# fhausmann/deepgrp

Measured on AMD Instinct MI355X. Metric: Mbp/sec predicted (whole node) at window=200 stride=50, 5-class, higher is better.
Workload: dtype f16

## Files before the change

### deepgrp_amd/_lib.py

```python
from __future__ import annotations

import ctypes as C
import os

_HERE = os.path.dirname(os.path.abspath(__file__))
LIB_PATH = os.path.join(_HERE, "libdeepgrp_hip.so")

i64, i32, vp, cint = C.c_int64, C.c_int32, C.c_void_p, C.c_int


class DgrpError(RuntimeError):
    """A libdeepgrp_hip call failed (message from dgrp_last_error())."""


class Segment(C.Structure):
    _fields_ = [("start", C.c_int64), ("end", C.c_int64), ("label", C.c_int32), ("contig", C.c_int32)]


class TrainJob(C.Structure):
    _fields_ = [("T", cint), ("u", cint), ("C", cint), ("attention", cint), ("d_params", vp), ("d_idx", vp), ("d_truth", vp),
                ("n", i64), ("d_starts", vp), ("B", i64), ("d_masks", vp), ("d_loss", vp), ("d_grads", vp), ("d_work", vp),
                ("work_bytes", i64)]


class InflateStreamStats(C.Structure):
    _fields_ = [(k, C.c_int64) for k in ("spans", "candidates", "repaired", "rounds", "longest_span", "false_starts", "chunks", "reserved")]

    def as_dict(self):
        return {k: int(getattr(self, k)) for k, _ in self._fields_ if k != "reserved"}


TRAIN_MAX_JOBS = 8

_SIGNATURES = {
    "dgrp_abi_version": (cint, []),
    "dgrp_last_error": (C.c_char_p, []),
    "dgrp_device_info": (cint, [C.c_char_p, C.c_size_t, C.POINTER(cint), C.POINTER(i64)]),
    "dgrp_strip_n": (cint, [vp, i64, C.POINTER(i64), C.POINTER(i64)]),
    "dgrp_encode": (cint, [vp, i64, vp, vp]),
    "dgrp_onehot": (cint, [vp, i64, vp, vp]),
    "dgrp_fasta_workspace_bytes": (i64, [i64]),
    "dgrp_fasta_encode": (cint, [vp, i64, vp, C.POINTER(i64), vp, i64, vp]),
    "dgrp_fasta_batch_workspace_bytes": (i64, [i64, i64]),
    "dgrp_fasta_encode_batch": (cint, [vp, i64, vp, vp, vp, vp, vp, i64, vp]),
    "dgrp_fasta_chunks_workspace_bytes": (i64, [i64]),
    "dgrp_fasta_chunks": (cint, [vp, i64, i64, vp, vp, C.POINTER(i64), vp, i64, vp]),
    "dgrp_fasta_mask_workspace_bytes": (i64, [i64, i64, i64]),
    "dgrp_fasta_mask_batch": (cint, [vp, i64, vp, vp, vp, vp, cint, C.c_uint64, vp, vp, i64, vp]),
    "dgrp_fasta_extract_workspace_bytes": (i64, [i64, i64, i64]),
    "dgrp_fasta_extract_batch": (cint, [vp, i64, vp, vp, vp, vp, vp, vp, i64, cint, C.c_uint64, vp, i64, C.POINTER(i64), vp, C.POINTER(i64),
                                        vp, i64, vp]),
    "dgrp_repeat_summary_workspace_bytes": (i64, [i64, i64, i64]),
    "dgrp_repeat_summary_batch": (cint, [vp, i64, vp, vp, vp, vp, cint, i64, vp, vp, vp, vp, vp, i64, vp]),
    "dgrp_twobit_workspace_bytes": (i64, [i64]),
    "dgrp_twobit_encode_batch": (cint, [vp, i64, i64, vp, vp, vp, vp, i64, vp, vp, i64, vp, i64, vp]),
    "dgrp_twobit_text_batch": (cint, [vp, i64, i64, vp, vp, vp, vp, vp, vp, i64, vp, vp, i64, vp, vp, i64, vp, i64, vp]),
    "dgrp_twobit_pack_workspace_bytes": (i64, [i64, i64]),
    "dgrp_twobit_pack_batch": (cint, [vp, i64, vp, vp, vp, i64, i64, vp, vp, vp, i64, vp]),
    "dgrp_format_rows_bound": (i64, [i64, i64]),
    "dgrp_format_rows": (cint, [vp, vp, i64, cint, vp, i64, vp, i64, C.POINTER(i64)]),
    "dgrp_track_workspace_bytes": (i64, [i64, i64]),
    "dgrp_track_text": (cint, [vp, i64, cint, cint, cint, i64, i64, C.c_char_p, i64, vp, i64, C.POINTER(i64), vp, i64, vp]),
    "dgrp_track_batch_workspace_bytes": (i64, [i64, vp, vp, i64, cint, i64]),
    "dgrp_track_text_batch": (cint, [vp, cint, i64, vp, vp, vp, C.c_char_p, vp, vp, cint, cint, i64, vp, i64, vp, vp, i64, vp]),
    "dgrp_track_index_workspace_bytes": (i64, [i64, vp, vp, i64, cint, i64]),
    "dgrp_track_index_batch": (cint, [vp, cint, i64, vp, vp, vp, C.c_char_p, vp, vp, cint, cint, i64, vp, i64, vp, vp, i64, vp, i64, vp]),
    "dgrp_track_sections_workspace_bytes": (i64, [i64, vp, vp, i64, cint]),
    "dgrp_track_sections_batch": (cint, [vp, cint, i64, vp, vp, vp, vp, cint, cint, i64, i64, vp, i64, vp, vp, i64, vp, vp, i64, vp]),
    "dgrp_track_zoom_workspace_bytes": (i64, [i64, vp, vp, i64, cint]),
    "dgrp_track_zoom_batch": (cint, [vp, cint, i64, vp, vp, vp, vp, cint, cint, i64, i64, vp, i64, vp, vp, i64, vp, vp, vp, i64, vp]),
    "dgrp_zlib_bound": (i64, [i64, i64]),
    "dgrp_zlib_workspace_bytes": (i64, [i64, cint]),
    "dgrp_zlib_compress_batch": (cint, [vp, i64, vp, i64, i64, cint, vp, i64, vp, C.POINTER(i64), vp, i64, vp]),
    "dgrp_zlib_compress_host": (cint, [vp, i64, vp, i64, i64, cint, vp, i64, vp, C.POINTER(i64)]),
    "dgrp_window_count":(i64, [i64, i64, i64]),
    "dgrp_windows_onehot": (cint, [vp, i64, i64, i64, i64, i64, cint, vp, vp]),
    "dgrp_model_create": (cint, [C.POINTER(vp), cint, cint, cint, cint, vp, vp, vp, vp, vp, vp]),
    "dgrp_model_create_lstm": (cint, [C.POINTER(vp), cint, cint, cint, vp, vp, vp, vp, vp]),
    "dgrp_model_destroy": (cint, [vp]),
    "dgrp_model_dims": (cint, [vp, C.POINTER(cint), C.POINTER(cint), C.POINTER(cint), C.POINTER(cint)]),
    "dgrp_model_flags": (cint, [vp]),
    "dgrp_model_set_precision": (cint, [vp, cint]),
    "dgrp_model_view": (cint, [vp, cint, C.POINTER(vp)]),
    "dgrp_model_plan": (cint, [vp, cint, i64, C.POINTER(cint), C.POINTER(i64), C.POINTER(cint), C.POINTER(cint)]),
    "dgrp_forward_workspace_bytes": (i64, [vp, i64]),
    "dgrp_forward_window_chunk": (i64, [vp]),
    "dgrp_forward_windows": (cint, [vp, vp, i64, i64, i64, i64, vp, vp, i64, vp]),
    "dgrp_forward_merge": (cint, [vp, vp, i64, i64, i64, i64, i64, vp, vp, i64, vp]),
    "dgrp_forward_merge_record": (cint, [vp, vp, i64, i64, i64, vp, vp, i64, vp]),
    "dgrp_forward_merge_record_workspace_bytes": (i64, [vp, i64, i64]),
    "dgrp_forward_reference_workspace_bytes": (i64, [vp, i64]),
    "dgrp_forward_windows_reference": (cint, [vp, vp, i64, i64, i64, i64, vp, vp, i64, vp]),
    "dgrp_get_max": (cint, [vp, i64, vp, i64, i64, i64, i64, vp]),
    "dgrp_scores": (cint, [vp, i64, cint, vp, vp, vp]),
    "dgrp_softmax_labels": (cint, [vp, i64, cint, vp, vp, vp, i64, vp]),
    "dgrp_mss_workspace_bytes": (i64, [i64]),
    "dgrp_mss_labels": (cint, [vp, vp, i64, cint, cint, cint, vp, vp, vp, i64, vp]),
    "dgrp_mss_segments_host": (cint, [vp, i64, vp, i64, C.POINTER(i64)]),
    "dgrp_mss_batch_workspace_bytes": (i64, [i64, i64]),
    "dgrp_mss_labels_batch": (cint, [vp, vp, i64, i64, vp, cint, cint, cint, vp, vp, i64, vp]),
    "dgrp_segments_workspace_bytes": (i64, [i64]),
    "dgrp_segments": (cint, [vp, i64, i64, i32, vp, i64, vp, vp, i64, vp]),
    "dgrp_record_workspace_bytes": (i64, [vp, i64, i64, cint]),
    "dgrp_predict_record": (cint, [vp, vp, i64, i64, i64, cint, cint, cint, i64, i32, vp, i64, C.POINTER(i64), vp, i64, vp]),
    "dgrp_batch_workspace_bytes": (i64, [vp, i64, vp, i64]),
    "dgrp_predict_batch": (cint, [vp, vp, i64, vp, vp, vp, vp, i64, i64, cint, cint, vp, i64, C.POINTER(i64), vp, i64, vp]),
    "dgrp_batch_rows": (i64, [i64, vp]),
    "dgrp_predict_batch_probs": (cint, [vp, vp, i64, vp, vp, vp, vp, i64, i64, cint, cint, vp, i64, C.POINTER(i64), vp, i64, vp, vp]),
    "dgrp_confusion_matrix": (cint, [vp, vp, i64, cint, vp, vp, vp]),
    "dgrp_filter_segments": (cint, [vp, vp, i64, i64, vp]),
    "dgrp_eval_workspace_bytes": (i64, [i64, i64]),
    "dgrp_paint_rows_batch": (cint, [vp, i64, vp, vp, vp, vp, vp, vp, i64, vp]),
    "dgrp_row_hits_batch": (cint, [vp, i64, vp, vp, vp, vp, vp, vp, vp, i64, vp]),
    "dgrp_row_scores_workspace_bytes": (i64, [i64, i64]),
    "dgrp_row_scores_batch": (cint, [vp, cint, i64, vp, vp, vp, vp, vp, vp, vp, i64, vp]),
    "dgrp_prob_hist_workspace_bytes": (i64, [i64, cint, cint]),
    "dgrp_prob_hist_batch": (cint, [vp, cint, i64, vp, vp, vp, vp, cint, vp, vp, vp, i64, vp]),
    "dgrp_row_detect_workspace_bytes": (i64, [i64, i64]),
    "dgrp_paint_row_keys_batch": (cint, [vp, i64, vp, vp, vp, vp, vp, vp, vp, i64, vp]),
    "dgrp_row_detect_batch": (cint, [vp, i64, vp, vp, vp, vp, vp, vp, vp, vp, i64, vp]),
    "dgrp_format_bed_bound": (i64, [i64, i64]),
    "dgrp_format_bed_rows": (cint, [vp, vp, i64, cint, vp, vp, i64, cint, vp, i64, C.POINTER(i64)]),
    "dgrp_bed_text_workspace_bytes": (i64, [i64, i64, i64]),
    "dgrp_bed_text_batch": (cint, [vp, vp, i64, cint, vp, vp, i64, cint, vp, i64, C.POINTER(i64), vp, i64, vp]),
    "dgrp_bed_index_workspace_bytes": (i64, [i64, i64, i64, i64]),
    "dgrp_bed_index_batch": (cint, [vp, vp, i64, cint, vp, vp, i64, cint, i64, vp, vp, i64, C.POINTER(i64), vp, i64, vp, vp, i64, vp]),
    "dgrp_gff_text_workspace_bytes": (i64, [i64, i64, i64, i64, i64]),
    "dgrp_gff_text_batch": (cint, [vp, vp, i64, cint, vp, vp, i64, vp, vp, i64, cint, i64, vp, i64, C.POINTER(i64), C.POINTER(i64), vp, i64,
                                   vp]),
    "dgrp_gff_index_workspace_bytes": (i64, [i64, i64, i64, i64, i64, i64]),
    "dgrp_gff_index_batch": (cint, [vp, vp, i64, cint, vp, vp, i64, vp, vp, i64, cint, i64, i64, vp, vp, i64, C.POINTER(i64), vp, i64, vp, vp,
                                    i64, vp]),
    "dgrp_bed_blocks_workspace_bytes": (i64, [i64, i64, vp]),
    "dgrp_bed_blocks_batch": (cint, [cint, vp, vp, i64, cint, i64, vp, i64, vp, i64, C.POINTER(i64), vp, i64, C.POINTER(i64), C.POINTER(i64),
                                     vp, i64, vp]),
    "dgrp_bed_zoom_workspace_bytes": (i64, [i64, i64, vp]),
    "dgrp_bed_zoom_batch": (cint, [cint, vp, vp, i64, cint, i64, vp, i64, vp, i64, vp, vp, i64, vp, vp, vp, i64, vp]),
    "dgrp_inflate_raw_host": (cint, [vp, i64, vp, i64, C.POINTER(i64), C.POINTER(i64), C.POINTER(cint)]),
    "dgrp_inflate_workspace_bytes": (i64, [i64]),
    "dgrp_inflate_batch": (cint, [vp, i64, i64, vp, vp, vp, vp, i64, C.POINTER(i64), C.POINTER(cint), vp, i64, vp]),
    "dgrp_inflate_stream_host": (cint, [vp, i64, i64, i64, cint, vp, i64, C.POINTER(i64), C.POINTER(i64), vp, C.POINTER(cint)]),
    "dgrp_inflate_stream_workspace_bytes": (i64, [i64, i64]),
    "dgrp_inflate_stream_scan": (cint, [vp, i64, i64, i64, i64, cint, C.POINTER(i64), vp, C.POINTER(cint), vp, i64, vp]),
    "dgrp_inflate_stream_write": (cint, [vp, i64, i64, i64, vp, vp, i64, C.POINTER(C.c_uint32), C.POINTER(i64), C.POINTER(cint), vp, i64,
                                         vp]),
    "dgrp_bgzf_bound": (i64, [i64, cint]),
    "dgrp_bgzf_workspace_bytes": (i64, [i64]),
    "dgrp_bgzf_compress": (cint, [vp, i64, vp, i64, C.POINTER(i64), cint, vp, i64, vp]),
    "dgrp_bgzf_compress_host": (cint, [vp, i64, vp, i64, C.POINTER(i64), cint]),
    "dgrp_bgzf_workspace_bytes_level": (i64, [i64, cint]),
    "dgrp_bgzf_compress_level": (cint, [vp, i64, vp, i64, C.POINTER(i64), cint, cint, vp, i64, vp]),
    "dgrp_bgzf_compress_host_level": (cint, [vp, i64, vp, i64, C.POINTER(i64), cint, cint]),
    "dgrp_train_param_count": (i64, [cint, cint, cint]),
    "dgrp_train_workspace_bytes": (i64, [cint, cint, cint, cint, i64]),
    "dgrp_train_step": (cint, [cint, cint, cint, cint, vp, vp, vp, i64, vp, i64, vp, vp, vp, vp, i64, vp]),
    "dgrp_train_step_multi": (cint, [C.POINTER(TrainJob), cint, vp]),
    "dgrp_optimizer_step": (cint, [cint, vp, vp, vp, vp, i64, C.c_double, C.c_double, C.c_double, C.c_double, i64, vp]),
    "dgrp_truth_workspace_bytes": (i64, [i64, i64]),
    "dgrp_truth_multihot_batch": (cint, [vp, cint, i64, i64, vp, vp, vp, vp, vp, vp, i64, vp]),
    "dgrp_class_starts_workspace_bytes": (i64, [i64, i64]),
    "dgrp_class_window_starts": (cint, [vp, i64, i64, vp, vp, cint, vp, i64, C.POINTER(i64), vp, i64, vp]),
    "dgrp_train_resolve_starts": (cint, [vp, i64, vp, vp, cint, vp, vp, i64, vp, vp]),
    "dgrp_kernel_timer_enable": (cint, [cint]),
    "dgrp_kernel_timer_read": (cint, [C.POINTER(C.c_double), C.POINTER(i64), C.POINTER(i64)]),
}

_lib = None


def lib() -> C.CDLL:
    global _lib
    if _lib is None:
        if not os.path.exists(LIB_PATH):
            raise ImportError(
                f"{LIB_PATH} is missing: build it with `make -C deepgrp_amd/csrc` (hipcc, gfx950) "
                "or `python -c 'import __graft_entry__ as g; g.build()'`. There is no CPU fallback.")
        import torch
        L = C.CDLL(LIB_PATH)
        for name, (res, args) in _SIGNATURES.items():
            f = getattr(L, name)
            f.restype = res
            f.argtypes = args
        if L.dgrp_abi_version() != 1:
            raise ImportError("libdeepgrp_hip.so ABI version mismatch")
        _lib = L
    return _lib


def check(rc: int, what: str = "") -> None:
    if rc != 0:
        msg = lib().dgrp_last_error().decode("utf-8", "replace")
        raise DgrpError(f"{what or 'libdeepgrp_hip'} failed (code {rc}): {msg}")


def name_blob(names):
    import numpy as np
    raw = [nm if isinstance(nm, bytes) else nm.encode("utf-8", "surrogateescape") for nm in names]
    off = np.zeros(len(raw) + 1, np.int64)
    np.cumsum([len(x) for x in raw], out=off[1:])
    return raw, b"".join(raw), off


def exported_symbols():
    return sorted(_SIGNATURES)
```

### deepgrp_amd/csrc/api.hip

```cpp
#include "dgrp_model.h"

#include <stdarg.h>
#include <string.h>

#include <algorithm>
#include <vector>
#include <mutex>

static thread_local char g_err[512] = "";

void dgrp_set_error(const char *fmt, ...)
{
    va_list ap;
    va_start(ap, fmt);
    vsnprintf(g_err, sizeof(g_err), fmt, ap);
    va_end(ap);
}

DGRP_EXPORT int dgrp_abi_version(void) { return DGRP_ABI_VERSION; }
DGRP_EXPORT const char *dgrp_last_error(void) { return g_err; }

DGRP_EXPORT int dgrp_device_info(char *name, size_t name_cap, int *cu_count, int64_t *hbm_bytes)
{
    int dev = 0;
// ... 545 lines not shown

DGRP_EXPORT int dgrp_model_plan(const dgrp_model *m, int mode, int64_t step, int *kernel, int64_t *lds_bytes, int *ospan, int *avg_up)
{
    DGRP_REQUIRE(m, "dgrp_model_plan: NULL model");
    DGRP_REQUIRE(kernel && lds_bytes && ospan && avg_up, "dgrp_model_plan: NULL output pointer");
    DGRP_REQUIRE(mode >= 0 && mode <= 2, "dgrp_model_plan: mode %d (0 merged, 1 window probabilities, 2 attention pre-pass)", mode);
    DGRP_REQUIRE(step >= 1, "dgrp_model_plan: step %lld < 1", (long long)step);
    DGRP_REQUIRE(mode != 2 || m->attention, "dgrp_model_plan: mode 2 on a model without attention");
    if (m->ref_only) {
        *kernel = DGRP_KERNEL_FP32; *lds_bytes = 0; *ospan = 0; *avg_up = 0;
        return DGRP_OK;
    }
    const dgrp_gru_plan plan = dgrp_gru_plan_for(m, mode, step);
    *kernel = (int)plan.kernel; *lds_bytes = (int64_t)plan.lds; *ospan = plan.ospan; *avg_up = plan.avg_up;
    return DGRP_OK;
}

DGRP_EXPORT int dgrp_model_set_precision(dgrp_model *m, int level)
{
    DGRP_REQUIRE(m, "dgrp_model_set_precision: NULL model");
    DGRP_REQUIRE(level == 0 || level == 1, "dgrp_model_set_precision: level must be 0 (fp16 operands) or 1 (split operands)");
    if (m->ref_only) return DGRP_OK;
    DGRP_REQUIRE(level == 0 || m->d_pack_lo || m->d_stream, "dgrp_model_set_precision: this model has no split-operand kernel");
    m->precision = level;
    return DGRP_OK;
}

static int64_t ref_sub_windows(const dgrp_model *m)
{
    const int64_t per = 2 * (int64_t)m->T * m->u * 4 + (int64_t)m->T * (m->C + 1) * 4 + 2 * (int64_t)m->u * 4;
    return std::max<int64_t>(16, std::min<int64_t>(4096, (512ll << 20) / per) / 16 * 16);
}

DGRP_EXPORT int64_t dgrp_forward_workspace_bytes(const dgrp_model *m, int64_t nw)
{
    if (!m || nw < 0) return 0;
    if (m->ref_only) {
        const int64_t sub = std::min<int64_t>(ref_sub_windows(m), std::max<int64_t>(nw, 1));
        return dgrp_align_up(dgrp_forward_reference_workspace_bytes(m, sub), 256) + dgrp_align_up(sub * m->T * (int64_t)m->C * 4, 256);
    }
    if (!m->attention) return 256;
    return dgrp_align_up(nw * m->T * (int64_t)m->UP * 4, 256) + dgrp_align_up(nw * m->T * (int64_t)m->C * 4, 256) + 256;
}

static unsigned *forward_queue(const dgrp_model *m, int64_t nw, void *d_work, int64_t work_bytes)
{
    if (!d_work || work_bytes < dgrp_forward_workspace_bytes(m, nw)) return nullptr;
    return (unsigned *)((char *)d_work + (m->attention ? dgrp_forward_workspace_bytes(m, nw) - 256 : 0));
}

static int forward_ref(const dgrp_model *m, const uint8_t *d_idx, int64_t n, int64_t s, dgrp_placement place, int64_t w0, int64_t nw,
                       int merge, float *d_out, void *d_work, int64_t work_bytes, hipStream_t stream)
{
    if (work_bytes < dgrp_forward_workspace_bytes(m, nw) || !d_work) {
        dgrp_set_error("dgrp_forward: this model runs on the fp32 kernels and needs %lld bytes of workspace for %lld windows",
                       (long long)dgrp_forward_workspace_bytes(m, nw), (long long)nw);
        return DGRP_ENOMEM;
    }
    const int64_t sub = std::min<int64_t>(ref_sub_windows(m), nw);
    const int64_t ref_bytes = dgrp_align_up(dgrp_forward_reference_workspace_bytes(m, sub), 256);
    float *probs = (float *)((char *)d_work + ref_bytes);
    for (int64_t a = w0; a < w0 + nw; a += sub) {
        const int64_t k = std::min<int64_t>(sub, w0 + nw - a);
        float *dst = merge ? probs : d_out + (a - w0) * (int64_t)m->T * m->C;
        int rc = dgrp_forward_windows_reference(m, d_idx, n, s, a, k, dst, d_work, ref_bytes, stream);
        if (rc) return rc;
        if (!merge) continue;
        for (int64_t b = a; b < a + k;) {
            const int64_t e = (b < place.nfullB && a + k > place.nfullB) ? place.nfullB : a + k;
            const int64_t row = dgrp_place_row(place, b, s);
            if (row < n) {
                rc = dgrp_get_max(d_out + row * m->C, n - row, probs + (b - a) * (int64_t)m->T * m->C, m->T, m->C, s, e - b, stream);
                if (rc) return rc;
            }
            b = e;
        }
    }
    return DGRP_OK;
}

static int forward_common(const dgrp_model *m, const uint8_t *d_idx, int64_t n, int64_t s, int64_t batch, int64_t w0,
                          int64_t nw, int merge, float *d_out, void *d_work, int64_t work_bytes, hipStream_t stream)
{
    DGRP_REQUIRE(m && s >= 1 && w0 >= 0 && nw >= 0 && n >= 0, "dgrp_forward: bad arguments");
    if (nw == 0) return DGRP_OK;
    DGRP_REQUIRE(d_idx && d_out, "dgrp_forward: NULL pointer");
    DGRP_REQUIRE((w0 + nw - 1) * s + m->T <= n, "dgrp_forward: window %lld (start %lld) runs past n=%lld",
                 (long long)(w0 + nw - 1), (long long)((w0 + nw - 1) * s), (long long)n);
    dgrp_placement place = { 0, 0 };
    if (merge) {
        DGRP_REQUIRE(batch >= 1, "dgrp_forward_merge: batch must be >= 1");
        const int64_t total = dgrp_window_count(n, m->T, s);
        DGRP_REQUIRE(w0 + nw <= total, "dgrp_forward_merge: windows %lld..%lld exceed the record's %lld",
                     (long long)w0, (long long)(w0 + nw), (long long)total);
        place = dgrp_make_placement(total, batch);
    }
    if (m->ref_only) return forward_ref(m, d_idx, n, s, place, w0, nw, merge, d_out, d_work, work_bytes, stream);
    if (!m->attention)
        return dgrp_gru_launch(m, dgrp_gru_plan_for(m, merge ? 0 : 1, s), d_idx, n, place, w0, nw, d_out, nullptr,
                               forward_queue(m, nw, d_work, work_bytes), stream);
    if (work_bytes < dgrp_forward_workspace_bytes(m, nw) || !d_work) {
        dgrp_set_error("dgrp_forward: attention model needs %lld bytes of workspace for %lld windows",
                       (long long)dgrp_forward_workspace_bytes(m, nw), (long long)nw);
        return DGRP_ENOMEM;
    }
    void *avg = d_work;
    float *pl = (float *)((char *)d_work + dgrp_align_up(nw * m->T * (int64_t)m->UP * 4, 256));
    const dgrp_gru_plan pre = dgrp_gru_plan_for(m, 2, s);
    int rc = dgrp_gru_launch(m, pre, d_idx, n, place, w0, nw, pl, avg, forward_queue(m, nw, d_work, work_bytes), stream);
    if (rc) return rc;
    return dgrp_attention_launch_recs(m, pre, place, w0, nw, merge, n, avg, pl, d_out, nullptr, 0, stream);
}

DGRP_EXPORT int dgrp_forward_windows(const dgrp_model *m, const uint8_t *d_idx, int64_t n, int64_t s, int64_t w0,
                                     int64_t nw, float *d_probs, void *d_work, int64_t work_bytes, void *stream)
{
    return forward_common(m, d_idx, n, s, 1, w0, nw, 0, d_probs, d_work, work_bytes, (hipStream_t)stream);
}

DGRP_EXPORT int dgrp_forward_merge(const dgrp_model *m, const uint8_t *d_idx, int64_t n, int64_t s, int64_t batch,
                                   int64_t w0, int64_t nw, float *d_out, void *d_work, int64_t work_bytes, void *stream)
{
    return forward_common(m, d_idx, n, s, batch, w0, nw, 1, d_out, d_work, work_bytes, (hipStream_t)stream);
}

static int64_t spill_cap_bytes()
{
    static const int64_t cap = [] {
        if (const char *e = getenv("DGRP_SPILL_BYTES")) {
            const long long v = atoll(e);
            if (v >= (1ll << 20)) return (int64_t)v;
        }
        size_t free_b = 0, total_b = 0;
        if (hipMemGetInfo(&free_b, &total_b) != hipSuccess || total_b == 0) return (int64_t)(4ll << 30);
        return std::min<int64_t>(8ll << 30, std::max<int64_t>(1ll << 30, (int64_t)(total_b / 32)));
    }();
    return cap;
}

static int64_t record_window_chunk(const dgrp_model *m)
{
    if (m->ref_only) return ref_sub_windows(m);
    if (!m->attention) return 1ll << 23;
    const int64_t per = (int64_t)m->T * ((int64_t)m->UP * 4 + (int64_t)m->C * 4);
    int64_t c = spill_cap_bytes() / per;
    c = c >= 32768 ? c / 32768 * 32768 : c >= 4096 ? c / 4096 * 4096 : c / 16 * 16;
    if (c < 16) c = 16;
    return c < (1ll << 20) ? c : (1ll << 20);
}

DGRP_EXPORT int64_t dgrp_forward_window_chunk(const dgrp_model *m)
{
    return m ? record_window_chunk(m) : 0;
}

#define DGRP_LANES 3
static int64_t lane_window_chunk(const dgrp_model *m)
{
    if (m->ref_only || !m->attention) return 0;
    if (const char *e = getenv("DGRP_LANE_CHUNK")) {
        const long long v = atoll(e);
        return v >= 16 ? (int64_t)(v / 16 * 16) : 0;
    }
    const int64_t c = record_window_chunk(m);
    if (c < 65536) return 0;
    const int64_t lc = c / DGRP_LANES / 32768 * 32768;
    return lc >= 32768 ? lc : 32768;
}
struct lane_pool { hipStream_t s[DGRP_LANES]; int dev; bool ok; };
static lane_pool *lanes_get()
{
    static std::mutex mu;
    static std::vector<lane_pool *> pools;
    int dev = 0;
    if (hipGetDevice(&dev) != hipSuccess) return nullptr;
    std::lock_guard<std::mutex> lock(mu);
    for (lane_pool *q : pools)
        if (q->dev == dev) return q->ok ? q : nullptr;
    lane_pool *q = new lane_pool();
    q->dev = dev; q->ok = true;
    for (int i = 0; i < DGRP_LANES; ++i)
        if (hipStreamCreateWithFlags(&q->s[i], hipStreamNonBlocking) != hipSuccess) q->ok = false;
    pools.push_back(q);
    return q->ok ? q : nullptr;
}

static int64_t record_forward_bytes(const dgrp_model *m, int64_t nwin)
{
    const int64_t lc = lane_window_chunk(m);
    if (lc > 0 && nwin > lc)
        return DGRP_LANES * dgrp_align_up(std::max<int64_t>(dgrp_forward_workspace_bytes(m, std::min(lc, nwin)), 256), 256);
    const int64_t chunk = std::min<int64_t>(record_window_chunk(m), nwin > 0 ? nwin : 1);
    return std::max<int64_t>(dgrp_forward_workspace_bytes(m, chunk), 256);
}

DGRP_EXPORT int64_t dgrp_forward_merge_record_workspace_bytes(const dgrp_model *m, int64_t n, int64_t s)
{
    if (!m || n < 0 || s < 1) return 0;
    return record_forward_bytes(m, dgrp_window_count(n, m->T, s));
}

DGRP_EXPORT int dgrp_forward_merge_record(const dgrp_model *m, const uint8_t *d_idx, int64_t n, int64_t s, int64_t batch, float *d_out,
                                          void *d_work, int64_t work_bytes, void *stream_)
{
    hipStream_t stream = (hipStream_t)stream_;
    DGRP_REQUIRE(m && n >= 0 && s >= 1 && batch >= 1, "dgrp_forward_merge_record: bad arguments");
    const int64_t nwin = dgrp_window_count(n, m->T, s);
    if (nwin == 0) return DGRP_OK;
    DGRP_REQUIRE(d_idx && d_out && d_work, "dgrp_forward_merge_record: NULL pointer");
    const int64_t need = record_forward_bytes(m, nwin);
    if (work_bytes < need) {
        dgrp_set_error("dgrp_forward_merge_record: workspace %lld < %lld bytes", (long long)work_bytes, (long long)need);
        return DGRP_ENOMEM;
    }
    const int64_t lc = lane_window_chunk(m);
    lane_pool *lp = lc > 0 && nwin > lc ? lanes_get() : nullptr;
    if (!lp) {
        const int64_t chunk = lc > 0 && nwin > lc ? lc : record_window_chunk(m);
        for (int64_t w0 = 0; w0 < nwin; w0 += chunk) {
            const int64_t nw = std::min<int64_t>(chunk, nwin - w0);
            const int rc = dgrp_forward_merge(m, d_idx, n, s, batch, w0, nw, d_out, d_work, work_bytes, stream);
            if (rc) return rc;
        }
        return DGRP_OK;
    }
    const int64_t per = need / DGRP_LANES;
    hipEvent_t fork = nullptr, join[DGRP_LANES] = { nullptr, nullptr, nullptr };
    int rc = DGRP_OK;
    auto bail = [&](hipError_t e) { if (e != hipSuccess && rc == DGRP_OK) { dgrp_set_error("dgrp_forward_merge_record: %s", hipGetErrorString(e)); rc = DGRP_EHIP; } };
    bail(hipEventCreateWithFlags(&fork, hipEventDisableTiming));
    for (int i = 0; i < DGRP_LANES; ++i) bail(hipEventCreateWithFlags(&join[i], hipEventDisableTiming));
    if (rc == DGRP_OK) {
        bail(hipEventRecord(fork, stream));
        for (int i = 0; i < DGRP_LANES; ++i) bail(hipStreamWaitEvent(lp->s[i], fork, 0));
        int64_t k = 0;
        for (int64_t w0 = 0; w0 < nwin && rc == DGRP_OK; w0 += lc, ++k) {
            const int64_t nw = std::min<int64_t>(lc, nwin - w0);
            const int lane = (int)(k % DGRP_LANES);
            rc = dgrp_forward_merge(m, d_idx, n, s, batch, w0, nw, d_out, (char *)d_work + lane * per, per, lp->s[lane]);
        }
        for (int i = 0; i < DGRP_LANES; ++i) {
            bail(hipEventRecord(join[i], lp->s[i]));
            bail(hipStreamWaitEvent(stream, join[i], 0));
        }
    }
    if (fork) (void)hipEventDestroy(fork);
    for (int i = 0; i < DGRP_LANES; ++i)
        if (join[i]) (void)hipEventDestroy(join[i]);
    return rc;
}

struct record_layout {
    int64_t out, scores, cls, labels, count, fwd, post, bytes, post_bytes, fwd_bytes;
};

static record_layout record_carve(const dgrp_model *m, int64_t n, int64_t s, int use_mss)
{
    record_layout l;
    int64_t p = 0;
    auto take = [&](int64_t b) { const int64_t q = p; p += dgrp_align_up(b, 256); return q; };
    const int64_t nwin = dgrp_window_count(n, m->T, s);
    l.out = take(n * m->C * 4);
    l.scores = take(use_mss ? n * 8 : 0);
    l.cls = take(use_mss ? n : 0);
    l.labels = take(n);
    l.count = take(8);
    l.fwd_bytes = record_forward_bytes(m, nwin);
    l.fwd = take(l.fwd_bytes);
    l.post_bytes = std::max<int64_t>(std::max<int64_t>(use_mss ? dgrp_mss_workspace_bytes(n) : 4096, dgrp_segments_workspace_bytes(n)), 4096);
    l.post = take(l.post_bytes);
    l.bytes = p;
    return l;
}

DGRP_EXPORT int64_t dgrp_record_workspace_bytes(const dgrp_model *m, int64_t n, int64_t s, int use_mss)
{
    if (!m || n < 0 || s < 1) return 0;
    return record_carve(m, n, s, use_mss).bytes;
}

DGRP_EXPORT int dgrp_predict_record(const dgrp_model *m, const uint8_t *d_idx, int64_t n, int64_t s, int64_t batch,
                                    int min_mss_len, int xdrop_len, int use_mss, int64_t offset, int32_t contig,
                                    dgrp_segment *d_records, int64_t cap, int64_t *h_count, void *d_work,
                                    int64_t work_bytes, void *stream_)
{
    hipStream_t stream = (hipStream_t)stream_;
    DGRP_REQUIRE(m && n >= 0 && s >= 1 && batch >= 1 && cap >= 0 && h_count, "dgrp_predict_record: bad arguments");
    *h_count = 0;
    if (n == 0) return DGRP_OK;
    DGRP_REQUIRE(d_idx && d_work && (cap == 0 || d_records), "dgrp_predict_record: NULL pointer");
    const record_layout l = record_carve(m, n, s, use_mss);
    if (work_bytes < l.bytes) {
        dgrp_set_error("dgrp_predict_record: workspace %lld < %lld bytes", (long long)work_bytes, (long long)l.bytes);
        return DGRP_ENOMEM;
    }
    char *w = (char *)d_work;
    float *out = (float *)(w + l.out);
    int8_t *labels = (int8_t *)(w + l.labels);
    int64_t *d_count = (int64_t *)(w + l.count);
    DGRP_HIP(hipMemsetAsync(out, 0, (size_t)n * m->C * 4, stream));
    int rc = dgrp_forward_merge_record(m, d_idx, n, s, batch, out, w + l.fwd, l.fwd_bytes, stream);
    if (rc) return rc;
    if (use_mss) {
        rc = dgrp_scores(out, n, m->C, (double *)(w + l.scores), (int8_t *)(w + l.cls), stream);
        if (rc) return rc;
        rc = dgrp_mss_labels((const double *)(w + l.scores), (const int8_t *)(w + l.cls), n, m->C, min_mss_len, xdrop_len,
                             labels, nullptr, w + l.post, l.post_bytes, stream);
    } else {
        rc = dgrp_softmax_labels(out, n, m->C, nullptr, labels, w + l.post, l.post_bytes, stream);
    }
    if (rc) return rc;
    rc = dgrp_segments(labels, n, offset, contig, d_records, cap, d_count, w + l.post, l.post_bytes, stream);
    if (rc) return rc;
    DGRP_HIP(hipMemcpyAsync(h_count, d_count, 8, hipMemcpyDeviceToHost, stream));
    DGRP_HIP(hipStreamSynchronize(stream));
    return DGRP_OK;
}

int dgrp_batch_marks(const int64_t *d_start, const int64_t *d_len, int64_t nrec, int64_t total_n, uint8_t *d_marks,
                     double *d_scores, int8_t *d_cls, hipStream_t stream);
int dgrp_batch_segments(const int8_t *d_labels, const uint8_t *d_marks, int64_t total_n, const int64_t *d_start, int64_t nrec,
                        const int64_t *d_startpos, const int32_t *d_contig, dgrp_segment *d_records, int64_t cap,
                        int64_t *d_count, void *d_work, int64_t work_bytes, hipStream_t stream);

struct batch_layout {
    int64_t out, scores, cls, labels, marks, count, recs, wgf, start, len, spos, contig, post, post_bytes, avg, pl, queue, bytes;
};

static batch_layout batch_carve(const dgrp_model *m, int64_t nrec, int64_t total_rows, int64_t total_windows)
{
    batch_layout l;
    int64_t p = 0;
    auto take = [&](int64_t b) { const int64_t q = p; p += dgrp_align_up(b, 256); return q; };
    l.out = take(total_rows * m->C * 4);
    l.scores = take(total_rows * 8);
    l.cls = take(total_rows);
    l.labels = take(total_rows);
    l.marks = take(total_rows);
    l.count = take(8);
    l.recs = take(nrec * 64);
    l.wgf = take((nrec + 1) * 8);
    l.start = take((nrec + 1) * 8);
    l.len = take(nrec * 8);
    l.spos = take(nrec * 8);
    l.contig = take(nrec * 4);
    l.post_bytes = std::max<int64_t>(std::max<int64_t>(dgrp_mss_batch_workspace_bytes(total_rows, nrec), dgrp_segments_workspace_bytes(total_rows)), 4096);
    l.post = take(l.post_bytes);
    l.avg = take(m->attention ? total_windows * m->T * (int64_t)m->UP * 4 : 0);
    l.pl = take(m->attention ? total_windows * m->T * (int64_t)m->C * 4 : 0);
    l.queue = take(4);
    l.bytes = p;
    return l;
}

static int64_t batch_windows(const dgrp_model *m, int64_t nrec, const int64_t *h_n, int64_t s)
{
    int64_t w = 0;
    for (int64_t r = 0; r < nrec; ++r) w += dgrp_window_count(h_n[r], m->T, s);
    return w;
}

static int64_t batch_rows(int64_t nrec, const int64_t *h_n)
{
    int64_t rows = 0;
    for (int64_t r = 0; r < nrec; ++r) rows += dgrp_align_up(h_n[r], 64);
    return rows;
}

DGRP_EXPORT int64_t dgrp_batch_workspace_bytes(const dgrp_model *m, int64_t nrec, const int64_t *h_n, int64_t s)
{
    if (!m || nrec < 0 || s < 1 || (nrec > 0 && !h_n)) return 0;
    for (int64_t r = 0; r < nrec; ++r)
        if (h_n[r] < 1) return 0;
    return batch_carve(m, nrec, batch_rows(nrec, h_n), batch_windows(m, nrec, h_n, s)).bytes;
}

DGRP_EXPORT int64_t dgrp_batch_rows(int64_t nrec, const int64_t *h_n)
{
    return nrec > 0 && h_n ? batch_rows(nrec, h_n) : 0;
}

static int predict_batch_common(const char *who, const dgrp_model *m, const uint8_t *d_idx, int64_t nrec, const int64_t *h_idx_off,
                                const int64_t *h_n, const int64_t *h_startpos, const int32_t *h_contig, int64_t s,
                                int64_t batch, int min_mss_len, int xdrop_len, dgrp_segment *d_records, int64_t cap,
                                int64_t *h_count, void *d_work, int64_t work_bytes, hipStream_t stream, float *d_probs)
{
    DGRP_REQUIRE(m && nrec >= 0 && s >= 1 && batch >= 1 && cap >= 0 && h_count, "%s: bad arguments", who);
    *h_count = 0;
    if (nrec == 0) return DGRP_OK;
    DGRP_REQUIRE(!m->ref_only && (m->cell == 0 || (m->cell == 1 && m->NW <= 8)), "%s: unsupported model (fp32 path: record by record)", who);
    DGRP_REQUIRE(d_idx && h_idx_off && h_n && h_startpos && h_contig && d_work && (cap == 0 || d_records), "%s: NULL pointer", who);
    for (int64_t r = 0; r < nrec; ++r)
        DGRP_REQUIRE(h_n[r] >= 1 && h_idx_off[r] >= 0, "%s: record %lld: empty records do not belong in a batch", who, (long long)r);
    const int64_t rows = batch_rows(nrec, h_n);
    DGRP_REQUIRE(rows < (1ll << 31), "%s: %lld rows in one batch (limit 2^31)", who, (long long)rows);
    const int64_t windows = batch_windows(m, nrec, h_n, s);
    DGRP_REQUIRE(windows < (1ll << 31), "%s: too many windows in one batch", who);
    const batch_layout l = batch_carve(m, nrec, rows, windows);
    if (work_bytes < l.bytes) {
        dgrp_set_error("%s: workspace %lld < %lld bytes", who, (long long)work_bytes, (long long)l.bytes);
        return DGRP_ENOMEM;
    }
    char *w = (char *)d_work;
    std::vector<int64_t> recs((size_t)nrec * 8, 0), wgf((size_t)nrec + 1, 0), start((size_t)nrec + 1, 0);
    int64_t wfirst = 0;
    for (int64_t r = 0; r < nrec; ++r) {
        const int64_t nwin = dgrp_window_count(h_n[r], m->T, s);
        const dgrp_placement pl = dgrp_make_placement(nwin, batch);
        int64_t *e = recs.data() + (size_t)r * 8;
        e[0] = h_idx_off[r]; e[1] = h_n[r]; e[2] = start[(size_t)r]; e[3] = nwin; e[4] = pl.nfullB; e[5] = pl.shift; e[6] = wfirst;
        wfirst += nwin;
        wgf[(size_t)r + 1] = wgf[(size_t)r] + (nwin + 15) / 16;
        start[(size_t)r + 1] = start[(size_t)r] + dgrp_align_up(h_n[r], 64);
    }
    DGRP_HIP(hipMemcpyAsync(w + l.recs, recs.data(), recs.size() * 8, hipMemcpyHostToDevice, stream));
    DGRP_HIP(hipMemcpyAsync(w + l.wgf, wgf.data(), wgf.size() * 8, hipMemcpyHostToDevice, stream));
    DGRP_HIP(hipMemcpyAsync(w + l.start, start.data(), start.size() * 8, hipMemcpyHostToDevice, stream));
    DGRP_HIP(hipMemcpyAsync(w + l.len, h_n, (size_t)nrec * 8, hipMemcpyHostToDevice, stream));
    DGRP_HIP(hipMemcpyAsync(w + l.spos, h_startpos, (size_t)nrec * 8, hipMemcpyHostToDevice, stream));
    DGRP_HIP(hipMemcpyAsync(w + l.contig, h_contig, (size_t)nrec * 4, hipMemcpyHostToDevice, stream));
    float *out = d_probs ? d_probs : (float *)(w + l.out);
    DGRP_HIP(hipMemsetAsync(out, 0, (size_t)rows * m->C * 4, stream));
    int rc;
    if (!m->attention) {
        rc = dgrp_gru_launch_batch(m, dgrp_gru_plan_for(m, 0, s), d_idx, w + l.recs, (const int64_t *)(w + l.wgf), nrec, wgf[(size_t)nrec],
                                   out, nullptr, (unsigned *)(w + l.queue), stream);
        if (rc) return rc;
    } else {
        const dgrp_gru_plan pre = dgrp_gru_plan_for(m, 2, s);
        rc = dgrp_gru_launch_batch(m, pre, d_idx, w + l.recs, (const int64_t *)(w + l.wgf), nrec, wgf[(size_t)nrec], (float *)(w + l.pl),
                                   w + l.avg, (unsigned *)(w + l.queue), stream);
        if (rc) return rc;
        rc = dgrp_attention_launch_recs(m, pre, dgrp_placement{ 0, 0 }, 0, windows, 1, rows, w + l.avg, (const float *)(w + l.pl), out,
                                        w + l.recs, nrec, stream);
        if (rc) return rc;
    }
    double *scores = (double *)(w + l.scores);
    int8_t *cls = (int8_t *)(w + l.cls), *labels = (int8_t *)(w + l.labels);
    uint8_t *marks = (uint8_t *)(w + l.marks);
    rc = dgrp_scores(out, rows, m->C, scores, cls, stream);
    if (rc) return rc;
    rc = dgrp_batch_marks((const int64_t *)(w + l.start), (const int64_t *)(w + l.len), nrec, rows, marks, scores, cls, stream);
    if (rc) return rc;
    rc = dgrp_mss_labels_batch(scores, cls, rows, nrec, start.data(), m->C, min_mss_len, xdrop_len, labels, w + l.post, l.post_bytes, stream);
    if (rc) return rc;
    int64_t *d_count = (int64_t *)(w + l.count);
    rc = dgrp_batch_segments(labels, marks, rows, (const int64_t *)(w + l.start), nrec, (const int64_t *)(w + l.spos),
                             (const int32_t *)(w + l.contig), d_records, cap, d_count, w + l.post, l.post_bytes, stream);
    if (rc) return rc;
    DGRP_HIP(hipMemcpyAsync(h_count, d_count, 8, hipMemcpyDeviceToHost, stream));
    DGRP_HIP(hipStreamSynchronize(stream));
    return DGRP_OK;
}

DGRP_EXPORT int dgrp_predict_batch(const dgrp_model *m, const uint8_t *d_idx, int64_t nrec, const int64_t *h_idx_off,
                                   const int64_t *h_n, const int64_t *h_startpos, const int32_t *h_contig, int64_t s,
                                   int64_t batch, int min_mss_len, int xdrop_len, dgrp_segment *d_records, int64_t cap,
                                   int64_t *h_count, void *d_work, int64_t work_bytes, void *stream)
{
    return predict_batch_common("dgrp_predict_batch", m, d_idx, nrec, h_idx_off, h_n, h_startpos, h_contig, s, batch, min_mss_len, xdrop_len,
                                d_records, cap, h_count, d_work, work_bytes, (hipStream_t)stream, nullptr);
}

DGRP_EXPORT int dgrp_predict_batch_probs(const dgrp_model *m, const uint8_t *d_idx, int64_t nrec, const int64_t *h_idx_off,
                                         const int64_t *h_n, const int64_t *h_startpos, const int32_t *h_contig, int64_t s,
                                         int64_t batch, int min_mss_len, int xdrop_len, dgrp_segment *d_records, int64_t cap,
                                         int64_t *h_count, void *d_work, int64_t work_bytes, void *stream, float *d_probs)
{
    DGRP_REQUIRE(d_probs || nrec <= 0, "dgrp_predict_batch_probs: NULL d_probs");
    return predict_batch_common("dgrp_predict_batch_probs", m, d_idx, nrec, h_idx_off, h_n, h_startpos, h_contig, s, batch, min_mss_len,
                                xdrop_len, d_records, cap, h_count, d_work, work_bytes, (hipStream_t)stream, d_probs);
}
```

### deepgrp_amd/csrc/mss_kernels.hip

```cpp
#include "dgrp_common.h"
#include "scan.h"
#include <vector>
#include <math.h>

struct mss_cand { int32_t st, en; double L, R; int32_t pre, pad; };

#define MSS_SUB_MIN 256
#define MSS_SUBENT_BYTES 80
struct mss_subent {
    int64_t start, run;
    double L, peak, run_L;
    int64_t run_st;
    int32_t open, first;
    int32_t vci, nst;
    int32_t reset, pad;
    double Lf;
};
static_assert(sizeof(mss_subent) == 80, "MSS_SUBENT_BYTES");
#define MSS_LCAP 160
#define MSS_NEG (-1e30)
#define MSS_QNONE (-4096)
#define MSS_QBAD 4096

struct mss_layout {
    int64_t nblk;
    uint64_t *blk;
    double *blk_sum;
    double *blk_abs;
    int32_t *blk_q;
    uint8_t *flags;
    int64_t nsup;
    double *sup_sum, *sup_abs;
    int32_t *sup_q;
    uint8_t *sup_flags;
    uint64_t *tiles;
    uint64_t *grand;
    int64_t *ustart;
    int64_t *urun;
    double *exitL[2];
    uint64_t *segcnt;
    uint64_t *cutcnt;
    uint64_t *lblk;
    int64_t *lstart, *lrun;
    uint8_t *lforced;
    void *lstate[2];
    int64_t *cut_st, *cut_run;
    double *cut_L;
    int2 *cut_kj;
    int64_t *ustart2, *urun2;
    double *entry2;
    void *subs;
    int64_t dump_cap;
    mss_cand *dump;
    mss_cand *stack;
    int32_t *segs;
    int32_t *segs_out;
    int64_t bytes;
};

static mss_layout mss_carve(void *work, int64_t n)
{
    mss_layout l;
    unsigned char *p = (unsigned char *)work;
    auto take = [&](int64_t bytes) { unsigned char *q = p; p += dgrp_align_up(bytes, 256); return q; };
    l.nblk = (n + 63) / 64;
    const int64_t maxunits = l.nblk + 1, maxruns = n / 2 + 2;
    l.blk = (uint64_t *)take((l.nblk + 1) * 8);
    l.blk_sum = (double *)take(l.nblk * 8);
    l.blk_abs = (double *)take(l.nblk * 8);
    l.blk_q = (int32_t *)take(l.nblk * 4);
    l.flags = (uint8_t *)take(l.nblk + 64);
    l.nsup = (l.nblk + 63) / 64;
    l.sup_sum = (double *)take(l.nsup * 8);
    l.sup_abs = (double *)take(l.nsup * 8);
    l.sup_q = (int32_t *)take(l.nsup * 4);
    l.sup_flags = (uint8_t *)take(l.nsup + 64);
    l.tiles = (uint64_t *)take(((maxunits + 1 + SCAN_TILE - 1) / SCAN_TILE + 1) * 8);
    l.grand = (uint64_t *)take(64);
    l.ustart = (int64_t *)take((maxunits + 1) * 8);
    l.urun = (int64_t *)take((maxunits + 1) * 8);
    l.exitL[0] = (double *)take(maxunits * 8);
    l.exitL[1] = (double *)take(maxunits * 8);
    l.segcnt = (uint64_t *)take((maxunits + 1) * 8);
    l.cutcnt = (uint64_t *)take((maxunits + 1) * 8);
    l.lblk = (uint64_t *)take((l.nblk + 1) * 8);
    l.lstart = (int64_t *)take((maxunits + 1) * 8);
    l.lrun = (int64_t *)take((maxunits + 1) * 8);
    l.lforced = (uint8_t *)take(maxunits + 64);
    l.lstate[0] = take(maxunits * 64);
    l.lstate[1] = take(maxunits * 64);
    l.cut_st = (int64_t *)take(l.nblk * 8);
    l.cut_run = (int64_t *)take(l.nblk * 8);
    l.cut_L = (double *)take(l.nblk * 8);
    l.cut_kj = (int2 *)take(l.nblk * 8);
    l.ustart2 = (int64_t *)take((2 * maxunits + 2) * 8);
    l.urun2 = (int64_t *)take((2 * maxunits + 2) * 8);
    l.entry2 = (double *)take((2 * maxunits + 2) * 8);
    l.subs = take((maxunits + 8) * (int64_t)MSS_SUBENT_BYTES);
    l.dump_cap = 2 * (l.nblk / MSS_SUB_MIN + 2);
    l.dump = (mss_cand *)take(l.dump_cap * MSS_LCAP * (int64_t)sizeof(mss_cand));
    l.stack = (mss_cand *)take(maxruns * (int64_t)sizeof(mss_cand));
    l.segs = (int32_t *)take(maxruns * 8);
    l.segs_out = (int32_t *)take(maxruns * 8);
    l.bytes = p - (unsigned char *)work;
    return l;
}

DGRP_EXPORT int64_t dgrp_mss_workspace_bytes(int64_t n)
{
    if (n < 0) return 0;
    return mss_carve(nullptr, n).bytes;
}

__device__ __forceinline__ int quantum_exp(double x)
{
    const uint64_t b = (uint64_t)__double_as_longlong(x) & 0x7fffffffffffffffull;
    if (b == 0) return MSS_QNONE;
    const int e = (int)(b >> 52);
    if (e == 0 || e == 0x7ff) return MSS_QBAD;
    const uint64_t m = b & 0x000fffffffffffffull;
    const int tz = m ? __builtin_ctzll(m) : 52;
    return -((e - 1023) - 52 + tz);
}

__device__ __forceinline__ bool mss_certified(double L, double sumabs, int q_scores)
{
    const int qL = quantum_exp(L);
    const int Q = qL > q_scores ? qL : q_scores;
    if (Q >= MSS_QBAD) return false;
    const int ex = 53 - Q;
    if (ex > 1000) return true;
    if (ex < -1000) return false;
    return (fabs(L) + sumabs) * 1.0000001 < ldexp(1.0, ex);
}

__device__ __forceinline__ double wave_sum(double v)
{
#pragma unroll
    for (int o = 32; o > 0; o >>= 1) v += __shfl_xor(v, o);
    return v;
}
__device__ __forceinline__ int wave_max(int v)
{
#pragma unroll
    for (int o = 32; o > 0; o >>= 1) { int w = __shfl_xor(v, o); v = w > v ? w : v; }
    return v;
}

__device__ __forceinline__ double lane_value(double x, int l)
{
    const long long b = __double_as_longlong(x);
    const int lo = __builtin_amdgcn_readlane((int)b, l), hi = __builtin_amdgcn_readlane((int)(b >> 32), l);
    return __longlong_as_double(((long long)hi << 32) | (unsigned int)lo);
}

__global__ void __launch_bounds__(256) mss_blockstat_kernel(const double *__restrict__ S, int64_t n,
                                                            uint64_t *__restrict__ blk, double *__restrict__ blk_sum,
                                                            double *__restrict__ blk_abs, int32_t *__restrict__ blk_q,
                                                            uint8_t *__restrict__ flags)
{
    const int lane = threadIdx.x & 63;
    const int64_t b = (int64_t)blockIdx.x * 4 + (threadIdx.x >> 6);
    if (b * 64 >= n) return;
    const int64_t i = b * 64 + lane;
    const double s = i < n ? S[i] : 0.0;
    const bool pos = i < n && s > 0;
    const bool prevpos = i > 0 && i < n && S[i - 1] > 0;
    const unsigned long long mpos = __ballot(pos);
    const unsigned long long mstart = __ballot(pos && !prevpos);
    const double sum = wave_sum(s), sabs = wave_sum(fabs(s));
    const int q = wave_max(quantum_exp(s));
    if (lane == 0) {
        flags[b] = (uint8_t)(mpos != 0ull ? 1 : 0);
        blk[b] = (uint64_t)__popcll(mstart);
        blk_sum[b] = sum;
        blk_abs[b] = sabs;
        blk_q[b] = q;
    }
}

__global__ void __launch_bounds__(256) mss_superstat_kernel(const double *__restrict__ blk_sum, const double *__restrict__ blk_abs,
                                                            const int32_t *__restrict__ blk_q, const uint8_t *__restrict__ flags,
                                                            int64_t nblk, double *__restrict__ sup_sum, double *__restrict__ sup_abs,
                                                            int32_t *__restrict__ sup_q, uint8_t *__restrict__ sup_flags)
{
    const int lane = threadIdx.x & 63;
    const int64_t g = (int64_t)blockIdx.x * 4 + (threadIdx.x >> 6);
    if (g * 64 >= nblk) return;
    const int64_t b = g * 64 + lane;
    const bool in = b < nblk;
    const unsigned long long mp = __ballot(in && (flags[b] & 1));
    const double sum = wave_sum(in ? blk_sum[b] : 0.0), sabs = wave_sum(in ? blk_abs[b] : 0.0);
    const int q = wave_max(in ? blk_q[b] : MSS_QNONE);
    if (lane == 0) {
        sup_flags[g] = (uint8_t)(mp != 0ull ? 1 : 0);
        sup_sum[g] = sum;
        sup_abs[g] = sabs;
        sup_q[g] = q;
    }
}

__device__ __forceinline__ bool mss_is_boundary(const uint8_t *flags, const double *blk_sum, int64_t b, int64_t nblk,
                                                int64_t n, double thr)
{
    if (!(thr > 0.0) || b + 1 >= nblk || (flags[b] & 1) || !(flags[b + 1] & 1)) return false;
    if (b * 64 + 64 > n) return false;
    double cum = 0.0;
    for (int64_t j = b; j >= 0 && j > b - 16; --j) {
        if (flags[j] & 1) break;
        cum += blk_sum[j];
        if (cum < -thr) return true;
    }
    return false;
}

__global__ void __launch_bounds__(256) mss_boundary_kernel(const uint8_t *__restrict__ flags, const double *__restrict__ blk_sum,
                                                           int64_t nblk, int64_t n, double thr, uint64_t *__restrict__ blk)
{
    const int64_t b = (int64_t)blockIdx.x * blockDim.x + threadIdx.x;
    if (b >= nblk) return;
    if (mss_is_boundary(flags, blk_sum, b, nblk, n, thr)) blk[b] |= 1ull << 32;
}

__global__ void __launch_bounds__(256) mss_units_kernel(const uint64_t *__restrict__ blk, const uint8_t *__restrict__ flags,
                                                        const double *__restrict__ blk_sum, int64_t nblk, int64_t n, double thr,
                                                        int64_t *__restrict__ ustart, int64_t *__restrict__ urun,
                                                        const uint64_t *__restrict__ grand)
{
    const int64_t b = (int64_t)blockIdx.x * blockDim.x + threadIdx.x;
    if (b == 0) {
        ustart[0] = 0;
        urun[0] = 0;
        const int64_t nunits = (int64_t)(grand[0] >> 32) + 1;
        ustart[nunits] = n;
        urun[nunits] = (int64_t)(grand[0] & 0xffffffffull);
    }
    if (b >= nblk) return;
    if (mss_is_boundary(flags, blk_sum, b, nblk, n, thr)) {
        const int64_t k = (int64_t)(blk[b] >> 32) + 1;
        ustart[k] = (b + 1) * 64;
        urun[k] = (int64_t)(blk[b] & 0xffffffffull);
    }
}

template <int CTRL, int RMASK>
__device__ __forceinline__ int dpp_i(int src, int old) { return __builtin_amdgcn_update_dpp(old, src, CTRL, RMASK, 0xf, false); }
template <int CTRL, int RMASK>
__device__ __forceinline__ double dpp_d(double src, double old)
{
    const long long s = __double_as_longlong(src), o = __double_as_longlong(old);
    const int lo = __builtin_amdgcn_update_dpp((int)o, (int)s, CTRL, RMASK, 0xf, false);
    const int hi = __builtin_amdgcn_update_dpp((int)(o >> 32), (int)(s >> 32), CTRL, RMASK, 0xf, false);
    return __longlong_as_double(((long long)hi << 32) | (unsigned int)lo);
}
#define DPP_SHR(n) (0x110 + (n))
#define DPP_BCAST15 0x142
#define DPP_BCAST31 0x143
#define DPP_WAVE_SHR1 0x138
#define DPP_SCAN_STEPS(STEP) STEP(DPP_SHR(1), 0xf) STEP(DPP_SHR(2), 0xf) STEP(DPP_SHR(4), 0xf) STEP(DPP_SHR(8), 0xf) STEP(DPP_BCAST15, 0xa) STEP(DPP_BCAST31, 0xc)
__device__ __forceinline__ double scan_add_d(double x)
{
#define STEP(c, m) x = x + dpp_d<c, m>(x, 0.0);
    DPP_SCAN_STEPS(STEP)
#undef STEP
    return x;
}
__device__ __forceinline__ double scan_min_d(double x)
{
#define STEP(c, m) { const double y = dpp_d<c, m>(x, INFINITY); x = y < x ? y : x; }
    DPP_SCAN_STEPS(STEP)
#undef STEP
    return x;
}
__device__ __forceinline__ int scan_max_i(int x)
{
#define STEP(c, m) { const int y = dpp_i<c, m>(x, -1); x = y > x ? y : x; }
    DPP_SCAN_STEPS(STEP)
#undef STEP
    return x;
}
__device__ __forceinline__ void scan_segmax_d(int &fl, double &v)
{
#define STEP(c, m) { const double yv = dpp_d<c, m>(v, -INFINITY); const int yf = dpp_i<c, m>(fl, 0); if (!fl) v = yv > v ? yv : v; fl |= yf; }
    DPP_SCAN_STEPS(STEP)
#undef STEP
}
__device__ __forceinline__ double lane_below_d(double x, double first) { return dpp_d<DPP_WAVE_SHR1, 0xf>(x, first); }
__device__ __forceinline__ int lane_below_i(int x, int first) { return dpp_i<DPP_WAVE_SHR1, 0xf>(x, first); }
__device__ __forceinline__ int lane_value_i(int x, int l) { return __builtin_amdgcn_readlane(x, l); }

__device__ __forceinline__ double mss_fold(double s, double a0, int t, int nvalid, int lane)
{
    const double sm = lane >= t && lane < nvalid ? s : 0.0;
    double X = a0;
    for (int j = t; j < nvalid; j += 4) {
        X = lane_below_d(X, a0) + sm;
        X = lane_below_d(X, a0) + sm;
        X = lane_below_d(X, a0) + sm;
        X = lane_below_d(X, a0) + sm;
    }
    return X;
}

__global__ void __launch_bounds__(64) mss_scan_kernel(const double *__restrict__ S, const int64_t *__restrict__ ustart,
                                                      const int64_t *__restrict__ urun, int64_t nunits,
                                                      const double *__restrict__ exit_prev, double *__restrict__ exit_cur,
                                                      mss_cand *stack_all, int32_t *__restrict__ segs_all,
                                                      uint64_t *__restrict__ segcnt, int min_sc, double xdrop,
                                                      uint64_t *__restrict__ grand, int pass,
                                                      const double *__restrict__ blk_sum, const double *__restrict__ blk_abs,
                                                      const int32_t *__restrict__ blk_q, const uint8_t *__restrict__ flags,
                                                      const double *__restrict__ sup_sum, const double *__restrict__ sup_abs,
                                                      const int32_t *__restrict__ sup_q, const uint8_t *__restrict__ sup_flags,
                                                      int have_stats, int independent, int cutmode,
                                                      mss_subent *subs, mss_cand *dump_all)
{
    __shared__ double2 sLR[MSS_LCAP];
    __shared__ int4 sIdx[MSS_LCAP];
    const int lane = threadIdx.x;
    const int64_t k = blockIdx.x;
    const bool sub = subs != nullptr;
    const bool head = !sub || subs[k].first != 0;
    const bool tail = !sub || k + 1 == nunits || subs[k + 1].first != 0;
    const int64_t begin = sub ? subs[k].start : ustart[k], end = sub ? subs[k + 1].start : ustart[k + 1];
    const int64_t slot0 = sub ? subs[k].run : urun[k];
    volatile mss_cand *ovf = stack_all + slot0;
    int32_t *segs = segs_all + 2 * slot0;
    int64_t nst = 0, nseg = 0;
    double cur = sub ? subs[k].L : (k == 0 || independent) ? 0.0 : exit_prev[k - 1];
    double peak = sub && !head ? subs[k].peak : MSS_NEG;
    bool run_open = sub && !head && subs[k].open != 0;
    int64_t run_st = run_open ? subs[k].run_st : 0;
    double run_L = run_open ? subs[k].run_L : 0.0;
    bool was_reset = false;
    double Lf = sub && !head ? subs[k].Lf : INFINITY;

    struct cand_v { double L, R; int32_t st, en, pre, open; };
    auto get = [&](int64_t j) -> cand_v {
        cand_v c;
        if (j < MSS_LCAP) {
            const double2 lr = sLR[j];
            const int4 ix = sIdx[j];
            c.L = lr.x; c.R = lr.y; c.st = ix.x; c.en = ix.y; c.pre = ix.z; c.open = ix.w;
        } else {
            volatile mss_cand *o = ovf + (j - MSS_LCAP);
            c.L = o->L; c.R = o->R; c.st = o->st; c.en = o->en; c.pre = o->pre; c.open = o->pad;
        }
        return c;
    };

    auto flush = [&]() {
        for (int64_t base = 0; base < nst; base += 64) {
            const int64_t j = base + lane;
            bool keep = false;
            int32_t a = 0, b = 0;
            if (j < nst) {
                const cand_v c = get(j);
                keep = c.R - c.L >= min_sc;
                a = c.st;
                b = c.en;
            }
            const unsigned long long m = __ballot(keep);
            if (keep) {
                const int64_t slot = nseg + __popcll(m & ((1ull << lane) - 1ull));
                segs[2 * slot] = a;
                segs[2 * slot + 1] = b;
            }
            nseg += __popcll(m);
        }
        nst = 0;
    };

    auto close_run = [&](double R, int64_t en) {
        if (R > peak) peak = R;
        if (!head && run_L <= Lf) { Lf = run_L; peak = R; }
        int32_t tst = (int32_t)run_st;
        double tL = run_L;
        int64_t j;
        for (;;) {
            j = nst - 1;
            cand_v c;
            while (j >= 0) {
                c = get(j);
                if (c.L < tL) break;
                j = c.pre >= 0 ? c.pre : j - 1;
            }
            if (j >= 0 && c.R < R) {
                tst = c.st;
                tL = c.L;
                nst = j;
                continue;
            }
            break;
        }
        const int lopen = j < 0 && !head ? 1 : 0;
        if (j < 0 && head) { flush(); peak = R; }
        if (was_reset && lane == 0) { atomicOr((unsigned long long *)&grand[2], 1ull); atomicOr((unsigned long long *)&grand[4], 8ull); }
        if (nst < MSS_LCAP) {
            if (lane == 0) {
                sLR[nst] = make_double2(tL, R);
                sIdx[nst] = make_int4(tst, (int32_t)en, (int32_t)j, lopen);
            }
        } else {
            volatile mss_cand *c = ovf + (nst - MSS_LCAP);
            c->st = tst; c->en = (int32_t)en; c->L = tL; c->R = R; c->pre = (int32_t)j; c->pad = lopen;
        }
        __threadfence_block();
        ++nst;
        run_open = false;
    };
    auto reset_flush = [&]() {
        if (head) flush(); else { was_reset = true; Lf = INFINITY; }
    };

    int64_t pos = begin;
    while (pos < end) {
        const int nvalid = (int)min((int64_t)64, end - pos);
        if (have_stats && !run_open && peak == MSS_NEG && (pos & 63) == 0) {
            if ((pos & 4095) == 0) {
                const int64_t gj = (pos >> 12) + lane;
                const bool stop2 = gj * 4096 + 4096 > end || (sup_flags[gj] & 1);
                const unsigned long long ms2 = __ballot(stop2);
                const int m2 = ms2 ? __builtin_ctzll(ms2) : 64;
                if (m2 > 0) {
                    const bool in = lane < m2;
                    const double gs = wave_sum(in ? sup_sum[gj] : 0.0);
                    const double ga = wave_sum(in ? sup_abs[gj] : 0.0);
                    const int gq = wave_max(in ? sup_q[gj] : MSS_QNONE);
                    if (mss_certified(cur, ga, gq)) {
                        cur += gs;
                        pos += (int64_t)m2 * 4096;
                        continue;
                    }
                }
            }
            const int64_t b0 = pos >> 6, bend = (end + 63) >> 6;
            const int64_t bj = b0 + lane;
            const bool stop = bj >= bend || (flags[bj] & 1) || (bj * 64 + 64 > end) || (lane > 0 && (bj & 63) == 0);
            const unsigned long long mstop = __ballot(stop);
            const int m = mstop ? __builtin_ctzll(mstop) : 64;
            if (m > 0) {
                const bool in = lane < m;
                const double gs = wave_sum(in ? blk_sum[bj] : 0.0);
                const double ga = wave_sum(in ? blk_abs[bj] : 0.0);
                const int gq = wave_max(in ? blk_q[bj] : MSS_QNONE);
                if (mss_certified(cur, ga, gq)) {
                    cur += gs;
                    pos += (int64_t)m * 64;
                    continue;
                }
            }
        }
        const double s = lane < nvalid ? S[pos + lane] : 0.0;
        const bool ispos = lane < nvalid && s > 0;
        const unsigned long long vmask = nvalid == 64 ? ~0ull : ((1ull << nvalid) - 1ull);
        const unsigned long long mpos = __ballot(ispos);
        const double sabs = wave_sum(fabs(s));
        const int q = wave_max(quantum_exp(s));
        const bool cert = mss_certified(cur, sabs, q);
        if (cert || (q < MSS_QBAD && quantum_exp(cur) < MSS_QBAD)) {
            double pre = s;
            if (cert) {
#pragma unroll
                for (int o = 1; o < 64; o <<= 1) {
                    const double y = __shfl_up(pre, o);
                    if (lane >= o) pre += y;
                }
            } else {
                pre = mss_fold(s, cur, 0, nvalid, lane);
            }
            double base = cert ? cur : 0.0;
            const double front = cur;
            int p = 0;
            if (nst >= 1 && nst <= MSS_LCAP) {
                const cand_v c0 = get(nst - 1);
                const int64_t nb = c0.pre;
                const bool lone = nst == 1 && !c0.open;
                double lim = INFINITY;
                if (!lone && nb >= 0) lim = get(nb).R;
                if (lone || nb >= 0 || c0.open) {
                const double V = base + pre;
                const bool edge_close = run_open && !(mpos & 1ull);
                const bool isend = ispos && lane + 1 < nvalid && !((mpos >> (lane + 1)) & 1ull);
                const bool isstart = ispos && (lane == 0 ? !run_open : !((mpos >> (lane - 1)) & 1ull));
                double vprev = __shfl_up(V, 1);
                if (lane == 0) vprev = cur;
                double rmax = isend ? V : -INFINITY;
#pragma unroll
                for (int o = 1; o < 64; o <<= 1) {
                    const double y = __shfl_up(rmax, o);
                    if (lane >= o) rmax = y > rmax ? y : rmax;
                }
                double before = __shfl_up(rmax, 1);
                if (lane == 0) before = -INFINITY;
                const double base_r = edge_close ? cur : c0.R;
                const double base_peak = edge_close ? (lone ? cur : (cur > peak ? cur : peak)) : peak;
                const double top_r = before > base_r ? before : base_r;
                const double peak_i = lone ? (before > -INFINITY ? before : base_peak) : (before > base_peak ? before : base_peak);
                bool ok = !run_open || c0.L < run_L;
                if (edge_close) ok = ok && cur > c0.R && !(lim < cur);
                if (isend) ok = ok && V > top_r && !(lim < V);
                if (isstart) ok = ok && (c0.L < vprev);
                if (lane < nvalid && !ispos && xdrop > 0.0 && V + xdrop < peak_i) ok = false;
                if (__all(ok)) {
                    const unsigned long long mend = __ballot(isend);
                    if (mend || edge_close) {
                        const int last = mend ? 63 - __builtin_clzll(mend) : -1;
                        const double newR = mend ? lane_value(V, last) : cur;
                        if (lane == 0) {
                            sLR[nst - 1] = make_double2(c0.L, newR);
                            sIdx[nst - 1] = make_int4(c0.st, (int32_t)(pos + last + 1), (int32_t)nb, c0.open);
                        }
                        __threadfence_block();
                        peak = lone ? newR : (newR > peak ? newR : peak);
                    }
                    if ((mpos >> (nvalid - 1)) & 1ull) {
                        const unsigned long long znon = ~mpos & vmask;
                        if (znon || !run_open) {
                            const int ls = znon ? 64 - __builtin_clzll(znon) : 0;
                            run_st = pos + ls;
                            run_L = ls == 0 ? cur : lane_value(V, ls - 1);
                        }
                        run_open = true;
                    } else {
                        run_open = false;
                    }
                    cur = lane_value(V, nvalid - 1);
                    pos += nvalid;
                    continue;
                }
                }
            }
            while (p < nvalid) {
                const unsigned long long rest = vmask & ~((1ull << p) - 1ull);
                if ((mpos >> p) & 1ull) {
                    const unsigned long long z = ~mpos & rest;
                    const int e = z ? __builtin_ctzll(z) : nvalid;
                    if (!run_open) { run_open = true; run_st = pos + p; run_L = p == 0 ? front : base + lane_value(pre, p - 1); }
                    cur = base + lane_value(pre, e - 1);
                    p = e;
                    if (e < nvalid) close_run(cur, pos + e);
                } else {
                    if (run_open) close_run(cur, pos + p);
                    const unsigned long long z = mpos & rest;
                    const int e = z ? __builtin_ctzll(z) : nvalid;
                    if (xdrop > 0.0 && peak != MSS_NEG) {
                        const bool trig = lane >= p && lane < e && ((base + pre) + xdrop < peak);
                        const unsigned long long mt = __ballot(trig);
                        if (mt) {
                            const int t = __builtin_ctzll(mt);
                            reset_flush();
                            peak = MSS_NEG;
                            if (cert) base = t == 0 ? 0.0 : -lane_value(pre, t - 1);
                            else pre = mss_fold(s, 0.0, t, nvalid, lane);
                        }
                    }
                    cur = base + lane_value(pre, e - 1);
                    p = e;
                }
            }
        } else {
            for (int i = 0; i < nvalid; ++i) {
                const double v = lane_value(s, i);
                if (v > 0) {
                    if (!run_open) { run_open = true; run_st = pos + i; run_L = cur; }
                    cur = cur + v;
                } else {
                    if (run_open) close_run(cur, pos + i);
                    if (xdrop > 0.0 && cur + v + xdrop < peak) { reset_flush(); cur = 0.0; peak = MSS_NEG; }
                    cur += v;
                }
            }
        }
        pos += nvalid;
    }
    if (run_open && tail) close_run(cur, end);
    if (sub && !(head && tail)) {
        const int64_t slot = head ? 2 * (int64_t)subs[k + 1].vci + 1 : 2 * (int64_t)subs[k].vci;
        mss_cand *d = dump_all + slot * MSS_LCAP;
        for (int64_t j = lane; j < nst && j < MSS_LCAP; j += 64) {
            const double2 lr = sLR[j];
            const int4 ix = sIdx[j];
            mss_cand c;
            c.st = ix.x; c.en = ix.y; c.L = lr.x; c.R = lr.y; c.pre = ix.z; c.pad = ix.w;
            d[j] = c;
        }
        if (lane == 0) {
            subs[k].nst = (int32_t)(nst < (1ll << 31) ? nst : -1);
            subs[k].reset = was_reset ? 1 : 0;
        }
    } else if (k == nunits - 1 || independent || cutmode) {
        flush();
    } else if (nst != 0 || peak != MSS_NEG) {
        if (lane == 0) atomicOr((unsigned long long *)&grand[2], 1ull);
    }
    if (lane == 0) {
        segcnt[k] = (uint64_t)nseg;
        const double want = sub ? subs[k + 1].L : exit_prev[k];
        if (!independent && (pass == 0 || __double_as_longlong(want) != __double_as_longlong(cur)))
            atomicOr((unsigned long long *)&grand[1], 1ull);
        exit_cur[k] = cur;
    }
}

__global__ void __launch_bounds__(64) mss_stitch_kernel(mss_subent *subs, int64_t nunits, mss_cand *stack_all, const mss_cand *dump_all,
                                                        int32_t *__restrict__ segs_all, uint64_t *__restrict__ segcnt, int min_sc,
                                                        uint64_t *__restrict__ grand)
{
    const int lane = threadIdx.x;
    const int64_t k = blockIdx.x;
    if (!subs[k].first || k + 1 >= nunits || subs[k + 1].first) return;
    __shared__ mss_cand loc[256];
    volatile mss_cand *T = stack_all + subs[k].run;
    int64_t nT = subs[k].nst;
    bool bad = nT < 0;
    if (!bad) {
        for (int64_t hi = nT; hi > MSS_LCAP; hi -= 64) {
            const int64_t j = hi - 1 - lane;
            mss_cand c;
            const bool on = j >= MSS_LCAP;
            if (on) { volatile mss_cand *o = T + (j - MSS_LCAP); c.st = o->st; c.en = o->en; c.L = o->L; c.R = o->R; c.pre = o->pre; c.pad = 0; }
            __threadfence_block();
            if (on) { volatile mss_cand *o = T + j; o->st = c.st; o->en = c.en; o->L = c.L; o->R = c.R; o->pre = c.pre; o->pad = 0; }
            __threadfence_block();
        }
        const mss_cand *d = dump_all + (2 * (int64_t)subs[k + 1].vci + 1) * MSS_LCAP;
        for (int64_t j = lane; j < nT && j < MSS_LCAP; j += 64) {
            const mss_cand c = d[j];
            volatile mss_cand *o = T + j; o->st = c.st; o->en = c.en; o->L = c.L; o->R = c.R; o->pre = c.pre; o->pad = 0;
        }
        __threadfence();
    }
    int64_t nseg = (int64_t)segcnt[k];
    int32_t *segs = segs_all + 2 * subs[k].run;
    auto flush_T = [&]() {
        for (int64_t base = 0; base < nT; base += 64) {
            const int64_t j = base + lane;
            bool keep = false;
            int32_t a = 0, b = 0;
            if (j < nT) {
                volatile mss_cand *c = T + j;
                keep = c->R - c->L >= min_sc;
                a = c->st;
                b = c->en;
            }
            const unsigned long long m = __ballot(keep);
            if (keep) {
                const int64_t slot = nseg + __popcll(m & ((1ull << lane) - 1ull));
                segs[2 * slot] = a;
                segs[2 * slot + 1] = b;
            }
            nseg += __popcll(m);
        }
        nT = 0;
    };
    for (int64_t u = k + 1; !bad && u < nunits && !subs[u].first; ++u) {
        const int64_t nl = subs[u].nst;
        if (nl < 0) { bad = true; break; }
        const mss_cand *d = dump_all + 2 * (int64_t)subs[u].vci * MSS_LCAP;
        const mss_cand *deep = stack_all + subs[u].run;
        if (nl > MSS_LCAP && subs[k].run + nT > subs[u].run) { bad = true; break; }
        int64_t w = 0;
        auto load_chunk = [&]() {
            const int64_t j = w + lane;
            if (j < nl) loc[j & 255] = j < MSS_LCAP ? d[j] : deep[j - MSS_LCAP];
            w += 64;
        };
        __syncthreads();
        while (w < nl && w < 256) load_chunk();
        __syncthreads();
        int64_t delta = 0;
        for (int64_t i = 0; i < nl && !bad; ++i) {
            if (w < nl && i + 192 >= w) {
                if (subs[k].run + nT > subs[u].run + w - MSS_LCAP) { bad = true; break; }
                __syncthreads();
                load_chunk();
                __syncthreads();
            }
            const mss_cand e = loc[i & 255];
            int32_t tst = e.st, pre;
            double tL = e.L;
            if (e.pad) {
                int64_t j;
                for (;;) {
                    j = nT - 1;
                    double cL = 0.0, cR = 0.0;
                    int32_t cst = 0;
                    while (j >= 0) {
                        volatile mss_cand *c = T + j;
                        cL = c->L;
                        if (cL < tL) { cR = c->R; cst = c->st; break; }
                        const int32_t pr = c->pre;
                        j = pr >= 0 ? pr : j - 1;
                    }
                    if (j >= 0 && cR < e.R) { tst = cst; tL = cL; nT = j; continue; }
                    break;
                }
                if (j < 0 && nT > 0) flush_T();
                pre = (int32_t)j;
                delta = nT - i;
            } else {
                if (i == 0 || e.pre < 0) { bad = true; if (lane == 0) atomicOr((unsigned long long *)&grand[4], 4ull); break; }
                pre = (int32_t)(e.pre + delta);
            }
            volatile mss_cand *o = T + nT;
            o->st = tst; o->en = e.en; o->L = tL; o->R = e.R; o->pre = pre; o->pad = 0;
            __threadfence();
            ++nT;
        }
    }
    if (bad) {
        if (lane == 0) atomicOr((unsigned long long *)&grand[2], 1ull);
        return;
    }
    flush_T();
    if (lane == 0) segcnt[k] = (uint64_t)nseg;
}

#define MSS_LIGHT_SUB 2048
struct mss_light_state {
    double L, peak, Lf, run_L;
    int64_t run_st, run_slot;
    int64_t last_blk, open;
};

__global__ void __launch_bounds__(256) mss_lightflag_kernel(const uint8_t *__restrict__ flags, const double *__restrict__ blk_sum,
                                                            int64_t nblk, int64_t n, double thr, int sub, int use_forced,
                                                            uint64_t *__restrict__ lblk)
{
    const int64_t b = (int64_t)blockIdx.x * blockDim.x + threadIdx.x;
    if (b >= nblk) return;
    const bool forced = use_forced && mss_is_boundary(flags, blk_sum, b, nblk, n, thr);
    const bool spec = ((b + 1) % sub) == 0 && (b + 1) * 64 < n;
    lblk[b] = forced || spec ? 1 : 0;
}

__global__ void __launch_bounds__(256) mss_lightunits_kernel(const uint64_t *__restrict__ lblk, const uint64_t *__restrict__ lcount,
                                                             const uint8_t *__restrict__ flags, const double *__restrict__ blk_sum,
                                                             const uint64_t *__restrict__ runs_before, const uint64_t *__restrict__ runs_total,
                                                             int64_t nblk, int64_t n, double thr, int sub, int use_forced,
                                                             int64_t *__restrict__ lstart, int64_t *__restrict__ lrun,
                                                             uint8_t *__restrict__ lforced)
{
    const int64_t b = (int64_t)blockIdx.x * blockDim.x + threadIdx.x;
    if (b == 0) {
        lstart[0] = 0; lrun[0] = 0; lforced[0] = 1;
        const int64_t nl = (int64_t)*lcount + 1;
        lstart[nl] = n; lrun[nl] = (int64_t)(*runs_total & 0xffffffffull); lforced[nl] = 1;
    }
    if (b >= nblk) return;
    const bool forced = use_forced && mss_is_boundary(flags, blk_sum, b, nblk, n, thr);
    const bool spec = ((b + 1) % sub) == 0 && (b + 1) * 64 < n;
    if (forced || spec) {
        const int64_t j = (int64_t)lblk[b] + 1;
        lstart[j] = (b + 1) * 64;
        lrun[j] = (int64_t)((b + 1 < nblk ? runs_before[b + 1] : *runs_total) & 0xffffffffull);
        lforced[j] = forced ? 1 : 0;
    }
}

__global__ void __launch_bounds__(64) mss_light_kernel(const double *__restrict__ S, const int64_t *__restrict__ ustart,
                                                       const int64_t *__restrict__ urun, const uint8_t *__restrict__ uforced,
                                                       int64_t nunits, const mss_light_state *__restrict__ st_prev,
                                                       mss_light_state *__restrict__ st_cur,
                                                       double xdrop, uint64_t *__restrict__ grand, int pass,
                                                       const double *__restrict__ blk_sum, const double *__restrict__ blk_abs,
                                                       const int32_t *__restrict__ blk_q, const uint8_t *__restrict__ flags,
                                                       const double *__restrict__ sup_sum, const double *__restrict__ sup_abs,
                                                       const int32_t *__restrict__ sup_q, const uint8_t *__restrict__ sup_flags,
                                                       uint64_t *__restrict__ cut_cnt, int64_t *__restrict__ cut_st,
                                                       int64_t *__restrict__ cut_run, double *__restrict__ cut_L,
                                                       int2 *__restrict__ cut_kj)
{
    const int lane = threadIdx.x;
    const int64_t k = blockIdx.x;
    const int64_t begin = ustart[k], end = ustart[k + 1];
    const int64_t slot0 = urun[k];
    const bool forced = uforced[k] != 0;
    double cur = 0.0, peak = MSS_NEG, Lf = INFINITY, run_L = 0.0;
    bool run_open = false;
    int64_t run_st = 0, run_slot = 0;
    int64_t last_blk = begin >> 6;
    if (k > 0 && pass > 0) {
        const mss_light_state e = st_prev[k - 1];
        cur = e.L; peak = e.peak; Lf = e.Lf; run_L = e.run_L;
        run_st = e.run_st; run_slot = e.run_slot; run_open = e.open != 0;
        if (!forced) last_blk = e.last_blk;
    }
    int64_t nruns = 0;
    int64_t ncut = forced ? 1 : 0;
    auto file_cut = [&](int64_t st, int64_t slot, double Ls) {
        if (lane == 0) {
            const int64_t b = st >> 6;
            cut_st[b] = st; cut_run[b] = slot; cut_L[b] = Ls; cut_kj[b] = make_int2((int)k, (int)ncut);
        }
    };

    auto close_scalar = [&](double Ls, double R, int64_t st, int64_t slot) {
        if (R > peak) peak = R;
        if (Ls <= Lf) {
            Lf = Ls;
            peak = R;
            if ((st >> 6) != last_blk) {
                file_cut(st, slot, Ls);
                ++ncut;
                last_blk = st >> 6;
            }
        }
    };

    int64_t pos = begin;
    int64_t pf_pos = -1;
    double pf_s = 0.0, pf_abs = 0.0;
    int pf_q = 0;
    while (pos < end) {
        const int nvalid = (int)min((int64_t)(64 - (pos & 63)), end - pos);
        if (!run_open && peak == MSS_NEG && (pos & 63) == 0) {
            if ((pos & 4095) == 0) {
                const int64_t gj = (pos >> 12) + lane;
                const bool stop2 = gj * 4096 + 4096 > end || (sup_flags[gj] & 1);
                const unsigned long long ms2 = __ballot(stop2);
                const int m2 = ms2 ? __builtin_ctzll(ms2) : 64;
                if (m2 > 0) {
                    const bool in = lane < m2;
                    const double gs = wave_sum(in ? sup_sum[gj] : 0.0);
                    const double ga = wave_sum(in ? sup_abs[gj] : 0.0);
                    const int gq = wave_max(in ? sup_q[gj] : MSS_QNONE);
                    if (mss_certified(cur, ga, gq)) { cur += gs; pos += (int64_t)m2 * 4096; continue; }
                }
            }
            const int64_t b0 = pos >> 6, bend = (end + 63) >> 6;
            const int64_t bj = b0 + lane;
            const bool stop = bj >= bend || (flags[bj] & 1) || (bj * 64 + 64 > end) || (lane > 0 && (bj & 63) == 0);
            const unsigned long long mstop = __ballot(stop);
            const int m = mstop ? __builtin_ctzll(mstop) : 64;
            if (m > 0) {
                const bool in = lane < m;
                const double gs = wave_sum(in ? blk_sum[bj] : 0.0);
                const double ga = wave_sum(in ? blk_abs[bj] : 0.0);
                const int gq = wave_max(in ? blk_q[bj] : MSS_QNONE);
                if (mss_certified(cur, ga, gq)) { cur += gs; pos += (int64_t)m * 64; continue; }
            }
        }
        const bool whole = nvalid == 64;
        double s, sabs;
        int q;
        if (pf_pos == pos) { s = pf_s; sabs = pf_abs; q = pf_q; }
        else {
            s = lane < nvalid ? S[pos + lane] : 0.0;
            if (whole) { sabs = blk_abs[pos >> 6]; q = blk_q[pos >> 6]; }
        }
        {
            const int64_t np = pos + nvalid;
            pf_pos = np;
            pf_s = np + lane < end ? S[np + lane] : 0.0;
            if (np + 64 <= end) { pf_abs = blk_abs[np >> 6]; pf_q = blk_q[np >> 6]; }
        }
        const bool ispos = lane < nvalid && s > 0;
        const unsigned long long mpos = __ballot(ispos);
        if (!whole) {
            sabs = lane_value(scan_add_d(fabs(s)), 63);
            q = lane_value_i(scan_max_i(quantum_exp(s) + 8192), 63) - 8192;
        }
        const bool cert = mss_certified(cur, sabs, q);
        if (cert || (q < MSS_QBAD && quantum_exp(cur) < MSS_QBAD)) {
            const double pre = cert ? scan_add_d(s) : 0.0;
            double base = cur;
            double V = cert ? base + pre : mss_fold(s, cur, 0, nvalid, lane);
            int p0 = 0;
            for (;;) {
                const bool act = lane >= p0 && lane < nvalid;
                const double Vb = lane_below_d(V, base);
                const bool prevpos = lane > p0 && ((mpos >> (lane - 1)) & 1ull);
                const bool isstart = act && ispos && !prevpos && !(lane == p0 && run_open);
                const bool closes = act && !ispos && (lane == p0 ? run_open : prevpos);
                const unsigned long long mstart = __ballot(isstart), mclose = __ballot(closes);
                const int ms = scan_max_i(isstart ? lane : -1);
                const int msp = lane_below_i(ms, -1);
                const bool carried = closes && msp < p0;
                const double Ls_g = __shfl(Vb, carried || !closes ? 0 : msp);
                const double Ls = carried ? run_L : Ls_g;
                const double R = Vb;
                const double mn = scan_min_d(closes ? Ls : INFINITY);
                const double mnb = lane_below_d(mn, INFINITY);
                const double Lf_before = mnb < Lf ? mnb : Lf;
                const bool cut = closes && Ls <= Lf_before;
                int fl = cut ? 1 : 0;
                double pk = closes ? R : -INFINITY;
                scan_segmax_d(fl, pk);
                const double peak_here = fl ? pk : (pk > peak ? pk : peak);
                const bool trig = act && !ispos && xdrop > 0.0 && peak_here != MSS_NEG && (V + xdrop < peak_here);
                const unsigned long long mt = __ballot(trig);
                const int t = mt ? __builtin_ctzll(mt) : nvalid;
                const unsigned long long upto = t >= 63 ? ~0ull : ((2ull << t) - 1ull);
                const unsigned long long mcl = mclose & upto;
                if (mcl) {
                    const int lastc = 63 - __builtin_clzll(mcl);
                    const int64_t st_pos = carried ? run_st : pos + msp;
                    const unsigned long long mrep = __ballot(cut && lane <= t && (st_pos >> 6) != last_blk);
                    if (mrep) {
                        const int f = __builtin_ctzll(mrep);
                        const int msp_f = lane_value_i(msp, f);
                        const bool car_f = (bool)lane_value_i((int)carried, f);
                        const int64_t st_f = car_f ? run_st : pos + msp_f;
                        const int64_t sl = car_f ? run_slot : slot0 + nruns + __popcll(mstart & ((1ull << msp_f) - 1ull));
                        const double Ls_f = lane_value(Ls, f);
                        file_cut(st_f, sl, Ls_f);
                        ++ncut;
                        last_blk = st_f >> 6;
                    }
                    const double mn_l = lane_value(mn, lastc);
                    Lf = mn_l < Lf ? mn_l : Lf;
                    peak = lane_value(peak_here, lastc);
                    run_open = false;
                }
                if (t < nvalid) {
                    nruns += __popcll(mstart & upto);
                    Lf = INFINITY;
                    peak = MSS_NEG;
                    run_open = false;
                    if (cert) {
                        base = t == 0 ? 0.0 : -lane_value(pre, t - 1);
                        V = base + pre;
                    } else {
                        base = 0.0;
                        V = mss_fold(s, 0.0, t, nvalid, lane);
                    }
                    p0 = t + 1;
                    if (p0 >= nvalid) { cur = lane_value(V, nvalid - 1); break; }
                    continue;
                }
                cur = lane_value(V, nvalid - 1);
                const bool lastpos = (mpos >> (nvalid - 1)) & 1ull;
                if (lastpos) {
                    const int msl = lane_value_i(ms, nvalid - 1);
                    if (msl >= p0) {
                        run_st = pos + msl;
                        run_L = lane_value(Vb, msl);
                        run_slot = slot0 + nruns + __popcll(mstart & ((1ull << msl) - 1ull));
                    }
                    run_open = true;
                }
                nruns += __popcll(mstart);
                break;
            }
        } else {
            for (int i = 0; i < nvalid; ++i) {
                const double v = lane_value(s, i);
                if (v > 0) {
                    if (!run_open) { run_open = true; run_st = pos + i; run_L = cur; run_slot = slot0 + nruns; ++nruns; }
                    cur = cur + v;
                } else {
                    if (run_open) { close_scalar(run_L, cur, run_st, run_slot); run_open = false; }
                    if (xdrop > 0.0 && cur + v + xdrop < peak) { cur = 0.0; peak = MSS_NEG; Lf = INFINITY; }
                    cur += v;
                }
            }
        }
        pos += nvalid;
    }
    if (run_open && k == nunits - 1) { close_scalar(run_L, cur, run_st, run_slot); run_open = false; }
    if (lane == 0) {
        if (k != nunits - 1 && uforced[k + 1] && (Lf != INFINITY || peak != MSS_NEG || run_open))
            atomicOr((unsigned long long *)&grand[2], 1ull);
        mss_light_state x;
        x.L = cur; x.peak = peak; x.Lf = Lf; x.run_L = run_open ? run_L : 0.0;
        x.run_st = run_open ? run_st : 0; x.run_slot = run_open ? run_slot : 0; x.last_blk = last_blk; x.open = run_open ? 1 : 0;
        bool same = pass > 0;
        if (pass > 0) {
            const long long *o = (const long long *)&st_prev[k], *w = (const long long *)&x;
            for (int i = 0; i < 8; ++i) same = same && o[i] == w[i];
        }
        if (!same) atomicOr((unsigned long long *)&grand[1], 1ull);
        st_cur[k] = x;
        cut_cnt[k] = (uint64_t)ncut;
    }
}

__global__ void __launch_bounds__(256) mss_pieces_kernel(const int64_t *__restrict__ ustart, const int64_t *__restrict__ urun,
                                                         const uint8_t *__restrict__ uforced, int64_t nunits,
                                                         const mss_light_state *__restrict__ st, const uint64_t *__restrict__ cut_off,
                                                         const int64_t *__restrict__ cut_st, const int64_t *__restrict__ cut_run,
                                                         const double *__restrict__ cut_L, const int2 *__restrict__ cut_kj, int64_t nblk,
                                                         int64_t cap, int64_t *__restrict__ ustart2, int64_t *__restrict__ urun2,
                                                         double *__restrict__ entry2)
{
    const int64_t i = (int64_t)blockIdx.x * blockDim.x + threadIdx.x;
    if (i < nunits && uforced[i]) {
        const uint64_t at = cut_off[i];
        if ((int64_t)at < cap) { ustart2[at] = ustart[i]; urun2[at] = urun[i]; entry2[at] = i == 0 ? 0.0 : st[i - 1].L; }
    }
    if (i < nblk && cut_st[i] >= 0) {
        const int2 kj = cut_kj[i];
        const uint64_t at = cut_off[kj.x] + (uint64_t)kj.y;
        if ((int64_t)at < cap) { ustart2[at] = cut_st[i]; urun2[at] = cut_run[i]; entry2[at] = cut_L[i]; }
    }
}

__device__ __forceinline__ int64_t mss_lower_bound(const int64_t *a, int64_t n, int64_t x)
{
    int64_t lo = 0, hi = n;
    while (lo < hi) { const int64_t mid = (lo + hi) >> 1; if (a[mid] < x) lo = mid + 1; else hi = mid; }
    return lo;
}
__global__ void __launch_bounds__(256) mss_specvalid_kernel(const int64_t *__restrict__ lstart, const uint8_t *__restrict__ lforced, int64_t nl,
                                                            const int64_t *__restrict__ pstart, int64_t np, uint64_t *__restrict__ valid)
{
    const int64_t j = (int64_t)blockIdx.x * blockDim.x + threadIdx.x;
    if (j > nl) return;
    bool v = j >= 1 && j < nl && !lforced[j];
    if (v) {
        const int64_t at = mss_lower_bound(pstart, np, lstart[j]);
        v = !(at < np && pstart[at] == lstart[j]);
    }
    valid[j] = v ? 1 : 0;
}
__global__ void __launch_bounds__(256) mss_subtable_kernel(const int64_t *__restrict__ lstart, const int64_t *__restrict__ lrun,
                                                           const uint8_t *__restrict__ lforced, int64_t nl, const mss_light_state *__restrict__ lst,
                                                           const uint64_t *__restrict__ vc, const uint64_t *__restrict__ nv_p,
                                                           const int64_t *__restrict__ pstart, const int64_t *__restrict__ prun,
                                                           const double *__restrict__ pentry, int64_t np, int64_t n, mss_subent *__restrict__ subs)
{
    const int64_t i = (int64_t)blockIdx.x * blockDim.x + threadIdx.x;
    const int64_t nv = (int64_t)*nv_p;
    if (i < np) {
        const int64_t jx = mss_lower_bound(lstart, nl + 1, pstart[i]);
        mss_subent e = {};
        e.start = pstart[i]; e.run = prun[i]; e.L = pentry[i]; e.peak = MSS_NEG; e.first = 1; e.vci = -1; e.nst = 0;
        subs[i + (int64_t)vc[jx]] = e;
    }
    if (i >= 1 && i < nl && !lforced[i]) {
        const bool valid = vc[i + 1] != vc[i];
        if (valid) {
            const int64_t pb = mss_lower_bound(pstart, np, lstart[i] + 1);
            const mss_light_state st = lst[i - 1];
            mss_subent e = {};
            e.start = lstart[i]; e.run = lrun[i]; e.L = st.L; e.peak = st.peak; e.run_L = st.run_L; e.run_st = st.run_st;
            e.open = st.open != 0; e.first = 0; e.vci = (int32_t)vc[i]; e.nst = 0; e.Lf = st.Lf;
            subs[pb + (int64_t)vc[i]] = e;
        }
    }
    if (i == 0) {
        mss_subent e = {};
        e.start = n; e.first = 1; e.L = pentry[np]; e.vci = -1;
        subs[np + nv] = e;
    }
}

__global__ void __launch_bounds__(256) mss_compact_kernel(const int32_t *__restrict__ segs, const int64_t *__restrict__ urun,
                                                          const uint64_t *__restrict__ segoff, const uint64_t *__restrict__ segcnt_total,
                                                          int64_t nunits, int32_t *__restrict__ out, const mss_subent *__restrict__ subs)
{
    const int64_t k = (int64_t)blockIdx.x * blockDim.x + threadIdx.x;
    if (k >= nunits) return;
    const int64_t from = subs ? subs[k].run : urun[k];
    const uint64_t to = segoff[k];
    const uint64_t cnt = (k + 1 < nunits ? segoff[k + 1] : *segcnt_total) - to;
    for (uint64_t j = 0; j < cnt; ++j) {
        out[2 * (to + j)] = segs[2 * (from + j)];
        out[2 * (to + j) + 1] = segs[2 * (from + j) + 1];
    }
}

#define MSS_VOTE_LONG 65536
#define MSS_VOTE_CHUNK 16384
__global__ void __launch_bounds__(256) mss_vote_kernel(const int32_t *__restrict__ segs, const uint64_t *__restrict__ nseg_p,
                                                       const int8_t *__restrict__ cls, int nof_labels,
                                                       int8_t *__restrict__ out, unsigned long long *__restrict__ nlong,
                                                       int32_t *__restrict__ longlist, int64_t longcap)
{
    const int lane = threadIdx.x & 63;
    const int64_t nseg = (int64_t)*nseg_p;
    for (int64_t sidx = (int64_t)blockIdx.x * 4 + (threadIdx.x >> 6); sidx < nseg; sidx += (int64_t)gridDim.x * 4) {
        const int64_t st = segs[2 * sidx], en = segs[2 * sidx + 1];
        if (nlong && en - st > MSS_VOTE_LONG) {
            unsigned long long q = 0;
            if (lane == 0) q = atomicAdd(nlong, 1ull);
            q = __shfl(q, 0);
            if ((int64_t)q < longcap) {
                if (lane == 0) longlist[q] = (int32_t)sidx;
                if (lane < DGRP_MAXC) longlist[longcap + DGRP_MAXC * q + lane] = 0;
                continue;
            }
        }
        int best = 1, bv = 0;
        for (int c0 = 0; c0 < nof_labels; c0 += 16) {
            int cnt[16];
#pragma unroll
            for (int c = 0; c < 16; ++c) cnt[c] = 0;
            for (int64_t j = st + lane; j < en; j += 64) {
                const int l = cls[j] - c0;
#pragma unroll
                for (int c = 0; c < 16; ++c) cnt[c] += (l == c);
            }
#pragma unroll
            for (int c = 0; c < 16; ++c) {
                int v = cnt[c];
                for (int o = 32; o > 0; o >>= 1) v += __shfl_xor(v, o);
                if (c0 + c == 1) bv = v;
                else if (c0 + c > 1 && c0 + c < nof_labels && bv < v) { best = c0 + c; bv = v; }
            }
        }
        for (int64_t j = st + lane; j < en; j += 64)
            if (cls[j] == 0) out[j] = (int8_t)best;
    }
}

template <int PHASE>
__global__ void __launch_bounds__(256) mss_vote_long_kernel(const int32_t *__restrict__ segs, const int8_t *__restrict__ cls, int nof_labels,
                                                            int8_t *__restrict__ out, const unsigned long long *__restrict__ nlong,
                                                            int32_t *__restrict__ longlist, int64_t longcap)
{
    const int64_t nq = (int64_t)min((unsigned long long)longcap, *nlong);
    for (int64_t q = 0; q < nq; ++q) {
        const int64_t sidx = longlist[q];
        const int64_t st = segs[2 * sidx], en = segs[2 * sidx + 1];
        int32_t *hist = longlist + longcap + DGRP_MAXC * q;
        int best = 1;
        if (PHASE == 1) {
            int bv = hist[1];
            for (int c = 2; c < nof_labels; ++c)
                if (bv < hist[c]) { best = c; bv = hist[c]; }
        }
        for (int64_t c0 = st + (int64_t)blockIdx.x * MSS_VOTE_CHUNK; c0 < en; c0 += (int64_t)gridDim.x * MSS_VOTE_CHUNK) {
            const int64_t c1 = min(c0 + (int64_t)MSS_VOTE_CHUNK, en);
            if (PHASE == 0) {
                __shared__ int sh[DGRP_MAXC];
                if (threadIdx.x < DGRP_MAXC) sh[threadIdx.x] = 0;
                __syncthreads();
                for (int b0 = 0; b0 < nof_labels; b0 += 16) {
                    int cnt[16];
#pragma unroll
                    for (int c = 0; c < 16; ++c) cnt[c] = 0;
                    for (int64_t j = c0 + threadIdx.x; j < c1; j += 256) {
                        const int l = cls[j] - b0;
#pragma unroll
                        for (int c = 0; c < 16; ++c) cnt[c] += (l == c);
                    }
#pragma unroll
                    for (int c = 0; c < 16; ++c) {
                        int v = cnt[c];
                        for (int o = 32; o > 0; o >>= 1) v += __shfl_xor(v, o);
                        if ((threadIdx.x & 63) == 0 && v && b0 + c >= 1 && b0 + c < DGRP_MAXC) atomicAdd(&sh[b0 + c], v);
                    }
                }
                __syncthreads();
                if (threadIdx.x >= 1 && threadIdx.x < DGRP_MAXC && sh[threadIdx.x]) atomicAdd(&hist[threadIdx.x], sh[threadIdx.x]);
                __syncthreads();
            } else {
                for (int64_t j = c0 + threadIdx.x; j < c1; j += 256)
                    if (cls[j] == 0) out[j] = (int8_t)best;
            }
        }
    }
}

static int mss_vote_all(const mss_layout &l, const int8_t *d_cls, int nof_labels, int8_t *d_labels_out, int64_t n, hipStream_t stream)
{
    const int64_t longcap = n / MSS_VOTE_LONG + 1;
    unsigned long long *nlong = (unsigned long long *)l.grand;
    DGRP_HIP(hipMemsetAsync(nlong, 0, 8, stream));
    hipLaunchKernelGGL(mss_vote_kernel, dim3(1024), dim3(256), 0, stream, l.segs_out, l.grand + 3, d_cls, nof_labels, d_labels_out, nlong,
                       l.segs, longcap);
    DGRP_LAUNCH_CHECK();
    hipLaunchKernelGGL(mss_vote_long_kernel<0>, dim3(1024), dim3(256), 0, stream, l.segs_out, d_cls, nof_labels, d_labels_out, nlong, l.segs,
                       longcap);
    DGRP_LAUNCH_CHECK();
    hipLaunchKernelGGL(mss_vote_long_kernel<1>, dim3(1024), dim3(256), 0, stream, l.segs_out, d_cls, nof_labels, d_labels_out, nlong, l.segs,
                       longcap);
    DGRP_LAUNCH_CHECK();
    return DGRP_OK;
}

DGRP_EXPORT int dgrp_mss_labels(const double *d_scores, const int8_t *d_cls, int64_t n, int nof_labels,
                                int min_mss_len, int xdrop_len, int8_t *d_labels_out, int64_t *d_nseg,
                                void *d_work, int64_t work_bytes, void *stream_)
{
    hipStream_t stream = (hipStream_t)stream_;
    DGRP_REQUIRE(n >= 0 && n < (1ll << 31), "dgrp_mss_labels: n=%lld out of range (the reference indexes with int)", (long long)n);
    DGRP_REQUIRE(nof_labels >= 2 && nof_labels <= DGRP_MAXC, "dgrp_mss_labels: nof_labels must be in 2..64");
    if (n == 0) {
        if (d_nseg) DGRP_HIP(hipMemsetAsync(d_nseg, 0, sizeof(int64_t), stream));
        return DGRP_OK;
    }
    DGRP_REQUIRE(d_scores && d_cls && d_labels_out && d_work, "dgrp_mss_labels: NULL pointer");
    mss_layout l = mss_carve(d_work, n);
    if (work_bytes < l.bytes) {
        dgrp_set_error("dgrp_mss_labels: workspace %lld < %lld bytes", (long long)work_bytes, (long long)l.bytes);
        return DGRP_ENOMEM;
    }
    const double s0 = log(0.99 / (1.0 - 0.99));
    const double xdrop = xdrop_len > 0 ? s0 * xdrop_len * 10.0 : -1;
    const int min_sc = (int)(s0 * min_mss_len);
    const double thr = xdrop > 0.0 ? xdrop + 1.0 : -1.0;

    DGRP_HIP(hipMemsetAsync(l.blk, 0, (l.nblk + 1) * 8, stream));
    hipLaunchKernelGGL(mss_blockstat_kernel, dim3((unsigned)((l.nblk + 3) / 4)), dim3(256), 0, stream, d_scores, n, l.blk,
                       l.blk_sum, l.blk_abs, l.blk_q, l.flags);
    DGRP_LAUNCH_CHECK();
    hipLaunchKernelGGL(mss_superstat_kernel, dim3((unsigned)((l.nsup + 3) / 4)), dim3(256), 0, stream, l.blk_sum, l.blk_abs,
                       l.blk_q, l.flags, l.nblk, l.sup_sum, l.sup_abs, l.sup_q, l.sup_flags);
    DGRP_LAUNCH_CHECK();

    bool single = false;
    for (int attempt = 0; attempt < 2; ++attempt) {
        int64_t nunits = 1;
        DGRP_HIP(hipMemsetAsync(l.grand, 0, 64, stream));
        if (!single && xdrop > 0.0) {
            if (attempt == 0) {
                hipLaunchKernelGGL(mss_boundary_kernel, dim3((unsigned)((l.nblk + 255) / 256)), dim3(256), 0, stream,
                                   l.flags, l.blk_sum, l.nblk, n, thr, l.blk);
                DGRP_LAUNCH_CHECK();
                int rc = device_exclusive_scan(l.blk, l.blk, l.nblk, l.tiles, l.grand, stream);
                if (rc) return rc;
            }
            hipLaunchKernelGGL(mss_units_kernel, dim3((unsigned)((l.nblk + 255) / 256)), dim3(256), 0, stream, l.blk, l.flags,
                               l.blk_sum, l.nblk, n, thr, l.ustart, l.urun, l.grand);
            DGRP_LAUNCH_CHECK();
            uint64_t g = 0;
            DGRP_HIP(hipMemcpyAsync(&g, l.grand, 8, hipMemcpyDeviceToHost, stream));
            DGRP_HIP(hipStreamSynchronize(stream));
            nunits = (int64_t)(g >> 32) + 1;
        } else {
            int64_t h[2] = { 0, n };
            DGRP_HIP(hipMemcpyAsync(l.ustart, h, 16, hipMemcpyHostToDevice, stream));
            int64_t r[2] = { 0, 0 };
            DGRP_HIP(hipMemcpyAsync(l.urun, r, 16, hipMemcpyHostToDevice, stream));
            DGRP_HIP(hipStreamSynchronize(stream));
        }
        DGRP_REQUIRE(nunits < (1ll << 31), "dgrp_mss_labels: too many stretches");
        DGRP_HIP(hipMemsetAsync(l.exitL[0], 0, nunits * 8, stream));
        DGRP_HIP(hipMemsetAsync(l.exitL[1], 0, nunits * 8, stream));
        bool failed = false;
        bool done = false;
        if (!single && !getenv("DGRP_MSS_NO_CUTS")) {
            int64_t nl = 1;
            if (xdrop > 0.0) {
                const char *e = getenv("DGRP_MSS_SUB");
                const int sub = e && atoi(e) > 0 ? atoi(e) : MSS_LIGHT_SUB;
                hipLaunchKernelGGL(mss_lightflag_kernel, dim3((unsigned)((l.nblk + 255) / 256)), dim3(256), 0, stream, l.flags, l.blk_sum,
                                   l.nblk, n, thr, sub, 1, l.lblk);
                DGRP_LAUNCH_CHECK();
                int rc1 = device_exclusive_scan(l.lblk, l.lblk, l.nblk, l.tiles, l.grand + 6, stream);
                if (rc1) return rc1;
                hipLaunchKernelGGL(mss_lightunits_kernel, dim3((unsigned)((l.nblk + 255) / 256)), dim3(256), 0, stream, l.lblk, l.grand + 6,
                                   l.flags, l.blk_sum, l.blk, l.grand, l.nblk, n, thr, sub, 1, l.lstart, l.lrun, l.lforced);
                DGRP_LAUNCH_CHECK();
                uint64_t g6 = 0;
                DGRP_HIP(hipMemcpyAsync(&g6, l.grand + 6, 8, hipMemcpyDeviceToHost, stream));
                DGRP_HIP(hipStreamSynchronize(stream));
                nl = (int64_t)g6 + 1;
            } else {
                const int64_t h[2] = { 0, n }, r[2] = { 0, 0 };
                const uint8_t f[2] = { 1, 1 };
                DGRP_HIP(hipMemcpyAsync(l.lstart, h, 16, hipMemcpyHostToDevice, stream));
                DGRP_HIP(hipMemcpyAsync(l.lrun, r, 16, hipMemcpyHostToDevice, stream));
                DGRP_HIP(hipMemcpyAsync(l.lforced, f, 2, hipMemcpyHostToDevice, stream));
                DGRP_HIP(hipStreamSynchronize(stream));
            }
            int pass = 0;
            for (;; ++pass) {
                DGRP_HIP(hipMemsetAsync(l.grand + 1, 0, 8, stream));
                DGRP_HIP(hipMemsetAsync(l.cut_st, 0xff, l.nblk * 8, stream));
                hipLaunchKernelGGL(mss_light_kernel, dim3((unsigned)nl), dim3(64), 0, stream, d_scores, l.lstart, l.lrun, l.lforced, nl,
                                   (const mss_light_state *)l.lstate[(pass + 1) & 1], (mss_light_state *)l.lstate[pass & 1], xdrop, l.grand,
                                   pass, l.blk_sum, l.blk_abs, l.blk_q, l.flags, l.sup_sum, l.sup_abs, l.sup_q, l.sup_flags, l.cutcnt,
                                   l.cut_st, l.cut_run, l.cut_L, l.cut_kj);
                DGRP_LAUNCH_CHECK();
                uint64_t g[3] = { 0, 0, 0 };
                DGRP_HIP(hipMemcpyAsync(g, l.grand, 24, hipMemcpyDeviceToHost, stream));
                DGRP_HIP(hipStreamSynchronize(stream));
                if (g[2]) { failed = true; break; }
                if (nl == 1 || (pass > 0 && g[1] == 0)) break;
                if (pass > nl + 2) { failed = true; break; }
            }
            if (getenv("DGRP_MSS_TRACE")) fprintf(stderr, "dgrp_mss_labels: n=%lld stretches=%lld light units=%lld passes=%d%s\n", (long long)n,
                                                  (long long)nunits, (long long)nl, pass + 1, failed ? " FAILED" : "");
            if (failed) {
                if (single) { dgrp_set_error("dgrp_mss_labels: sequential scan reported an inconsistent state"); return DGRP_EHIP; }
                single = true;
                continue;
            }
            int rc2 = device_exclusive_scan(l.cutcnt, l.cutcnt, nl, l.tiles, l.grand + 5, stream);
            if (rc2) return rc2;
            const int64_t piece_cap = 2 * l.nblk + 2;
            {
                const int64_t threads = nl > l.nblk ? nl : l.nblk;
                hipLaunchKernelGGL(mss_pieces_kernel, dim3((unsigned)((threads + 255) / 256)), dim3(256), 0, stream, l.lstart, l.lrun, l.lforced,
                                   nl, (const mss_light_state *)l.lstate[pass & 1], l.cutcnt, l.cut_st, l.cut_run, l.cut_L, l.cut_kj, l.nblk,
                                   piece_cap, l.ustart2, l.urun2, l.entry2);
                DGRP_LAUNCH_CHECK();
            }
            uint64_t np = 0;
            DGRP_HIP(hipMemcpyAsync(&np, l.grand + 5, 8, hipMemcpyDeviceToHost, stream));
            DGRP_HIP(hipStreamSynchronize(stream));
            const int64_t npieces = (int64_t)np;
            if (npieces >= 1 && npieces <= piece_cap) {
                DGRP_HIP(hipMemcpyAsync(l.ustart2 + npieces, &n, 8, hipMemcpyHostToDevice, stream));
                DGRP_HIP(hipMemcpyAsync(l.entry2 + npieces, (const mss_light_state *)l.lstate[pass & 1] + (nl - 1), 8, hipMemcpyDeviceToDevice,
                                        stream));
                bool sub_done = false;
                mss_subent *subs = (mss_subent *)l.subs;
                if (nl > 1 && xdrop > 0.0 && !getenv("DGRP_MSS_NO_SUB")) {
                    const char *e = getenv("DGRP_MSS_SUB");
                    const int sub = e && atoi(e) > 0 ? atoi(e) : MSS_LIGHT_SUB;
                    if (sub >= MSS_SUB_MIN) {
                        hipLaunchKernelGGL(mss_specvalid_kernel, dim3((unsigned)((nl + 1 + 255) / 256)), dim3(256), 0, stream, l.lstart, l.lforced,
                                           nl, l.ustart2, npieces, l.lblk);
                        DGRP_LAUNCH_CHECK();
                        int rcv = device_exclusive_scan(l.lblk, l.lblk, nl + 1, l.tiles, l.grand + 7, stream);
                        if (rcv) return rcv;
                        uint64_t nv = 0;
                        DGRP_HIP(hipMemcpyAsync(&nv, l.grand + 7, 8, hipMemcpyDeviceToHost, stream));
                        DGRP_HIP(hipStreamSynchronize(stream));
                        if (nv > 0 && 2 * (int64_t)nv + 2 <= l.dump_cap && npieces + (int64_t)nv <= l.nblk) {
                            const int64_t nsub = npieces + (int64_t)nv;
                            const int64_t threads = (npieces > nl ? npieces : nl) + 1;
                            hipLaunchKernelGGL(mss_subtable_kernel, dim3((unsigned)((threads + 255) / 256)), dim3(256), 0, stream, l.lstart, l.lrun,
                                               l.lforced, nl, (const mss_light_state *)l.lstate[pass & 1], l.lblk, l.grand + 7, l.ustart2,
                                               l.urun2, l.entry2, npieces, n, subs);
                            DGRP_LAUNCH_CHECK();
                            DGRP_HIP(hipMemsetAsync(l.grand + 1, 0, 16, stream));
                            DGRP_HIP(hipMemsetAsync(l.grand + 4, 0, 8, stream));
                            hipLaunchKernelGGL(mss_scan_kernel, dim3((unsigned)nsub), dim3(64), 0, stream, d_scores, l.ustart2, l.urun2, nsub,
                                               l.entry2 + 1, l.exitL[(pass + 1) & 1], l.stack, l.segs, l.segcnt, min_sc, xdrop, l.grand, 1,
                                               l.blk_sum, l.blk_abs, l.blk_q, l.flags, l.sup_sum, l.sup_abs, l.sup_q, l.sup_flags, 1, 0, 1, subs,
                                               l.dump);
                            DGRP_LAUNCH_CHECK();
                            hipLaunchKernelGGL(mss_stitch_kernel, dim3((unsigned)nsub), dim3(64), 0, stream, subs, nsub, l.stack, l.dump, l.segs,
                                               l.segcnt, min_sc, l.grand);
                            DGRP_LAUNCH_CHECK();
                            uint64_t g[5] = { 0, 0, 0, 0, 0 };
                            DGRP_HIP(hipMemcpyAsync(g, l.grand, 40, hipMemcpyDeviceToHost, stream));
                            DGRP_HIP(hipStreamSynchronize(stream));
                            if (getenv("DGRP_MSS_TRACE"))
                                fprintf(stderr, "dgrp_mss_labels: %lld pieces in %lld parts (%llu speculative edges inside pieces)%s (exit %llu, error %llu, why %llu)\n",
                                        (long long)npieces, (long long)nsub, (unsigned long long)nv, g[1] || g[2] ? ": not stitched" : "",
                                        (unsigned long long)g[1], (unsigned long long)g[2], (unsigned long long)g[4]);
                            if (!g[1] && !g[2]) {
                                int rc3 = device_exclusive_scan(l.segcnt, l.segcnt, nsub, l.tiles, l.grand + 3, stream);
                                if (rc3) return rc3;
                                hipLaunchKernelGGL(mss_compact_kernel, dim3((unsigned)((nsub + 255) / 256)), dim3(256), 0, stream, l.segs,
                                                   l.urun2, l.segcnt, l.grand + 3, nsub, l.segs_out, (const mss_subent *)subs);
                                DGRP_LAUNCH_CHECK();
                                done = sub_done = true;
                            }
                        }
                    }
                }
                if (!sub_done) {
                DGRP_HIP(hipMemsetAsync(l.grand + 1, 0, 16, stream));
                hipLaunchKernelGGL(mss_scan_kernel, dim3((unsigned)npieces), dim3(64), 0, stream, d_scores, l.ustart2, l.urun2, npieces,
                                   l.entry2 + 1, l.exitL[(pass + 1) & 1], l.stack, l.segs, l.segcnt, min_sc, xdrop, l.grand, 1, l.blk_sum,
                                   l.blk_abs, l.blk_q, l.flags, l.sup_sum, l.sup_abs, l.sup_q, l.sup_flags, 1, 0, 1, (mss_subent *)nullptr,
                                   (mss_cand *)nullptr);
                DGRP_LAUNCH_CHECK();
                uint64_t g[3] = { 0, 0, 0 };
                DGRP_HIP(hipMemcpyAsync(g, l.grand, 24, hipMemcpyDeviceToHost, stream));
                DGRP_HIP(hipStreamSynchronize(stream));
                if (!g[1] && !g[2]) {
                    int rc3 = device_exclusive_scan(l.segcnt, l.segcnt, npieces, l.tiles, l.grand + 3, stream);
                    if (rc3) return rc3;
                    hipLaunchKernelGGL(mss_compact_kernel, dim3((unsigned)((npieces + 255) / 256)), dim3(256), 0, stream, l.segs, l.urun2,
                                       l.segcnt, l.grand + 3, npieces, l.segs_out, (const mss_subent *)nullptr);
                    DGRP_LAUNCH_CHECK();
                    done = true;
                }
                }
            }
            if (done) break;
            DGRP_HIP(hipMemsetAsync(l.exitL[0], 0, nunits * 8, stream));
            DGRP_HIP(hipMemsetAsync(l.exitL[1], 0, nunits * 8, stream));
            DGRP_HIP(hipMemsetAsync(l.grand + 1, 0, 16, stream));
        }
        for (int pass = 0;; ++pass) {
            DGRP_HIP(hipMemsetAsync(l.grand + 1, 0, 8, stream));
            hipLaunchKernelGGL(mss_scan_kernel, dim3((unsigned)nunits), dim3(64), 0, stream, d_scores, l.ustart, l.urun,
                               nunits, l.exitL[(pass + 1) & 1], l.exitL[pass & 1], l.stack, l.segs, l.segcnt, min_sc, xdrop,
                               l.grand, pass, l.blk_sum, l.blk_abs, l.blk_q, l.flags, l.sup_sum, l.sup_abs, l.sup_q,
                               l.sup_flags, 1, 0, 0, (mss_subent *)nullptr, (mss_cand *)nullptr);
            DGRP_LAUNCH_CHECK();
            uint64_t g[3] = { 0, 0, 0 };
            DGRP_HIP(hipMemcpyAsync(g, l.grand, 24, hipMemcpyDeviceToHost, stream));
            DGRP_HIP(hipStreamSynchronize(stream));
            if (g[2]) { failed = true; break; }
            if (nunits == 1 || (pass > 0 && g[1] == 0)) break;
            if (pass > nunits + 2) { failed = true; break; }
        }
        if (failed) {
            if (single) { dgrp_set_error("dgrp_mss_labels: sequential scan reported an inconsistent state"); return DGRP_EHIP; }
            single = true;
            continue;
        }
        int rc = device_exclusive_scan(l.segcnt, l.segcnt, nunits, l.tiles, l.grand + 3, stream);
        if (rc) return rc;
        hipLaunchKernelGGL(mss_compact_kernel, dim3((unsigned)((nunits + 255) / 256)), dim3(256), 0, stream, l.segs, l.urun,
                           l.segcnt, l.grand + 3, nunits, l.segs_out, (const mss_subent *)nullptr);
        DGRP_LAUNCH_CHECK();
        break;
    }
    DGRP_HIP(hipMemcpyAsync(d_labels_out, d_cls, n, hipMemcpyDeviceToDevice, stream));
    {
        const int rcv = mss_vote_all(l, d_cls, nof_labels, d_labels_out, n, stream);
        if (rcv) return rcv;
    }
    if (d_nseg) DGRP_HIP(hipMemcpyAsync(d_nseg, l.grand + 3, 8, hipMemcpyDeviceToDevice, stream));
    return DGRP_OK;
}

DGRP_EXPORT int dgrp_mss_segments_host(const void *d_work, int64_t work_bytes, int32_t *h_st_en, int64_t cap, int64_t *n_seg)
{
    DGRP_REQUIRE(d_work && n_seg, "dgrp_mss_segments_host: NULL pointer");
    int64_t lo = 0, hi = (1ll << 31) - 1;
    while (lo < hi) {
        int64_t mid = lo + (hi - lo + 1) / 2;
        if (mss_carve(nullptr, mid).bytes <= work_bytes) lo = mid; else hi = mid - 1;
    }
    mss_layout l = mss_carve((void *)d_work, lo);
    uint64_t cnt = 0;
    DGRP_HIP(hipDeviceSynchronize());
    DGRP_HIP(hipMemcpy(&cnt, l.grand + 3, 8, hipMemcpyDeviceToHost));
    *n_seg = (int64_t)cnt;
    const int64_t take = (int64_t)cnt < cap ? (int64_t)cnt : cap;
    if (take > 0 && h_st_en) DGRP_HIP(hipMemcpy(h_st_en, l.segs_out, take * 8, hipMemcpyDeviceToHost));
    return DGRP_OK;
}

DGRP_EXPORT int64_t dgrp_mss_batch_workspace_bytes(int64_t total_n, int64_t nrec)
{
    if (total_n < 0 || nrec < 0) return 0;
    return mss_carve(nullptr, total_n + 4 * nrec + 64).bytes;
}

DGRP_EXPORT int dgrp_mss_labels_batch(const double *d_scores, const int8_t *d_cls, int64_t total_n, int64_t nrec,
                                      const int64_t *h_start, int nof_labels, int min_mss_len, int xdrop_len,
                                      int8_t *d_labels_out, void *d_work, int64_t work_bytes, void *stream_)
{
    hipStream_t stream = (hipStream_t)stream_;
    DGRP_REQUIRE(total_n >= 0 && total_n < (1ll << 31) && nrec >= 0 && (nrec == 0 || h_start), "dgrp_mss_labels_batch: bad arguments");
    DGRP_REQUIRE(nof_labels >= 2 && nof_labels <= DGRP_MAXC, "dgrp_mss_labels_batch: nof_labels must be in 2..64");
    if (nrec == 0 || total_n == 0) return DGRP_OK;
    DGRP_REQUIRE(d_scores && d_cls && d_labels_out && d_work, "dgrp_mss_labels_batch: NULL pointer");
    DGRP_REQUIRE(h_start[0] == 0 && h_start[nrec] == total_n, "dgrp_mss_labels_batch: starts must run from 0 to total_n");
    for (int64_t r = 0; r < nrec; ++r)
        DGRP_REQUIRE((h_start[r] & 63) == 0 && h_start[r + 1] > h_start[r], "dgrp_mss_labels_batch: record %lld: starts must be increasing multiples of 64", (long long)r);
    mss_layout l = mss_carve(d_work, total_n + 4 * nrec + 64);
    if (work_bytes < l.bytes) {
        dgrp_set_error("dgrp_mss_labels_batch: workspace %lld < %lld bytes", (long long)work_bytes, (long long)l.bytes);
        return DGRP_ENOMEM;
    }
    l.nblk = (total_n + 63) / 64;
    l.nsup = (l.nblk + 63) / 64;
    const double s0 = log(0.99 / (1.0 - 0.99));
    const double xdrop = xdrop_len > 0 ? s0 * xdrop_len * 10.0 : -1;
    const int min_sc = (int)(s0 * min_mss_len);
    hipLaunchKernelGGL(mss_blockstat_kernel, dim3((unsigned)((l.nblk + 3) / 4)), dim3(256), 0, stream, d_scores, total_n, l.blk,
                       l.blk_sum, l.blk_abs, l.blk_q, l.flags);
    hipLaunchKernelGGL(mss_superstat_kernel, dim3((unsigned)((l.nsup + 3) / 4)), dim3(256), 0, stream, l.blk_sum, l.blk_abs,
                       l.blk_q, l.flags, l.nblk, l.sup_sum, l.sup_abs, l.sup_q, l.sup_flags);
    DGRP_LAUNCH_CHECK();
    std::vector<int64_t> urun((size_t)nrec + 1);
    for (int64_t r = 0; r <= nrec; ++r) urun[(size_t)r] = h_start[r] / 2 + 2 * r;
    DGRP_HIP(hipMemcpyAsync(l.ustart, h_start, (size_t)(nrec + 1) * 8, hipMemcpyHostToDevice, stream));
    DGRP_HIP(hipMemcpyAsync(l.urun, urun.data(), (size_t)(nrec + 1) * 8, hipMemcpyHostToDevice, stream));
    DGRP_HIP(hipMemsetAsync(l.grand, 0, 64, stream));
    hipLaunchKernelGGL(mss_scan_kernel, dim3((unsigned)nrec), dim3(64), 0, stream, d_scores, l.ustart, l.urun, nrec, l.exitL[1],
                       l.exitL[0], l.stack, l.segs, l.segcnt, min_sc, xdrop, l.grand, 0, l.blk_sum, l.blk_abs, l.blk_q, l.flags,
                       l.sup_sum, l.sup_abs, l.sup_q, l.sup_flags, 1, 1, 0, (mss_subent *)nullptr, (mss_cand *)nullptr);
    DGRP_LAUNCH_CHECK();
    int rc = device_exclusive_scan(l.segcnt, l.segcnt, nrec, l.tiles, l.grand + 3, stream);
    if (rc) return rc;
    hipLaunchKernelGGL(mss_compact_kernel, dim3((unsigned)((nrec + 255) / 256)), dim3(256), 0, stream, l.segs, l.urun, l.segcnt,
                       l.grand + 3, nrec, l.segs_out, (const mss_subent *)nullptr);
    DGRP_LAUNCH_CHECK();
    DGRP_HIP(hipMemcpyAsync(d_labels_out, d_cls, total_n, hipMemcpyDeviceToDevice, stream));
    hipLaunchKernelGGL(mss_vote_kernel, dim3(1024), dim3(256), 0, stream, l.segs_out, l.grand + 3, d_cls, nof_labels, d_labels_out,
                       (unsigned long long *)nullptr, (int32_t *)nullptr, (int64_t)0);
    DGRP_LAUNCH_CHECK();
    DGRP_HIP(hipStreamSynchronize(stream));
    return DGRP_OK;
}
```

### deepgrp_amd/csrc/post_kernels.hip

```cpp
#include "dgrp_common.h"
#include "scan.h"
#include <vector>

#include <math.h>

__device__ __forceinline__ float np_logf(float xin)
{
    const uint32_t bits = __float_as_uint(xin);
    float k = (float)((int)(bits >> 23) - 126);
    float m = __uint_as_float((bits & 0x007fffffu) | 0x3f000000u);
    if (m <= 0.70710678118654752440f) { m = m + m; k = k - 1.0f; }
    const float x = m - 1.0f;
    float den = fmaf(5.875095403124574342950e-03f, x, 1.546476374983906719538e-01f);
    den = fmaf(den, x, 9.864942958519418960339e-01f);
    den = fmaf(den, x, 2.453006071784736363091e+00f);
    den = fmaf(den, x, 2.612677543073109236779e+00f);
    den = fmaf(den, x, 1.0f);
    float num = fmaf(2.589979117907922693523e-02f, x, 3.808837741388407920751e-01f);
    num = fmaf(num, x, 1.480000633576506585156e+00f);
    num = fmaf(num, x, 2.112677543073053063722e+00f);
    num = fmaf(num, x, 9.999999999999998702752e-01f);
    num = fmaf(num, x, 0.0f);
    return fmaf(k, 0.693147180559945309417232121458176568f, __fdiv_rn(num, den));
}

__device__ __forceinline__ float np_expf(float x)
{
    if (x != x) return x;
    if (x >= 88.72283905206835f) return INFINITY;
    if (x <= -103.97208404541015625f) return 0.0f;
    const float q = rintf(x * 1.44269504088896340736f);
    float r = fmaf(q, -6.93145752e-1f, x);
    r = fmaf(q, -1.42860677e-6f, r);
    float num = fmaf(5.082762527590693718096e-04f, r, 6.757896990527504603057e-03f);
    num = fmaf(num, r, 5.114512081637298353406e-02f);
    num = fmaf(num, r, 2.473615434895520810817e-01f);
    num = fmaf(num, r, 7.257664613233124478488e-01f);
    num = fmaf(num, r, 9.999999999980870924916e-01f);
    float den = fmaf(2.159509375685829852307e-02f, r, -2.742335390411667452936e-01f);
    den = fmaf(den, r, 1.0f);
    return ldexpf(__fdiv_rn(num, den), (int)q);
}

__global__ void __launch_bounds__(256) scores_kernel(const float *__restrict__ probs, int64_t n, int C,
                                                     double *__restrict__ scores, int8_t *__restrict__ cls)
{
    const int64_t nthreads = (int64_t)gridDim.x * blockDim.x;
    for (int64_t i = (int64_t)blockIdx.x * blockDim.x + threadIdx.x; i < n; i += nthreads) {
        const float *p = probs + i * C;
        int a = 0;
        float mx = p[0];
        for (int c = 1; c < C; ++c) {
            const float v = p[c];
            if (v > mx) { mx = v; a = c; }
        }
        float m = mx + 1e-6f;
        if (m > 0.99f) m = 0.99f;
        const float t = np_logf(__fdiv_rn(m, 1.0f - m));
        const float sc = a > 0 ? t : -10.0f * t;
        scores[i] = (double)sc;
        cls[i] = (int8_t)a;
    }
}

DGRP_EXPORT int dgrp_scores(const float *d_probs, int64_t n, int C, double *d_scores, int8_t *d_cls, void *stream)
{
    DGRP_REQUIRE(n >= 0 && C >= 1 && C <= DGRP_MAXC, "dgrp_scores: bad n/C");
    if (n == 0) return DGRP_OK;
    DGRP_REQUIRE(d_probs && d_scores && d_cls, "dgrp_scores: NULL pointer");
    hipLaunchKernelGGL(scores_kernel, dim3(grid_for(n, 256, 256 * 16)), dim3(256), 0, (hipStream_t)stream, d_probs, n,
                       C, d_scores, d_cls);
    DGRP_LAUNCH_CHECK();
    return DGRP_OK;
}

__global__ void __launch_bounds__(256) blockmax_kernel(const float *__restrict__ a, int64_t total, float *__restrict__ part)
{
    __shared__ float red[4];
    const int64_t nthreads = (int64_t)gridDim.x * blockDim.x;
    float m = -INFINITY;
    for (int64_t i = (int64_t)blockIdx.x * blockDim.x + threadIdx.x; i < total; i += nthreads) m = fmaxf(m, a[i]);
    for (int o = 32; o > 0; o >>= 1) m = fmaxf(m, __shfl_xor(m, o));
    if ((threadIdx.x & 63) == 0) red[threadIdx.x >> 6] = m;
    __syncthreads();
    if (threadIdx.x == 0) part[blockIdx.x] = fmaxf(fmaxf(red[0], red[1]), fmaxf(red[2], red[3]));
}

__global__ void __launch_bounds__(256) softmax_labels_kernel(const float *__restrict__ a, int64_t n, int C,
                                                             const float *__restrict__ part, int nparts,
                                                             float *__restrict__ sm, int8_t *__restrict__ labels)
{
    float gmax = -INFINITY;
    for (int i = 0; i < nparts; ++i) gmax = fmaxf(gmax, part[i]);
    const int64_t nthreads = (int64_t)gridDim.x * blockDim.x;
    for (int64_t i = (int64_t)blockIdx.x * blockDim.x + threadIdx.x; i < n; i += nthreads) {
        const float *row = a + i * C;
        float sum;
        if (C < 8) {
            sum = np_expf(row[0] - gmax);
            for (int c = 1; c < C; ++c) sum = sum + np_expf(row[c] - gmax);
        } else {
            float r[8];
#pragma unroll
            for (int k = 0; k < 8; ++k) r[k] = np_expf(row[k] - gmax);
            const int whole = C - C % 8;
            int c = 8;
            for (; c < whole; c += 8) {
#pragma unroll
                for (int k = 0; k < 8; ++k) r[k] = r[k] + np_expf(row[c + k] - gmax);
            }
            sum = ((r[0] + r[1]) + (r[2] + r[3])) + ((r[4] + r[5]) + (r[6] + r[7]));
            for (; c < C; ++c) sum = sum + np_expf(row[c] - gmax);
        }
        int best = 0;
        float bv = __fdiv_rn(np_expf(a[i * C] - gmax), sum);
        if (sm) sm[i * C] = bv;
        for (int c = 1; c < C; ++c) {
            const float v = __fdiv_rn(np_expf(a[i * C + c] - gmax), sum);
            if (sm) sm[i * C + c] = v;
            if (v > bv) { bv = v; best = c; }
        }
        labels[i] = (int8_t)best;
    }
}

DGRP_EXPORT int dgrp_softmax_labels(const float *d_probs, int64_t n, int C, float *d_softmax, int8_t *d_labels,
                                    void *d_work, int64_t work_bytes, void *stream)
{
    DGRP_REQUIRE(n >= 0 && C >= 1 && C <= DGRP_MAXC, "dgrp_softmax_labels: bad n/C");
    if (n == 0) return DGRP_OK;
    const int nparts = 1024;
    DGRP_REQUIRE(d_probs && d_labels && d_work && work_bytes >= (int64_t)(nparts * sizeof(float)),
                 "dgrp_softmax_labels: need %d bytes of workspace", (int)(nparts * sizeof(float)));
    float *part = (float *)d_work;
    hipLaunchKernelGGL(blockmax_kernel, dim3(nparts), dim3(256), 0, (hipStream_t)stream, d_probs, n * C, part);
    DGRP_LAUNCH_CHECK();
    hipLaunchKernelGGL(softmax_labels_kernel, dim3(grid_for(n, 256, 256 * 16)), dim3(256), 0, (hipStream_t)stream,
                       d_probs, n, C, part, nparts, d_softmax, d_labels);
    DGRP_LAUNCH_CHECK();
    return DGRP_OK;
}

__device__ __forceinline__ bool seg_is_start(const int8_t *lab, int64_t i, int64_t n)
{
    const int8_t v = lab[i];
    return v != 0 && (i == 0 || i == n - 1 || lab[i - 1] != v);
}
__device__ __forceinline__ bool seg_is_end(const int8_t *lab, int64_t i, int64_t n)
{
    const int8_t v = lab[i];
    return v != 0 && (i >= n - 2 || lab[i + 1] != v);
}

__device__ __forceinline__ uint64_t seg_flags_batch(const int8_t *lab, const uint8_t *marks, int64_t i)
{
    const uint8_t m = marks[i];
    const int8_t v = lab[i];
    if ((m & 8) || v == 0) return 0;
    const bool st = (m & 1) || (m & 2) || lab[i - 1] != v;
    const bool en = (m & 2) || (m & 4) || lab[i + 1] != v;
    return ((uint64_t)st << 32) + (uint64_t)en;
}

template <bool BATCH>
__device__ __forceinline__ uint64_t seg_flags(const int8_t *lab, const uint8_t *marks, int64_t i, int64_t n)
{
    if (BATCH) return seg_flags_batch(lab, marks, i);
    return ((uint64_t)seg_is_start(lab, i, n) << 32) + (uint64_t)seg_is_end(lab, i, n);
}

struct seg_records {
    const int64_t *start;
    const int64_t *startpos;
    const int32_t *contig;
    int64_t nrec;
};

template <bool BATCH>
__global__ void __launch_bounds__(256) seg_count_kernel(const int8_t *__restrict__ lab, const uint8_t *__restrict__ marks, int64_t n,
                                                        uint64_t *__restrict__ tilecnt)
{
    __shared__ uint64_t lds[4];
    const int64_t base = (int64_t)blockIdx.x * SCAN_TILE;
    uint64_t c = 0;
    for (int j = 0; j < 8; ++j) {
        const int64_t i = base + j * 256 + threadIdx.x;
        if (i < n) c += seg_flags<BATCH>(lab, marks, i, n);
    }
    for (int o = 32; o > 0; o >>= 1) c += __shfl_xor(c, o);
    if ((threadIdx.x & 63) == 0) lds[threadIdx.x >> 6] = c;
    __syncthreads();
    if (threadIdx.x == 0) tilecnt[blockIdx.x] = lds[0] + lds[1] + lds[2] + lds[3];
}

template <bool BATCH>
__global__ void __launch_bounds__(256) seg_emit_kernel(const int8_t *__restrict__ lab, const uint8_t *__restrict__ marks, int64_t n,
                                                       int64_t offset, int32_t contig, seg_records recs,
                                                       const uint64_t *__restrict__ tileoff, dgrp_segment *__restrict__ rec, int64_t cap)
{
    __shared__ uint64_t lds[4];
    const int64_t base = (int64_t)blockIdx.x * SCAN_TILE + (int64_t)threadIdx.x * 8;
    uint64_t f[8], s = 0;
    for (int j = 0; j < 8; ++j) {
        const int64_t i = base + j;
        f[j] = i < n ? seg_flags<BATCH>(lab, marks, i, n) : 0;
        s += f[j];
    }
    uint64_t ex = block_exclusive_scan(s, nullptr, lds) + tileoff[blockIdx.x];
    for (int j = 0; j < 8; ++j) {
        const int64_t i = base + j;
        if (f[j]) {
            int64_t off = offset;
            int32_t tag = contig;
            if (BATCH) {
                int64_t lo = 0, hi = recs.nrec;
                while (hi - lo > 1) {
                    const int64_t mid = (lo + hi) >> 1;
                    if (recs.start[mid] <= i) lo = mid; else hi = mid;
                }
                off = recs.startpos[lo] - recs.start[lo];
                tag = recs.contig[lo];
            }
            if (f[j] >> 32) {
                const int64_t k = (int64_t)(ex >> 32);
                if (k < cap) { rec[k].start = i + off; rec[k].label = lab[i]; rec[k].contig = tag; }
            }
            if (f[j] & 1) {
                const int64_t k = (int64_t)(ex & 0xffffffffull);
                if (k < cap) rec[k].end = i + 1 + off;
            }
        }
        ex += f[j];
    }
}

__global__ void seg_total_kernel(const uint64_t *__restrict__ grand, int64_t *__restrict__ count)
{
    *count = (int64_t)(*grand >> 32);
}

__global__ void __launch_bounds__(64) rec_marks_kernel(const int64_t *__restrict__ start, const int64_t *__restrict__ len,
                                                       int64_t nrec, uint8_t *__restrict__ marks, double *__restrict__ scores,
                                                       int8_t *__restrict__ cls)
{
    const int64_t r = blockIdx.x;
    if (r >= nrec) return;
    const int64_t a = start[r], n = len[r], b = start[r + 1];
    if (threadIdx.x == 0) {
        uint8_t m0 = 1;
        if (n == 1) m0 |= 2;
        if (n == 2) m0 |= 4;
        marks[a] = m0;
        if (n >= 2) marks[a + n - 1] = (uint8_t)(2 | (n == 1 ? 1 : 0));
        if (n >= 3) marks[a + n - 2] = 4;
    }
    for (int64_t i = a + n + threadIdx.x; i < b; i += 64) {
        marks[i] = 8;
        if (scores) scores[i] = 0.0;
        if (cls) cls[i] = 0;
    }
}

int dgrp_batch_marks(const int64_t *d_start, const int64_t *d_len, int64_t nrec, int64_t total_n, uint8_t *d_marks,
                     double *d_scores, int8_t *d_cls, hipStream_t stream)
{
    DGRP_HIP(hipMemsetAsync(d_marks, 0, (size_t)total_n, stream));
    hipLaunchKernelGGL(rec_marks_kernel, dim3((unsigned)nrec), dim3(64), 0, stream, d_start, d_len, nrec, d_marks, d_scores, d_cls);
    DGRP_LAUNCH_CHECK();
    return DGRP_OK;
}

int dgrp_batch_segments(const int8_t *d_labels, const uint8_t *d_marks, int64_t total_n, const int64_t *d_start, int64_t nrec,
                        const int64_t *d_startpos, const int32_t *d_contig, dgrp_segment *d_records, int64_t cap,
                        int64_t *d_count, void *d_work, int64_t work_bytes, hipStream_t stream)
{
    if (work_bytes < dgrp_segments_workspace_bytes(total_n)) {
        dgrp_set_error("dgrp_batch_segments: workspace too small");
        return DGRP_ENOMEM;
    }
    const int64_t ntiles = (total_n + SCAN_TILE - 1) / SCAN_TILE;
    uint64_t *tiles = (uint64_t *)d_work;
    uint64_t *grand = tiles + ntiles + 1;
    hipLaunchKernelGGL(seg_count_kernel<true>, dim3((unsigned)ntiles), dim3(256), 0, stream, d_labels, d_marks, total_n, tiles);
    hipLaunchKernelGGL(scan_sums_kernel, dim3(1), dim3(256), 0, stream, tiles, ntiles, grand);
    hipLaunchKernelGGL(seg_emit_kernel<true>, dim3((unsigned)ntiles), dim3(256), 0, stream, d_labels, d_marks, total_n, (int64_t)0,
                       (int32_t)0, seg_records{ d_start, d_startpos, d_contig, nrec }, tiles, d_records, cap);
    hipLaunchKernelGGL(seg_total_kernel, dim3(1), dim3(1), 0, stream, grand, d_count);
    DGRP_LAUNCH_CHECK();
    return DGRP_OK;
}

DGRP_EXPORT int64_t dgrp_segments_workspace_bytes(int64_t n)
{
    if (n < 0) return 0;
    return dgrp_align_up(((n + SCAN_TILE - 1) / SCAN_TILE + 2) * 8, 256) + 256;
}

DGRP_EXPORT int dgrp_segments(const int8_t *d_labels, int64_t n, int64_t offset, int32_t contig, dgrp_segment *d_records,
                              int64_t cap, int64_t *d_count, void *d_work, int64_t work_bytes, void *stream_)
{
    hipStream_t stream = (hipStream_t)stream_;
    DGRP_REQUIRE(n >= 0 && n < (1ll << 31) && cap >= 0 && d_count, "dgrp_segments: bad arguments");
    if (n == 0) {
        DGRP_HIP(hipMemsetAsync(d_count, 0, sizeof(int64_t), stream));
        return DGRP_OK;
    }
    DGRP_REQUIRE(d_labels && d_work && (cap == 0 || d_records), "dgrp_segments: NULL pointer");
    if (work_bytes < dgrp_segments_workspace_bytes(n)) {
        dgrp_set_error("dgrp_segments: workspace too small");
        return DGRP_ENOMEM;
    }
    const int64_t ntiles = (n + SCAN_TILE - 1) / SCAN_TILE;
    uint64_t *tiles = (uint64_t *)d_work;
    uint64_t *grand = tiles + ntiles + 1;
    hipLaunchKernelGGL(seg_count_kernel<false>, dim3((unsigned)ntiles), dim3(256), 0, stream, d_labels, (const uint8_t *)nullptr, n, tiles);
    DGRP_LAUNCH_CHECK();
    hipLaunchKernelGGL(scan_sums_kernel, dim3(1), dim3(256), 0, stream, tiles, ntiles, grand);
    DGRP_LAUNCH_CHECK();
    hipLaunchKernelGGL(seg_emit_kernel<false>, dim3((unsigned)ntiles), dim3(256), 0, stream, d_labels, (const uint8_t *)nullptr, n, offset,
                       contig, seg_records{ nullptr, nullptr, nullptr, 0 }, tiles, d_records, cap);
    DGRP_LAUNCH_CHECK();
    hipLaunchKernelGGL(seg_total_kernel, dim3(1), dim3(1), 0, stream, grand, d_count);
    DGRP_LAUNCH_CHECK();
    return DGRP_OK;
}
```

### include/deepgrp_hip.h

```cpp
#ifndef DEEPGRP_HIP_H_
#define DEEPGRP_HIP_H_

#include <stddef.h>
#include <stdint.h>

#ifdef __cplusplus
extern "C" {
#endif

#define DGRP_OK 0
#define DGRP_EINVAL (-1)
#define DGRP_EHIP (-2)
#define DGRP_ENOMEM (-3)
#define DGRP_ENODEV (-4)

#define DGRP_ABI_VERSION 1

typedef struct dgrp_segment {
    int64_t start;
    int64_t end;
    int32_t label;
    int32_t contig;
} dgrp_segment;

typedef struct dgrp_model dgrp_model;

int dgrp_abi_version(void);
const char *dgrp_last_error(void);
int dgrp_device_info(char *name, size_t name_cap, int *cu_count, int64_t *hbm_bytes);

int dgrp_strip_n(const uint8_t *h_seq, int64_t len, int64_t *startpos, int64_t *kept);
int dgrp_encode(const uint8_t *d_seq, int64_t n, uint8_t *d_idx, void *stream);
int dgrp_onehot(const uint8_t *d_seq, int64_t n, int8_t *d_onehot, void *stream);

int64_t dgrp_fasta_workspace_bytes(int64_t nbytes);
int dgrp_fasta_encode(const uint8_t *d_raw, int64_t nbytes, uint8_t *d_idx, int64_t *h_info, void *d_work,
                      int64_t work_bytes, void *stream);

int64_t dgrp_fasta_batch_workspace_bytes(int64_t nrec, int64_t total_bytes);
int dgrp_fasta_encode_batch(const uint8_t *d_raw, int64_t nrec, const int64_t *h_off, const int64_t *h_len,
                            uint8_t *d_idx, int64_t *h_info, void *d_work, int64_t work_bytes, void *stream);

int64_t dgrp_fasta_chunks_workspace_bytes(int64_t cap);
int dgrp_fasta_chunks(const uint8_t *d_raw, int64_t nbytes, int64_t cap, int64_t *h_start, int64_t *h_first_lf,
                      int64_t *n_chunks, void *d_work, int64_t work_bytes, void *stream);

int64_t dgrp_fasta_mask_workspace_bytes(int64_t nrec, int64_t total_bytes, int64_t nrows);
int dgrp_fasta_mask_batch(const uint8_t *d_raw, int64_t nrec, const int64_t *h_off, const int64_t *h_len,
                          const dgrp_segment *d_rows, const int64_t *h_row_off, int mode, uint64_t class_mask,
                          uint8_t *d_out, void *d_work, int64_t work_bytes, void *stream);

int64_t dgrp_twobit_workspace_bytes(int64_t nrec);
int dgrp_twobit_encode_batch(const uint8_t *d_file, int64_t file_bytes, int64_t nrec, const int64_t *h_packed_off,
                             const int64_t *h_dna_size, const int64_t *d_n_iv, const int64_t *h_n_iv_off, int64_t n_iv,
                             const int64_t *h_out_off, uint8_t *d_idx, int64_t idx_cap, void *d_work, int64_t work_bytes,
                             void *stream);
int dgrp_twobit_text_batch(const uint8_t *d_file, int64_t file_bytes, int64_t nrec, const int64_t *h_name_off,
                           const int64_t *h_name_len, const int64_t *h_packed_off, const int64_t *h_dna_size,
                           const int64_t *d_n_iv, const int64_t *h_n_iv_off, int64_t n_iv, const int64_t *d_m_iv,
                           const int64_t *h_m_iv_off, int64_t m_iv, const int64_t *h_text_off, uint8_t *d_text,
                           int64_t text_cap, void *d_work, int64_t work_bytes, void *stream);

int64_t dgrp_twobit_pack_workspace_bytes(int64_t nrec, int64_t total_bytes);
int dgrp_twobit_pack_batch(const uint8_t *d_raw, int64_t nrec, const int64_t *h_off, const int64_t *h_len, uint8_t *d_out,
                           int64_t out_off, int64_t out_cap, int64_t *h_counts, int64_t *h_blob_off, void *d_work,
                           int64_t work_bytes, void *stream);

typedef struct dgrp_extract_entry {
    int64_t text_off;
    int64_t base_off;
    int64_t bases;
} dgrp_extract_entry;
int64_t dgrp_fasta_extract_workspace_bytes(int64_t nrec, int64_t total_bytes, int64_t nrows);
int dgrp_fasta_extract_batch(const uint8_t *d_raw, int64_t nrec, const int64_t *h_off, const int64_t *h_len,
                             const dgrp_segment *d_rows, const int64_t *h_row_off, const uint8_t *d_names,
                             const int64_t *h_name_off, int64_t flank, int width, uint64_t class_mask, uint8_t *d_text,
                             int64_t text_cap, int64_t *h_text_bytes, dgrp_extract_entry *d_entries, int64_t *h_kept,
                             void *d_work, int64_t work_bytes, void *stream);

int64_t dgrp_repeat_summary_workspace_bytes(int64_t nrec, int64_t total_bytes, int64_t nrows);
int dgrp_repeat_summary_batch(const uint8_t *d_raw, int64_t nrec, const int64_t *h_off, const int64_t *h_len,
                              const dgrp_segment *d_rows, const int64_t *h_row_off, int C, int64_t bin, const int64_t *h_bin_off,
                              int64_t *d_counts, int64_t *d_bins, int64_t *d_bad, void *d_work, int64_t work_bytes, void *stream);

int64_t dgrp_window_count(int64_t n, int64_t T, int64_t s);
int dgrp_windows_onehot(const uint8_t *d_idx, int64_t n, int64_t T, int64_t s, int64_t w0,
                        int64_t nw, int elem, void *d_out, void *stream);

int dgrp_model_create(dgrp_model **out, int T, int u, int C, int attention, const float *h_kernel,
                      const float *h_recurrent, const float *h_bias, const float *h_scale,
                      const float *h_ff_kernel, const float *h_ff_bias);
int dgrp_model_create_lstm(dgrp_model **out, int T, int u, int C, const float *h_kernel,
                           const float *h_recurrent, const float *h_bias, const float *h_ff_kernel,
                           const float *h_ff_bias);
int dgrp_model_destroy(dgrp_model *m);
int dgrp_model_dims(const dgrp_model *m, int *T, int *u, int *C, int *attention);
int dgrp_model_flags(const dgrp_model *m);
int dgrp_model_set_precision(dgrp_model *m, int level);
int dgrp_model_view(const dgrp_model *m, int level, dgrp_model **out);

#define DGRP_KERNEL_NONE 0
#define DGRP_KERNEL_WAVE 1
#define DGRP_KERNEL_SPLIT2 2
#define DGRP_KERNEL_STREAM64 3
#define DGRP_KERNEL_STREAM 4
#define DGRP_KERNEL_SPLIT 5
#define DGRP_KERNEL_LSTM 6
#define DGRP_KERNEL_FUSED 7
#define DGRP_KERNEL_FP32 8
int dgrp_model_plan(const dgrp_model *m, int mode, int64_t step, int *kernel, int64_t *lds_bytes, int *ospan, int *avg_up);

int64_t dgrp_forward_workspace_bytes(const dgrp_model *m, int64_t nw);
int64_t dgrp_forward_window_chunk(const dgrp_model *m);
int dgrp_forward_windows(const dgrp_model *m, const uint8_t *d_idx, int64_t n, int64_t s,
                         int64_t w0, int64_t nw, float *d_probs, void *d_work, int64_t work_bytes,
                         void *stream);

int dgrp_forward_merge(const dgrp_model *m, const uint8_t *d_idx, int64_t n, int64_t s,
                       int64_t batch, int64_t w0, int64_t nw, float *d_out, void *d_work,
                       int64_t work_bytes, void *stream);

int64_t dgrp_forward_merge_record_workspace_bytes(const dgrp_model *m, int64_t n, int64_t s);
int dgrp_forward_merge_record(const dgrp_model *m, const uint8_t *d_idx, int64_t n, int64_t s, int64_t batch, float *d_out,
                              void *d_work, int64_t work_bytes, void *stream);

int64_t dgrp_forward_reference_workspace_bytes(const dgrp_model *m, int64_t nw);
int dgrp_forward_windows_reference(const dgrp_model *m, const uint8_t *d_idx, int64_t n, int64_t s, int64_t w0,
                                   int64_t nw, float *d_probs, void *d_work, int64_t work_bytes, void *stream);

int dgrp_get_max(float *d_output, int64_t out_rows, const float *d_inputs, int64_t dim0,
                 int64_t dim1, int64_t stride, int64_t batchsize, void *stream);

int dgrp_scores(const float *d_probs, int64_t n, int C, double *d_scores, int8_t *d_cls,
                void *stream);
int dgrp_softmax_labels(const float *d_probs, int64_t n, int C, float *d_softmax, int8_t *d_labels,
                        void *d_work, int64_t work_bytes, void *stream);

int64_t dgrp_mss_workspace_bytes(int64_t n);
int dgrp_mss_labels(const double *d_scores, const int8_t *d_cls, int64_t n, int nof_labels,
                    int min_mss_len, int xdrop_len, int8_t *d_labels_out, int64_t *d_nseg,
                    void *d_work, int64_t work_bytes, void *stream);
int dgrp_mss_segments_host(const void *d_work, int64_t work_bytes, int32_t *h_st_en, int64_t cap,
                           int64_t *n_seg);

int64_t dgrp_mss_batch_workspace_bytes(int64_t total_n, int64_t nrec);
int dgrp_mss_labels_batch(const double *d_scores, const int8_t *d_cls, int64_t total_n, int64_t nrec,
                          const int64_t *h_start, int nof_labels, int min_mss_len, int xdrop_len,
                          int8_t *d_labels_out, void *d_work, int64_t work_bytes, void *stream);

int64_t dgrp_segments_workspace_bytes(int64_t n);
int dgrp_segments(const int8_t *d_labels, int64_t n, int64_t offset, int32_t contig,
                  dgrp_segment *d_records, int64_t cap, int64_t *d_count, void *d_work,
                  int64_t work_bytes, void *stream);

int64_t dgrp_format_rows_bound(int64_t nrows, int64_t longest_prefix);
int dgrp_format_rows(const char *prefixes, const int64_t *prefix_off, int64_t nprefix, int by_contig,
                     const dgrp_segment *rows, int64_t nrows, char *out, int64_t cap, int64_t *written);

#define DGRP_TRACK_NAME_ROOM 65536
int64_t dgrp_track_workspace_bytes(int64_t n, int64_t bin);
int dgrp_track_text(const float *d_probs, int64_t n, int C, int cls, int digits, int64_t bin, int64_t offset,
                    const char *name, int64_t name_len, char *d_text, int64_t cap, int64_t *h_bytes,
                    void *d_work, int64_t work_bytes, void *stream);

int64_t dgrp_track_batch_workspace_bytes(int64_t nrec, const int64_t *h_n, const int64_t *h_startpos, int64_t bin, int ncls,
                                         int64_t names_bytes);
int dgrp_track_text_batch(const float *d_probs, int C, int64_t nrec, const int64_t *h_row0, const int64_t *h_n,
                          const int64_t *h_startpos, const char *names, const int64_t *h_name_off, const int *h_cls, int ncls,
                          int digits, int64_t bin, char *d_text, int64_t cap, int64_t *h_class_off, void *d_work,
                          int64_t work_bytes, void *stream);

typedef struct { int64_t beg, end; int32_t rec; uint32_t bin; } dgrp_track_chunk;
int64_t dgrp_track_index_workspace_bytes(int64_t nrec, const int64_t *h_n, const int64_t *h_startpos, int64_t bin, int ncls,
                                         int64_t names_bytes);
int dgrp_track_index_batch(const float *d_probs, int C, int64_t nrec, const int64_t *h_row0, const int64_t *h_n,
                           const int64_t *h_startpos, const char *names, const int64_t *h_name_off, const int *h_cls, int ncls,
                           int digits, int64_t bin, dgrp_track_chunk *d_chunks, int64_t chunk_cap, int64_t *h_chunk_off,
                           int64_t *d_linear, int64_t linear_cap, void *d_work, int64_t work_bytes, void *stream);

typedef struct { int64_t off, bytes; int32_t rec; uint32_t start, end, pad; } dgrp_track_section;
int64_t dgrp_track_sections_workspace_bytes(int64_t nrec, const int64_t *h_n, const int64_t *h_startpos, int64_t bin, int ncls);
int dgrp_track_sections_batch(const float *d_probs, int C, int64_t nrec, const int64_t *h_row0, const int64_t *h_n,
                              const int64_t *h_startpos, const int *h_cls, int ncls, int digits, int64_t bin, int64_t chrom0, char *d_out,
                              int64_t cap, int64_t *h_class_off, dgrp_track_section *d_table, int64_t table_cap, int64_t *h_section_off,
                              void *d_work, int64_t work_bytes, void *stream);

#define DGRP_TRACK_ZOOM_LEVELS 10
typedef struct { int64_t off, bytes; int32_t cls, level, rec0, rec1; uint32_t start, end; } dgrp_track_zoom_block;
typedef struct { uint64_t covered, qmin, qmax, sum, sumsq; } dgrp_track_totals;
int64_t dgrp_track_zoom_workspace_bytes(int64_t nrec, const int64_t *h_n, const int64_t *h_startpos, int64_t bin, int ncls);
int dgrp_track_zoom_batch(const float *d_probs, int C, int64_t nrec, const int64_t *h_row0, const int64_t *h_n,
                          const int64_t *h_startpos, const int *h_cls, int ncls, int digits, int64_t bin, int64_t chrom0, char *d_out,
                          int64_t cap, int64_t *h_record_off, dgrp_track_zoom_block *d_table, int64_t table_cap, int64_t *h_block_off,
                          dgrp_track_totals *h_totals, void *d_work, int64_t work_bytes, void *stream);

int64_t dgrp_zlib_bound(int64_t nblk, int64_t in_bytes);
int64_t dgrp_zlib_workspace_bytes(int64_t nblk, int level);
int dgrp_zlib_compress_batch(const uint8_t *d_in, int64_t in_bytes, const void *d_rows, int64_t stride, int64_t nblk, int level,
                             uint8_t *d_out, int64_t out_cap, int64_t *d_sizes, int64_t *h_out_bytes, void *d_work, int64_t work_bytes,
                             void *stream);
int dgrp_zlib_compress_host(const uint8_t *h_in, int64_t in_bytes, const void *h_rows, int64_t stride, int64_t nblk, int level,
                            uint8_t *h_out, int64_t out_cap, int64_t *h_sizes, int64_t *h_out_bytes);

int64_t dgrp_record_workspace_bytes(const dgrp_model *m, int64_t n, int64_t s, int use_mss);
int dgrp_predict_record(const dgrp_model *m, const uint8_t *d_idx, int64_t n, int64_t s, int64_t batch,
                        int min_mss_len, int xdrop_len, int use_mss, int64_t offset, int32_t contig,
                        dgrp_segment *d_records, int64_t cap, int64_t *h_count, void *d_work, int64_t work_bytes,
                        void *stream);

int64_t dgrp_batch_workspace_bytes(const dgrp_model *m, int64_t nrec, const int64_t *h_n, int64_t s);
int dgrp_predict_batch(const dgrp_model *m, const uint8_t *d_idx, int64_t nrec, const int64_t *h_idx_off,
                       const int64_t *h_n, const int64_t *h_startpos, const int32_t *h_contig, int64_t s, int64_t batch,
                       int min_mss_len, int xdrop_len, dgrp_segment *d_records, int64_t cap, int64_t *h_count,
                       void *d_work, int64_t work_bytes, void *stream);

int64_t dgrp_batch_rows(int64_t nrec, const int64_t *h_n);
int dgrp_predict_batch_probs(const dgrp_model *m, const uint8_t *d_idx, int64_t nrec, const int64_t *h_idx_off,
                             const int64_t *h_n, const int64_t *h_startpos, const int32_t *h_contig, int64_t s, int64_t batch,
                             int min_mss_len, int xdrop_len, dgrp_segment *d_records, int64_t cap, int64_t *h_count,
                             void *d_work, int64_t work_bytes, void *stream, float *d_probs);

int dgrp_confusion_matrix(const int8_t *d_true, const int8_t *d_pred, int64_t n, int ncls, int64_t *d_cnf,
                          int *d_bad, void *stream);
int dgrp_filter_segments(const int8_t *d_labels, int8_t *d_out, int64_t n, int64_t min_len, void *stream);

int64_t dgrp_eval_workspace_bytes(int64_t nrec, int64_t nrows);
int dgrp_paint_rows_batch(int8_t *d_labels, int64_t nrec, const int64_t *h_off, const int64_t *h_len, const int64_t *h_origin,
                          const dgrp_segment *d_rows, const int64_t *h_row_off, void *d_work, int64_t work_bytes, void *stream);
int dgrp_row_hits_batch(const int8_t *d_labels, int64_t nrec, const int64_t *h_off, const int64_t *h_len, const int64_t *h_origin,
                        const dgrp_segment *d_rows, const int64_t *h_row_off, int64_t *d_hits, void *d_work, int64_t work_bytes,
                        void *stream);

typedef struct { uint64_t sum; int64_t bases; int64_t agree; uint32_t qmin; uint32_t pad; } dgrp_row_score;
int64_t dgrp_row_scores_workspace_bytes(int64_t nrec, int64_t nrows);
int dgrp_row_scores_batch(const float *d_probs, int C, int64_t nrec, const int64_t *h_row0, const int64_t *h_n,
                          const int64_t *h_startpos, const dgrp_segment *d_rows, const int64_t *h_row_off,
                          dgrp_row_score *d_scores, void *d_work, int64_t work_bytes, void *stream);

int64_t dgrp_prob_hist_workspace_bytes(int64_t nrec, int C, int bins);
int dgrp_prob_hist_batch(const float *d_probs, int C, int64_t nrec, const int64_t *h_row0, const int64_t *h_n,
                         const int8_t *d_truth, const int64_t *h_off, int bins, int64_t *d_hist, int *d_bad,
                         void *d_work, int64_t work_bytes, void *stream);

int64_t dgrp_row_detect_workspace_bytes(int64_t nrec, int64_t nrows);
int dgrp_paint_row_keys_batch(uint16_t *d_keys, int64_t nrec, const int64_t *h_off, const int64_t *h_len, const int64_t *h_origin,
                              const dgrp_segment *d_pred, const int64_t *h_pred_off, const dgrp_row_score *d_scores, void *d_work,
                              int64_t work_bytes, void *stream);
int dgrp_row_detect_batch(const uint16_t *d_keys, int64_t nrec, const int64_t *h_off, const int64_t *h_len, const int64_t *h_origin,
                          const dgrp_segment *d_true, const int64_t *h_true_off, const int64_t *d_need, int32_t *d_detect,
                          void *d_work, int64_t work_bytes, void *stream);

int64_t dgrp_format_bed_bound(int64_t nrows, int64_t longest_name);
int dgrp_format_bed_rows(const char *names, const int64_t *name_off, int64_t nnames, int by_contig,
                         const dgrp_segment *rows, const dgrp_row_score *scores, int64_t nrows, int min_score,
                         char *out, int64_t cap, int64_t *written);

int64_t dgrp_bed_text_workspace_bytes(int64_t nrows, int64_t nnames, int64_t names_bytes);
int dgrp_bed_text_batch(const char *names, const int64_t *name_off, int64_t nnames, int by_contig, const dgrp_segment *d_rows,
                        const dgrp_row_score *d_scores, int64_t nrows, int min_score, char *d_text, int64_t cap, int64_t *h_bytes,
                        void *d_work, int64_t work_bytes, void *stream);

int64_t dgrp_bed_index_workspace_bytes(int64_t nrows, int64_t nnames, int64_t names_bytes, int64_t nrec);
int dgrp_bed_index_batch(const char *names, const int64_t *name_off, int64_t nnames, int by_contig, const dgrp_segment *d_rows,
                         const dgrp_row_score *d_scores, int64_t nrows, int min_score, int64_t nrec, const int64_t *h_rec_end,
                         dgrp_track_chunk *d_chunks, int64_t chunk_cap, int64_t *h_nchunks, int64_t *d_linear, int64_t linear_cap,
                         int64_t *d_rec_last, void *d_work, int64_t work_bytes, void *stream);

int64_t dgrp_gff_text_workspace_bytes(int64_t nrows, int64_t nnames, int64_t names_bytes, int64_t ncnames, int64_t cnames_bytes);
int dgrp_gff_text_batch(const char *names, const int64_t *name_off, int64_t nnames, int by_contig, const char *cnames,
                        const int64_t *cname_off, int64_t ncnames, const dgrp_segment *d_rows, const dgrp_row_score *d_scores,
                        int64_t nrows, int min_score, int64_t id0, char *d_text, int64_t cap, int64_t *h_bytes, int64_t *h_lines,
                        void *d_work, int64_t work_bytes, void *stream);
int64_t dgrp_gff_index_workspace_bytes(int64_t nrows, int64_t nnames, int64_t names_bytes, int64_t ncnames, int64_t cnames_bytes,
                                       int64_t nrec);
int dgrp_gff_index_batch(const char *names, const int64_t *name_off, int64_t nnames, int by_contig, const char *cnames,
                         const int64_t *cname_off, int64_t ncnames, const dgrp_segment *d_rows, const dgrp_row_score *d_scores,
                         int64_t nrows, int min_score, int64_t id0, int64_t nrec, const int64_t *h_rec_end,
                         dgrp_track_chunk *d_chunks, int64_t chunk_cap, int64_t *h_nchunks, int64_t *d_linear, int64_t linear_cap,
                         int64_t *d_rec_last, void *d_work, int64_t work_bytes, void *stream);

typedef struct { int64_t off, bytes; int32_t rec; uint32_t start, end, items; } dgrp_bed_block;
int64_t dgrp_bed_blocks_workspace_bytes(int64_t nrows, int64_t nrec, const int64_t *h_rec_end);
int dgrp_bed_blocks_batch(int by_contig, const dgrp_segment *d_rows, const dgrp_row_score *d_scores, int64_t nrows, int min_score,
                          int64_t nrec, const int64_t *h_rec_end, int64_t chrom0, char *d_out, int64_t cap, int64_t *h_bytes,
                          dgrp_bed_block *d_table, int64_t table_cap, int64_t *h_nblocks, int64_t *h_items, void *d_work,
                          int64_t work_bytes, void *stream);
int64_t dgrp_bed_zoom_workspace_bytes(int64_t nrows, int64_t nrec, const int64_t *h_rec_end);
int dgrp_bed_zoom_batch(int by_contig, const dgrp_segment *d_rows, const dgrp_row_score *d_scores, int64_t nrows, int min_score,
                        int64_t nrec, const int64_t *h_rec_end, int64_t chrom0, char *d_out, int64_t cap, int64_t *h_record_off,
                        dgrp_track_zoom_block *d_table, int64_t table_cap, int64_t *h_block_off, dgrp_track_totals *h_totals,
                        void *d_work, int64_t work_bytes, void *stream);

#define DGRP_EDATA (-5)
#define DGRP_INFLATE_OK 0
#define DGRP_INFLATE_EINPUT 1
#define DGRP_INFLATE_EBLOCK 2
#define DGRP_INFLATE_ESTORED 3
#define DGRP_INFLATE_ECODES 4
#define DGRP_INFLATE_ESYMBOL 5
#define DGRP_INFLATE_EDIST 6
#define DGRP_INFLATE_EOUTPUT 7
#define DGRP_INFLATE_ECRC 8
#define DGRP_INFLATE_EISIZE 9
#define DGRP_INFLATE_ETRAIL 10

int dgrp_inflate_raw_host(const uint8_t *h_in, int64_t in_len, uint8_t *h_out, int64_t out_cap, int64_t *h_out_len,
                          int64_t *h_in_used, int *h_reason);

int64_t dgrp_inflate_workspace_bytes(int64_t nmem);
int dgrp_inflate_batch(const uint8_t *d_in, int64_t in_bytes, int64_t nmem, const int64_t *h_in_off, const int64_t *h_in_len,
                       const int64_t *h_out_off, uint8_t *d_out, int64_t out_bytes, int64_t *h_bad, int *h_reason, void *d_work,
                       int64_t work_bytes, void *stream);

#define DGRP_INFLATE_ESPAN 11
#define DGRP_INFLATE_EROUNDS 12
typedef struct dgrp_inflate_stream_stats {
    int64_t spans;
    int64_t candidates;
    int64_t repaired;
    int64_t rounds;
    int64_t longest_span;
    int64_t false_starts;
    int64_t chunks;
    int64_t reserved;
} dgrp_inflate_stream_stats;

int dgrp_inflate_stream_host(const uint8_t *h_in, int64_t in_len, int64_t chunk_bytes, int64_t max_span_bytes, int max_rounds,
                             uint8_t *h_out, int64_t out_cap, int64_t *h_out_len, int64_t *h_in_used,
                             dgrp_inflate_stream_stats *h_stats, int *h_reason);

int64_t dgrp_inflate_stream_workspace_bytes(int64_t in_bytes, int64_t chunk_bytes);
int dgrp_inflate_stream_scan(const uint8_t *d_in, int64_t in_bytes, int64_t data_off, int64_t chunk_bytes, int64_t max_span_bytes,
                             int max_rounds, int64_t *h_total, dgrp_inflate_stream_stats *h_stats, int *h_reason, void *d_work,
                             int64_t work_bytes, void *stream);
int dgrp_inflate_stream_write(const uint8_t *d_in, int64_t in_bytes, int64_t data_off, int64_t chunk_bytes, uint16_t *d_sym,
                              uint8_t *d_out, int64_t out_bytes, uint32_t *h_crc, int64_t *h_in_used, int *h_reason, void *d_work,
                              int64_t work_bytes, void *stream);

int64_t dgrp_bgzf_bound(int64_t n, int eof);
int64_t dgrp_bgzf_workspace_bytes(int64_t n);
int dgrp_bgzf_compress(const uint8_t *d_in, int64_t n, uint8_t *d_out, int64_t out_cap, int64_t *h_out_bytes, int eof, void *d_work,
                       int64_t work_bytes, void *stream);
int dgrp_bgzf_compress_host(const uint8_t *h_in, int64_t n, uint8_t *h_out, int64_t out_cap, int64_t *h_out_bytes, int eof);

int64_t dgrp_bgzf_workspace_bytes_level(int64_t n, int level);
int dgrp_bgzf_compress_level(const uint8_t *d_in, int64_t n, uint8_t *d_out, int64_t out_cap, int64_t *h_out_bytes, int eof, int level,
                             void *d_work, int64_t work_bytes, void *stream);
int dgrp_bgzf_compress_host_level(const uint8_t *h_in, int64_t n, uint8_t *h_out, int64_t out_cap, int64_t *h_out_bytes, int eof,
                                  int level);

int64_t dgrp_train_param_count(int u, int C, int attention);
int64_t dgrp_train_workspace_bytes(int T, int u, int C, int attention, int64_t B);
int dgrp_train_step(int T, int u, int C, int attention, const float *d_params, const uint8_t *d_idx, const int8_t *d_truth,
                    int64_t n, const int64_t *d_starts, int64_t B, const float *d_masks, float *d_loss, float *d_grads,
                    void *d_work, int64_t work_bytes, void *stream);

#define DGRP_TRAIN_MAX_JOBS 8
typedef struct dgrp_train_job {
    int T, u, C, attention;
    const float *d_params;
    const uint8_t *d_idx;
    const int8_t *d_truth;
    int64_t n;
    const int64_t *d_starts;
    int64_t B;
    const float *d_masks;
    float *d_loss, *d_grads;
    void *d_work;
    int64_t work_bytes;
} dgrp_train_job;
int dgrp_train_step_multi(const dgrp_train_job *h_jobs, int K, void *stream);

#define DGRP_OPT_RMSPROP 0
#define DGRP_OPT_ADAM 1
int dgrp_optimizer_step(int kind, float *d_params, const float *d_grads, float *d_state1, float *d_state2, int64_t count,
                        double learning_rate, double rho, double momentum, double epsilon, int64_t step, void *stream);

int64_t dgrp_truth_workspace_bytes(int64_t nrec, int64_t nrows);
int dgrp_truth_multihot_batch(int8_t *d_truth, int C, int64_t n_total, int64_t nrec, const int64_t *h_off, const int64_t *h_len,
                              const int64_t *h_origin, const dgrp_segment *d_rows, const int64_t *h_row_off, void *d_work,
                              int64_t work_bytes, void *stream);

int64_t dgrp_class_starts_workspace_bytes(int64_t nrec, int64_t n_total);
int dgrp_class_window_starts(const int8_t *d_row, int64_t n_total, int64_t nrec, const int64_t *h_off, const int64_t *h_len, int T,
                             int64_t *d_starts, int64_t cap, int64_t *h_count, void *d_work, int64_t work_bytes, void *stream);

int dgrp_train_resolve_starts(const int64_t *d_picks, int64_t B, const int64_t *const *d_set_ptr, const int64_t *d_set_size,
                              int nsets, const int64_t *d_base, const int64_t *d_wprefix, int64_t nrec, int64_t *d_starts,
                              void *stream);

int dgrp_kernel_timer_enable(int on);
int dgrp_kernel_timer_read(double *h_ms, int64_t *h_launches, int64_t *h_windows);

#ifdef __cplusplus
}
#endif
#endif
```

Before: 573.2.

## Fuse score computation with MSS block stats and skip unchanged light-unit rewalks

Adds a scores_blockstat kernel that computes per-position scores and the per-64-block MSS statistics in one pass, so the separate blockstat kernel and its memset disappear from the record path. The light-pass MSS kernel now remembers its entry state and returns early when that state is unchanged between passes. It also carries cuts that begin before the unit, removes the per-pass cut_st memset, and defers the units count readback into a later combined sync. This adds complexity in the cross-pass bookkeeping, with a risk to correctness if the early-exit state comparison misses a dependency.

```diff
diff --git a/deepgrp_amd/_lib.py b/deepgrp_amd/_lib.py
--- a/deepgrp_amd/_lib.py
+++ b/deepgrp_amd/_lib.py
@@ -97,6 +97,10 @@
     "dgrp_mss_workspace_bytes": (i64, [i64]),
     "dgrp_mss_labels": (cint, [vp, vp, i64, cint, cint, cint, vp, vp, vp, i64, vp]),
     "dgrp_mss_segments_host": (cint, [vp, i64, vp, i64, C.POINTER(i64)]),
+    "dgrp_scores_mss_labels": (cint, [vp, i64, cint, vp, vp, cint, cint, vp, vp, vp, i64, vp]),
+    "dgrp_scores_blockstats": (cint, [vp, i64, cint, vp, vp, vp, i64, vp]),
+    "dgrp_mss_blockstats": (cint, [vp, i64, vp, i64, vp]),
+    "dgrp_mss_blockstats_fetch": (cint, [vp, i64, i64, vp, vp, vp, vp, vp, vp]),
     "dgrp_mss_batch_workspace_bytes": (i64, [i64, i64]),
     "dgrp_mss_labels_batch": (cint, [vp, vp, i64, i64, vp, cint, cint, cint, vp, vp, i64, vp]),
     "dgrp_segments_workspace_bytes": (i64, [i64]),
diff --git a/deepgrp_amd/csrc/api.hip b/deepgrp_amd/csrc/api.hip
--- a/deepgrp_amd/csrc/api.hip
+++ b/deepgrp_amd/csrc/api.hip
@@ -871,10 +871,8 @@
     int rc = dgrp_forward_merge_record(m, d_idx, n, s, batch, out, w + l.fwd, l.fwd_bytes, stream);
     if (rc) return rc;
     if (use_mss) {
-        rc = dgrp_scores(out, n, m->C, (double *)(w + l.scores), (int8_t *)(w + l.cls), stream);
-        if (rc) return rc;
-        rc = dgrp_mss_labels((const double *)(w + l.scores), (const int8_t *)(w + l.cls), n, m->C, min_mss_len, xdrop_len,
-                             labels, nullptr, w + l.post, l.post_bytes, stream);
+        rc = dgrp_scores_mss_labels(out, n, m->C, (double *)(w + l.scores), (int8_t *)(w + l.cls), min_mss_len, xdrop_len, labels, nullptr,
+                                    w + l.post, l.post_bytes, stream);
     } else {
         rc = dgrp_softmax_labels(out, n, m->C, nullptr, labels, w + l.post, l.post_bytes, stream);
     }
diff --git a/deepgrp_amd/csrc/mss_kernels.hip b/deepgrp_amd/csrc/mss_kernels.hip
--- a/deepgrp_amd/csrc/mss_kernels.hip
+++ b/deepgrp_amd/csrc/mss_kernels.hip
@@ -1,5 +1,6 @@
 #include "dgrp_common.h"
 #include "scan.h"
+#include "mss_stats.h"
 #include <vector>
 #include <math.h>
 
@@ -19,8 +20,6 @@
 static_assert(sizeof(mss_subent) == 80, "MSS_SUBENT_BYTES");
 #define MSS_LCAP 160
 #define MSS_NEG (-1e30)
-#define MSS_QNONE (-4096)
-#define MSS_QBAD 4096
 
 struct mss_layout {
     int64_t nblk;
@@ -44,6 +43,8 @@
     int64_t *lstart, *lrun;
     uint8_t *lforced;
     void *lstate[2];
+    void *lentry;
+    void *ccut;
     int64_t *cut_st, *cut_run;
     double *cut_L;
     int2 *cut_kj;
@@ -89,6 +90,8 @@
     l.lforced = (uint8_t *)take(maxunits + 64);
     l.lstate[0] = take(maxunits * 64);
     l.lstate[1] = take(maxunits * 64);
+    l.lentry = take(maxunits * 64);
+    l.ccut = take(maxunits * 32);
     l.cut_st = (int64_t *)take(l.nblk * 8);
     l.cut_run = (int64_t *)take(l.nblk * 8);
     l.cut_L = (double *)take(l.nblk * 8);
@@ -112,17 +115,6 @@
     return mss_carve(nullptr, n).bytes;
 }
 
-__device__ __forceinline__ int quantum_exp(double x)
-{
-    const uint64_t b = (uint64_t)__double_as_longlong(x) & 0x7fffffffffffffffull;
-    if (b == 0) return MSS_QNONE;
-    const int e = (int)(b >> 52);
-    if (e == 0 || e == 0x7ff) return MSS_QBAD;
-    const uint64_t m = b & 0x000fffffffffffffull;
-    const int tz = m ? __builtin_ctzll(m) : 52;
-    return -((e - 1023) - 52 + tz);
-}
-
 __device__ __forceinline__ bool mss_certified(double L, double sumabs, int q_scores)
 {
     const int qL = quantum_exp(L);
@@ -134,19 +126,6 @@
     return (fabs(L) + sumabs) * 1.0000001 < ldexp(1.0, ex);
 }
 
-__device__ __forceinline__ double wave_sum(double v)
-{
-#pragma unroll
-    for (int o = 32; o > 0; o >>= 1) v += __shfl_xor(v, o);
-    return v;
-}
-__device__ __forceinline__ int wave_max(int v)
-{
-#pragma unroll
-    for (int o = 32; o > 0; o >>= 1) { int w = __shfl_xor(v, o); v = w > v ? w : v; }
-    return v;
-}
-
 __device__ __forceinline__ double lane_value(double x, int l)
 {
     const long long b = __double_as_longlong(x);
@@ -166,17 +145,7 @@
     const double s = i < n ? S[i] : 0.0;
     const bool pos = i < n && s > 0;
     const bool prevpos = i > 0 && i < n && S[i - 1] > 0;
-    const unsigned long long mpos = __ballot(pos);
-    const unsigned long long mstart = __ballot(pos && !prevpos);
-    const double sum = wave_sum(s), sabs = wave_sum(fabs(s));
-    const int q = wave_max(quantum_exp(s));
-    if (lane == 0) {
-        flags[b] = (uint8_t)(mpos != 0ull ? 1 : 0);
-        blk[b] = (uint64_t)__popcll(mstart);
-        blk_sum[b] = sum;
-        blk_abs[b] = sabs;
-        blk_q[b] = q;
-    }
+    mss_block_stats(s, pos, prevpos, lane, b, blk, blk_sum, blk_abs, blk_q, flags);
 }
 
 __global__ void __launch_bounds__(256) mss_superstat_kernel(const double *__restrict__ blk_sum, const double *__restrict__ blk_abs,
@@ -723,6 +692,9 @@
     int64_t run_st, run_slot;
     int64_t last_blk, open;
 };
+static_assert(sizeof(mss_light_state) == 64, "mss_carve: lstate, lentry");
+struct mss_carried_cut { int64_t st, run; double L; int64_t j; };
+static_assert(sizeof(mss_carried_cut) == 32, "mss_carve: ccut");
 
 __global__ void __launch_bounds__(256) mss_lightflag_kernel(const uint8_t *__restrict__ flags, const double *__restrict__ blk_sum,
                                                             int64_t nblk, int64_t n, double thr, int sub, int use_forced,
@@ -770,27 +742,44 @@
                                                        const int32_t *__restrict__ sup_q, const uint8_t *__restrict__ sup_flags,
                                                        uint64_t *__restrict__ cut_cnt, int64_t *__restrict__ cut_st,
                                                        int64_t *__restrict__ cut_run, double *__restrict__ cut_L,
-                                                       int2 *__restrict__ cut_kj)
+                                                       int2 *__restrict__ cut_kj, mss_light_state *__restrict__ entry_used,
+                                                       mss_carried_cut *__restrict__ ccut, int rewalk_all)
 {
     const int lane = threadIdx.x;
     const int64_t k = blockIdx.x;
     const int64_t begin = ustart[k], end = ustart[k + 1];
     const int64_t slot0 = urun[k];
     const bool forced = uforced[k] != 0;
-    double cur = 0.0, peak = MSS_NEG, Lf = INFINITY, run_L = 0.0;
-    bool run_open = false;
-    int64_t run_st = 0, run_slot = 0;
-    int64_t last_blk = begin >> 6;
+    mss_light_state e;
+    e.L = 0.0; e.peak = MSS_NEG; e.Lf = INFINITY; e.run_L = 0.0; e.run_st = 0; e.run_slot = 0; e.last_blk = begin >> 6; e.open = 0;
     if (k > 0 && pass > 0) {
-        const mss_light_state e = st_prev[k - 1];
-        cur = e.L; peak = e.peak; Lf = e.Lf; run_L = e.run_L;
-        run_st = e.run_st; run_slot = e.run_slot; run_open = e.open != 0;
-        if (!forced) last_blk = e.last_blk;
-    }
+        e = st_prev[k - 1];
+        if (forced) e.last_blk = begin >> 6;
+    }
+    if (pass > 0 && !rewalk_all) {
+        const long long *o = (const long long *)&entry_used[k], *w = (const long long *)&e;
+        bool same = true;
+        for (int i = 0; i < 8; ++i) same = same && o[i] == w[i];
+        if (same) {
+            if (lane == 0) st_cur[k] = st_prev[k];
+            return;
+        }
+    }
+    if (lane == 0) entry_used[k] = e;
+    for (int64_t b = (begin >> 6) + lane; b < ((end + 63) >> 6); b += 64) cut_st[b] = -1;
+    __threadfence_block();
+    double cur = e.L, peak = e.peak, Lf = e.Lf, run_L = e.run_L;
+    bool run_open = e.open != 0;
+    int64_t run_st = e.run_st, run_slot = e.run_slot;
+    int64_t last_blk = e.last_blk;
     int64_t nruns = 0;
     int64_t ncut = forced ? 1 : 0;
+    mss_carried_cut cc;
+    cc.st = -1; cc.run = 0; cc.L = 0.0; cc.j = 0;
     auto file_cut = [&](int64_t st, int64_t slot, double Ls) {
-        if (lane == 0) {
+        if (st < begin) {
+            cc.st = st; cc.run = slot; cc.L = Ls; cc.j = ncut;
+        } else if (lane == 0) {
             const int64_t b = st >> 6;
             cut_st[b] = st; cut_run[b] = slot; cut_L[b] = Ls; cut_kj[b] = make_int2((int)k, (int)ncut);
         }
@@ -974,6 +963,7 @@
         if (!same) atomicOr((unsigned long long *)&grand[1], 1ull);
         st_cur[k] = x;
         cut_cnt[k] = (uint64_t)ncut;
+        ccut[k] = cc;
     }
 }
 
@@ -981,14 +971,20 @@
                                                          const uint8_t *__restrict__ uforced, int64_t nunits,
                                                          const mss_light_state *__restrict__ st, const uint64_t *__restrict__ cut_off,
                                                          const int64_t *__restrict__ cut_st, const int64_t *__restrict__ cut_run,
-                                                         const double *__restrict__ cut_L, const int2 *__restrict__ cut_kj, int64_t nblk,
-                                                         int64_t cap, int64_t *__restrict__ ustart2, int64_t *__restrict__ urun2,
+                                                         const double *__restrict__ cut_L, const int2 *__restrict__ cut_kj,
+                                                         const mss_carried_cut *__restrict__ ccut, int64_t nblk, int64_t cap,
+                                                         int64_t *__restrict__ ustart2, int64_t *__restrict__ urun2,
                                                          double *__restrict__ entry2)
 {
     const int64_t i = (int64_t)blockIdx.x * blockDim.x + threadIdx.x;
     if (i < nunits && uforced[i]) {
         const uint64_t at = cut_off[i];
         if ((int64_t)at < cap) { ustart2[at] = ustart[i]; urun2[at] = urun[i]; entry2[at] = i == 0 ? 0.0 : st[i - 1].L; }
+    }
+    if (i < nunits && ccut[i].st >= 0) {
+        const mss_carried_cut c = ccut[i];
+        const uint64_t at = cut_off[i] + (uint64_t)c.j;
+        if ((int64_t)at < cap) { ustart2[at] = c.st; urun2[at] = c.run; entry2[at] = c.L; }
     }
     if (i < nblk && cut_st[i] >= 0) {
         const int2 kj = cut_kj[i];
@@ -1172,11 +1168,9 @@
     return DGRP_OK;
 }
 
-DGRP_EXPORT int dgrp_mss_labels(const double *d_scores, const int8_t *d_cls, int64_t n, int nof_labels,
-                                int min_mss_len, int xdrop_len, int8_t *d_labels_out, int64_t *d_nseg,
-                                void *d_work, int64_t work_bytes, void *stream_)
-{
-    hipStream_t stream = (hipStream_t)stream_;
+static int mss_labels_impl(const double *d_scores, const int8_t *d_cls, int64_t n, int nof_labels, int min_mss_len, int xdrop_len,
+                           int8_t *d_labels_out, int64_t *d_nseg, void *d_work, int64_t work_bytes, hipStream_t stream, bool have_stats)
+{
     DGRP_REQUIRE(n >= 0 && n < (1ll << 31), "dgrp_mss_labels: n=%lld out of range (the reference indexes with int)", (long long)n);
     DGRP_REQUIRE(nof_labels >= 2 && nof_labels <= DGRP_MAXC, "dgrp_mss_labels: nof_labels must be in 2..64");
     if (n == 0) {
@@ -1194,10 +1188,12 @@
     const int min_sc = (int)(s0 * min_mss_len);
     const double thr = xdrop > 0.0 ? xdrop + 1.0 : -1.0;
 
-    DGRP_HIP(hipMemsetAsync(l.blk, 0, (l.nblk + 1) * 8, stream));
-    hipLaunchKernelGGL(mss_blockstat_kernel, dim3((unsigned)((l.nblk + 3) / 4)), dim3(256), 0, stream, d_scores, n, l.blk,
-                       l.blk_sum, l.blk_abs, l.blk_q, l.flags);
-    DGRP_LAUNCH_CHECK();
+    if (!have_stats) {
+        DGRP_HIP(hipMemsetAsync(l.blk, 0, (l.nblk + 1) * 8, stream));
+        hipLaunchKernelGGL(mss_blockstat_kernel, dim3((unsigned)((l.nblk + 3) / 4)), dim3(256), 0, stream, d_scores, n, l.blk,
+                           l.blk_sum, l.blk_abs, l.blk_q, l.flags);
+        DGRP_LAUNCH_CHECK();
+    }
     hipLaunchKernelGGL(mss_superstat_kernel, dim3((unsigned)((l.nsup + 3) / 4)), dim3(256), 0, stream, l.blk_sum, l.blk_abs,
                        l.blk_q, l.flags, l.nblk, l.sup_sum, l.sup_abs, l.sup_q, l.sup_flags);
     DGRP_LAUNCH_CHECK();
@@ -1205,6 +1201,8 @@
     bool single = false;
     for (int attempt = 0; attempt < 2; ++attempt) {
         int64_t nunits = 1;
+        const bool cuts = !single && !getenv("DGRP_MSS_NO_CUTS");
+        bool units_pending = false;
         DGRP_HIP(hipMemsetAsync(l.grand, 0, 64, stream));
         if (!single && xdrop > 0.0) {
             if (attempt == 0) {
@@ -1217,10 +1215,14 @@
             hipLaunchKernelGGL(mss_units_kernel, dim3((unsigned)((l.nblk + 255) / 256)), dim3(256), 0, stream, l.blk, l.flags,
                                l.blk_sum, l.nblk, n, thr, l.ustart, l.urun, l.grand);
             DGRP_LAUNCH_CHECK();
-            uint64_t g = 0;
-            DGRP_HIP(hipMemcpyAsync(&g, l.grand, 8, hipMemcpyDeviceToHost, stream));
-            DGRP_HIP(hipStreamSynchronize(stream));
-            nunits = (int64_t)(g >> 32) + 1;
+            if (cuts) {
+                units_pending = true;
+            } else {
+                uint64_t g = 0;
+                DGRP_HIP(hipMemcpyAsync(&g, l.grand, 8, hipMemcpyDeviceToHost, stream));
+                DGRP_HIP(hipStreamSynchronize(stream));
+                nunits = (int64_t)(g >> 32) + 1;
+            }
         } else {
             int64_t h[2] = { 0, n };
             DGRP_HIP(hipMemcpyAsync(l.ustart, h, 16, hipMemcpyHostToDevice, stream));
@@ -1228,12 +1230,14 @@
             DGRP_HIP(hipMemcpyAsync(l.urun, r, 16, hipMemcpyHostToDevice, stream));
             DGRP_HIP(hipStreamSynchronize(stream));
         }
-        DGRP_REQUIRE(nunits < (1ll << 31), "dgrp_mss_labels: too many stretches");
-        DGRP_HIP(hipMemsetAsync(l.exitL[0], 0, nunits * 8, stream));
-        DGRP_HIP(hipMemsetAsync(l.exitL[1], 0, nunits * 8, stream));
+        if (!units_pending) {
+            DGRP_REQUIRE(nunits < (1ll << 31), "dgrp_mss_labels: too many stretches");
+            DGRP_HIP(hipMemsetAsync(l.exitL[0], 0, nunits * 8, stream));
+            DGRP_HIP(hipMemsetAsync(l.exitL[1], 0, nunits * 8, stream));
+        }
         bool failed = false;
         bool done = false;
-        if (!single && !getenv("DGRP_MSS_NO_CUTS")) {
+        if (cuts) {
             int64_t nl = 1;
             if (xdrop > 0.0) {
                 const char *e = getenv("DGRP_MSS_SUB");
@@ -1246,10 +1250,16 @@
                 hipLaunchKernelGGL(mss_lightunits_kernel, dim3((unsigned)((l.nblk + 255) / 256)), dim3(256), 0, stream, l.lblk, l.grand + 6,
                                    l.flags, l.blk_sum, l.blk, l.grand, l.nblk, n, thr, sub, 1, l.lstart, l.lrun, l.lforced);
                 DGRP_LAUNCH_CHECK();
-                uint64_t g6 = 0;
-                DGRP_HIP(hipMemcpyAsync(&g6, l.grand + 6, 8, hipMemcpyDeviceToHost, stream));
+                uint64_t g7[7] = { 0, 0, 0, 0, 0, 0, 0 };
+                DGRP_HIP(hipMemcpyAsync(g7, l.grand, 56, hipMemcpyDeviceToHost, stream));
                 DGRP_HIP(hipStreamSynchronize(stream));
-                nl = (int64_t)g6 + 1;
+                nl = (int64_t)g7[6] + 1;
+                if (units_pending) {
+                    nunits = (int64_t)(g7[0] >> 32) + 1;
+                    DGRP_REQUIRE(nunits < (1ll << 31), "dgrp_mss_labels: too many stretches");
+                    DGRP_HIP(hipMemsetAsync(l.exitL[0], 0, nunits * 8, stream));
+                    DGRP_HIP(hipMemsetAsync(l.exitL[1], 0, nunits * 8, stream));
+                }
             } else {
                 const int64_t h[2] = { 0, n }, r[2] = { 0, 0 };
                 const uint8_t f[2] = { 1, 1 };
@@ -1258,14 +1268,15 @@
                 DGRP_HIP(hipMemcpyAsync(l.lforced, f, 2, hipMemcpyHostToDevice, stream));
                 DGRP_HIP(hipStreamSynchronize(stream));
             }
+            const int rewalk_all = getenv("DGRP_MSS_NO_SKIP") ? 1 : 0;
             int pass = 0;
             for (;; ++pass) {
                 DGRP_HIP(hipMemsetAsync(l.grand + 1, 0, 8, stream));
-                DGRP_HIP(hipMemsetAsync(l.cut_st, 0xff, l.nblk * 8, stream));
                 hipLaunchKernelGGL(mss_light_kernel, dim3((unsigned)nl), dim3(64), 0, stream, d_scores, l.lstart, l.lrun, l.lforced, nl,
                                    (const mss_light_state *)l.lstate[(pass + 1) & 1], (mss_light_state *)l.lstate[pass & 1], xdrop, l.grand,
                                    pass, l.blk_sum, l.blk_abs, l.blk_q, l.flags, l.sup_sum, l.sup_abs, l.sup_q, l.sup_flags, l.cutcnt,
-                                   l.cut_st, l.cut_run, l.cut_L, l.cut_kj);
+                                   l.cut_st, l.cut_run, l.cut_L, l.cut_kj, (mss_light_state *)l.lentry, (mss_carried_cut *)l.ccut,
+                                   rewalk_all);
                 DGRP_LAUNCH_CHECK();
                 uint64_t g[3] = { 0, 0, 0 };
                 DGRP_HIP(hipMemcpyAsync(g, l.grand, 24, hipMemcpyDeviceToHost, stream));
@@ -1287,8 +1298,8 @@
             {
                 const int64_t threads = nl > l.nblk ? nl : l.nblk;
                 hipLaunchKernelGGL(mss_pieces_kernel, dim3((unsigned)((threads + 255) / 256)), dim3(256), 0, stream, l.lstart, l.lrun, l.lforced,
-                                   nl, (const mss_light_state *)l.lstate[pass & 1], l.cutcnt, l.cut_st, l.cut_run, l.cut_L, l.cut_kj, l.nblk,
-                                   piece_cap, l.ustart2, l.urun2, l.entry2);
+                                   nl, (const mss_light_state *)l.lstate[pass & 1], l.cutcnt, l.cut_st, l.cut_run, l.cut_L, l.cut_kj,
+                                   (const mss_carried_cut *)l.ccut, l.nblk, piece_cap, l.ustart2, l.urun2, l.entry2);
                 DGRP_LAUNCH_CHECK();
             }
             uint64_t np = 0;
@@ -1408,6 +1419,84 @@
     return DGRP_OK;
 }
 
+DGRP_EXPORT int dgrp_mss_labels(const double *d_scores, const int8_t *d_cls, int64_t n, int nof_labels,
+                                int min_mss_len, int xdrop_len, int8_t *d_labels_out, int64_t *d_nseg,
+                                void *d_work, int64_t work_bytes, void *stream)
+{
+    return mss_labels_impl(d_scores, d_cls, n, nof_labels, min_mss_len, xdrop_len, d_labels_out, d_nseg, d_work, work_bytes,
+                           (hipStream_t)stream, false);
+}
+
+int dgrp_scores_blockstat_launch(const float *d_probs, int64_t n, int C, double *d_scores, int8_t *d_cls, uint64_t *blk,
+                                 double *blk_sum, double *blk_abs, int32_t *blk_q, uint8_t *flags, hipStream_t stream);
+
+static int mss_stats_args(const char *who, int64_t n, const void *d_work, int64_t work_bytes, mss_layout *l)
+{
+    DGRP_REQUIRE(n >= 1 && n < (1ll << 31), "%s: n=%lld out of range", who, (long long)n);
+    DGRP_REQUIRE(d_work, "%s: NULL pointer", who);
+    *l = mss_carve((void *)d_work, n);
+    if (work_bytes < l->bytes) {
+        dgrp_set_error("%s: workspace %lld < %lld bytes", who, (long long)work_bytes, (long long)l->bytes);
+        return DGRP_ENOMEM;
+    }
+    return DGRP_OK;
+}
+
+DGRP_EXPORT int dgrp_scores_blockstats(const float *d_probs, int64_t n, int C, double *d_scores, int8_t *d_cls, void *d_work,
+                                       int64_t work_bytes, void *stream)
+{
+    DGRP_REQUIRE(C >= 1 && C <= DGRP_MAXC, "dgrp_scores_blockstats: bad C");
+    mss_layout l;
+    const int rc = mss_stats_args("dgrp_scores_blockstats", n, d_work, work_bytes, &l);
+    if (rc) return rc;
+    DGRP_REQUIRE(d_probs && d_scores && d_cls, "dgrp_scores_blockstats: NULL pointer");
+    return dgrp_scores_blockstat_launch(d_probs, n, C, d_scores, d_cls, l.blk, l.blk_sum, l.blk_abs, l.blk_q, l.flags, (hipStream_t)stream);
+}
+
+DGRP_EXPORT int dgrp_mss_blockstats(const double *d_scores, int64_t n, void *d_work, int64_t work_bytes, void *stream_)
+{
+    hipStream_t stream = (hipStream_t)stream_;
+    mss_layout l;
+    const int rc = mss_stats_args("dgrp_mss_blockstats", n, d_work, work_bytes, &l);
+    if (rc) return rc;
+    DGRP_REQUIRE(d_scores, "dgrp_mss_blockstats: NULL pointer");
+    DGRP_HIP(hipMemsetAsync(l.blk, 0, (l.nblk + 1) * 8, stream));
+    hipLaunchKernelGGL(mss_blockstat_kernel, dim3((unsigned)((l.nblk + 3) / 4)), dim3(256), 0, stream, d_scores, n, l.blk,
+                       l.blk_sum, l.blk_abs, l.blk_q, l.flags);
+    DGRP_LAUNCH_CHECK();
+    return DGRP_OK;
+}
+
+DGRP_EXPORT int dgrp_mss_blockstats_fetch(const void *d_work, int64_t work_bytes, int64_t n, uint64_t *h_blk, double *h_sum,
+                                          double *h_abs, int32_t *h_q, uint8_t *h_flags, void *stream_)
+{
+    hipStream_t stream = (hipStream_t)stream_;
+    mss_layout l;
+    const int rc = mss_stats_args("dgrp_mss_blockstats_fetch", n, d_work, work_bytes, &l);
+    if (rc) return rc;
+    DGRP_REQUIRE(h_blk && h_sum && h_abs && h_q && h_flags, "dgrp_mss_blockstats_fetch: NULL pointer");
+    DGRP_HIP(hipMemcpyAsync(h_blk, l.blk, (l.nblk + 1) * 8, hipMemcpyDeviceToHost, stream));
+    DGRP_HIP(hipMemcpyAsync(h_sum, l.blk_sum, l.nblk * 8, hipMemcpyDeviceToHost, stream));
+    DGRP_HIP(hipMemcpyAsync(h_abs, l.blk_abs, l.nblk * 8, hipMemcpyDeviceToHost, stream));
+    DGRP_HIP(hipMemcpyAsync(h_q, l.blk_q, l.nblk * 4, hipMemcpyDeviceToHost, stream));
+    DGRP_HIP(hipMemcpyAsync(h_flags, l.flags, l.nblk, hipMemcpyDeviceToHost, stream));
+    DGRP_HIP(hipStreamSynchronize(stream));
+    return DGRP_OK;
+}
+
+DGRP_EXPORT int dgrp_scores_mss_labels(const float *d_probs, int64_t n, int C, double *d_scores, int8_t *d_cls, int min_mss_len,
+                                       int xdrop_len, int8_t *d_labels_out, int64_t *d_nseg, void *d_work, int64_t work_bytes,
+                                       void *stream)
+{
+    DGRP_REQUIRE(n >= 0 && n < (1ll << 31), "dgrp_scores_mss_labels: n=%lld out of range (the reference indexes with int)", (long long)n);
+    DGRP_REQUIRE(C >= 2 && C <= DGRP_MAXC, "dgrp_scores_mss_labels: the number of classes must be in 2..64");
+    if (n > 0) {
+        const int rc = dgrp_scores_blockstats(d_probs, n, C, d_scores, d_cls, d_work, work_bytes, stream);
+        if (rc) return rc;
+    }
+    return mss_labels_impl(d_scores, d_cls, n, C, min_mss_len, xdrop_len, d_labels_out, d_nseg, d_work, work_bytes, (hipStream_t)stream, true);
+}
+
 DGRP_EXPORT int dgrp_mss_segments_host(const void *d_work, int64_t work_bytes, int32_t *h_st_en, int64_t cap, int64_t *n_seg)
 {
     DGRP_REQUIRE(d_work && n_seg, "dgrp_mss_segments_host: NULL pointer");
diff --git a/deepgrp_amd/csrc/mss_stats.h b/deepgrp_amd/csrc/mss_stats.h
--- /dev/null
+++ b/deepgrp_amd/csrc/mss_stats.h
@@ -0,0 +1,47 @@
+#pragma once
+#include "dgrp_common.h"
+#include <math.h>
+
+#define MSS_QNONE (-4096)
+#define MSS_QBAD 4096
+
+__device__ __forceinline__ int quantum_exp(double x)
+{
+    const uint64_t b = (uint64_t)__double_as_longlong(x) & 0x7fffffffffffffffull;
+    if (b == 0) return MSS_QNONE;
+    const int e = (int)(b >> 52);
+    if (e == 0 || e == 0x7ff) return MSS_QBAD;
+    const uint64_t m = b & 0x000fffffffffffffull;
+    const int tz = m ? __builtin_ctzll(m) : 52;
+    return -((e - 1023) - 52 + tz);
+}
+
+__device__ __forceinline__ double wave_sum(double v)
+{
+#pragma unroll
+    for (int o = 32; o > 0; o >>= 1) v += __shfl_xor(v, o);
+    return v;
+}
+__device__ __forceinline__ int wave_max(int v)
+{
+#pragma unroll
+    for (int o = 32; o > 0; o >>= 1) { int w = __shfl_xor(v, o); v = w > v ? w : v; }
+    return v;
+}
+
+__device__ __forceinline__ void mss_block_stats(double s, bool pos, bool prevpos, int lane, int64_t b, uint64_t *__restrict__ blk,
+                                                double *__restrict__ blk_sum, double *__restrict__ blk_abs, int32_t *__restrict__ blk_q,
+                                                uint8_t *__restrict__ flags)
+{
+    const unsigned long long mpos = __ballot(pos);
+    const unsigned long long mstart = __ballot(pos && !prevpos);
+    const double sum = wave_sum(s), sabs = wave_sum(fabs(s));
+    const int q = wave_max(quantum_exp(s));
+    if (lane == 0) {
+        flags[b] = (uint8_t)(mpos != 0ull ? 1 : 0);
+        blk[b] = (uint64_t)__popcll(mstart);
+        blk_sum[b] = sum;
+        blk_abs[b] = sabs;
+        blk_q[b] = q;
+    }
+}
diff --git a/deepgrp_amd/csrc/post_kernels.hip b/deepgrp_amd/csrc/post_kernels.hip
--- a/deepgrp_amd/csrc/post_kernels.hip
+++ b/deepgrp_amd/csrc/post_kernels.hip
@@ -1,5 +1,6 @@
 #include "dgrp_common.h"
 #include "scan.h"
+#include "mss_stats.h"
 #include <vector>
 
 #include <math.h>
@@ -42,25 +43,90 @@
     return ldexpf(__fdiv_rn(num, den), (int)q);
 }
 
+__device__ __forceinline__ float score_of_max(float mx, int a)
+{
+    float m = mx + 1e-6f;
+    if (m > 0.99f) m = 0.99f;
+    const float t = np_logf(__fdiv_rn(m, 1.0f - m));
+    return a > 0 ? t : -10.0f * t;
+}
+
+__device__ __forceinline__ float score_row(const float *__restrict__ p, int C, int &a)
+{
+    a = 0;
+    float mx = p[0];
+    for (int c = 1; c < C; ++c) {
+        const float v = p[c];
+        if (v > mx) { mx = v; a = c; }
+    }
+    return score_of_max(mx, a);
+}
+
 __global__ void __launch_bounds__(256) scores_kernel(const float *__restrict__ probs, int64_t n, int C,
                                                      double *__restrict__ scores, int8_t *__restrict__ cls)
 {
     const int64_t nthreads = (int64_t)gridDim.x * blockDim.x;
     for (int64_t i = (int64_t)blockIdx.x * blockDim.x + threadIdx.x; i < n; i += nthreads) {
-        const float *p = probs + i * C;
-        int a = 0;
-        float mx = p[0];
-        for (int c = 1; c < C; ++c) {
-            const float v = p[c];
-            if (v > mx) { mx = v; a = c; }
-        }
-        float m = mx + 1e-6f;
-        if (m > 0.99f) m = 0.99f;
-        const float t = np_logf(__fdiv_rn(m, 1.0f - m));
-        const float sc = a > 0 ? t : -10.0f * t;
+        int a;
+        const float sc = score_row(probs + i * C, C, a);
         scores[i] = (double)sc;
         cls[i] = (int8_t)a;
     }
+}
+
+#define SB_RUN 16
+#define SB_ILP 4
+__global__ void __launch_bounds__(256) scores_blockstat_kernel(const float *__restrict__ probs, int64_t n, int C,
+                                                               double *__restrict__ scores, int8_t *__restrict__ cls,
+                                                               uint64_t *__restrict__ blk, double *__restrict__ blk_sum,
+                                                               double *__restrict__ blk_abs, int32_t *__restrict__ blk_q,
+                                                               uint8_t *__restrict__ flags, int64_t nblk)
+{
+    const int lane = threadIdx.x & 63;
+    const int64_t b0 = ((int64_t)blockIdx.x * 4 + (threadIdx.x >> 6)) * SB_RUN;
+    if (b0 >= nblk) return;
+    const int64_t b1 = b0 + SB_RUN < nblk ? b0 + SB_RUN : nblk;
+    bool front = false;
+    if (lane == 0 && b0 > 0) {
+        int a;
+        front = score_row(probs + (b0 * 64 - 1) * C, C, a) > 0.0f;
+    }
+    for (int64_t b = b0; b < b1; b += SB_ILP) {
+        const float *p[SB_ILP];
+        float mx[SB_ILP];
+        int a[SB_ILP];
+#pragma unroll
+        for (int u = 0; u < SB_ILP; ++u) {
+            const int64_t i = (b + u) * 64 + lane;
+            p[u] = probs + (i < n ? i : n - 1) * C;
+            mx[u] = p[u][0];
+            a[u] = 0;
+        }
+        for (int c = 1; c < C; ++c) {
+#pragma unroll
+            for (int u = 0; u < SB_ILP; ++u) {
+                const float v = p[u][c];
+                if (v > mx[u]) { mx[u] = v; a[u] = c; }
+            }
+        }
+#pragma unroll
+        for (int u = 0; u < SB_ILP; ++u) {
+            const int64_t bu = b + u, i = bu * 64 + lane;
+            if (bu >= b1) break;
+            double s = 0.0;
+            if (i < n) {
+                s = (double)score_of_max(mx[u], a[u]);
+                scores[i] = s;
+                cls[i] = (int8_t)a[u];
+            }
+            const bool pos = i < n && s > 0;
+            const unsigned long long mpos = __ballot(pos);
+            const bool prevpos = lane == 0 ? front : (bool)((mpos >> ((lane - 1) & 63)) & 1ull);
+            mss_block_stats(s, pos, prevpos, lane, bu, blk, blk_sum, blk_abs, blk_q, flags);
+            front = (mpos >> 63) & 1ull;
+        }
+    }
+    if (b1 == nblk && lane == 0) blk[nblk] = 0;
 }
 
 DGRP_EXPORT int dgrp_scores(const float *d_probs, int64_t n, int C, double *d_scores, int8_t *d_cls, void *stream)
@@ -70,6 +136,16 @@
     DGRP_REQUIRE(d_probs && d_scores && d_cls, "dgrp_scores: NULL pointer");
     hipLaunchKernelGGL(scores_kernel, dim3(grid_for(n, 256, 256 * 16)), dim3(256), 0, (hipStream_t)stream, d_probs, n,
                        C, d_scores, d_cls);
+    DGRP_LAUNCH_CHECK();
+    return DGRP_OK;
+}
+
+int dgrp_scores_blockstat_launch(const float *d_probs, int64_t n, int C, double *d_scores, int8_t *d_cls, uint64_t *blk,
+                                 double *blk_sum, double *blk_abs, int32_t *blk_q, uint8_t *flags, hipStream_t stream)
+{
+    const int64_t nblk = (n + 63) / 64;
+    hipLaunchKernelGGL(scores_blockstat_kernel, dim3((unsigned)((nblk + 4 * SB_RUN - 1) / (4 * SB_RUN))), dim3(256), 0, stream, d_probs,
+                       n, C, d_scores, d_cls, blk, blk_sum, blk_abs, blk_q, flags, nblk);
     DGRP_LAUNCH_CHECK();
     return DGRP_OK;
 }
diff --git a/include/deepgrp_hip.h b/include/deepgrp_hip.h
--- a/include/deepgrp_hip.h
+++ b/include/deepgrp_hip.h
@@ -142,6 +142,15 @@
                     void *d_work, int64_t work_bytes, void *stream);
 int dgrp_mss_segments_host(const void *d_work, int64_t work_bytes, int32_t *h_st_en, int64_t cap,
                            int64_t *n_seg);
+
+int dgrp_scores_mss_labels(const float *d_probs, int64_t n, int C, double *d_scores, int8_t *d_cls, int min_mss_len,
+                           int xdrop_len, int8_t *d_labels_out, int64_t *d_nseg, void *d_work, int64_t work_bytes,
+                           void *stream);
+int dgrp_scores_blockstats(const float *d_probs, int64_t n, int C, double *d_scores, int8_t *d_cls, void *d_work,
+                           int64_t work_bytes, void *stream);
+int dgrp_mss_blockstats(const double *d_scores, int64_t n, void *d_work, int64_t work_bytes, void *stream);
+int dgrp_mss_blockstats_fetch(const void *d_work, int64_t work_bytes, int64_t n, uint64_t *h_blk, double *h_sum,
+                              double *h_abs, int32_t *h_q, uint8_t *h_flags, void *stream);
 
 int64_t dgrp_mss_batch_workspace_bytes(int64_t total_n, int64_t nrec);
 int dgrp_mss_labels_batch(const double *d_scores, const int8_t *d_cls, int64_t total_n, int64_t nrec,
```

After: 574.9 (median of 6 runs). About the same (+0.3%).
